# thangktran/HardwareAwareOptimalQuantumCircuitCuttingAndKnitting

Hardware: AMD Instinct MI355X
Metric: subcircuit-instances/s (full-knit wall time = ms_per_step), syc 32 p=2 (higher is better)
Workload: dtype f64

## Files before the change

hardwareawareoptimalquantumcircuitcuttingandknitting_amd/_lib.py:

```python
from __future__ import annotations

import ctypes
import os
import threading

_HERE = os.path.dirname(os.path.abspath(__file__))
LIB_PATH = os.environ.get("QKNIT_LIB") or os.path.join(_HERE, "libqknit.so")

c_i32, c_i64, c_u32, c_u64 = ctypes.c_int32, ctypes.c_int64, ctypes.c_uint32, ctypes.c_uint64
c_vp, c_dp, c_lp = ctypes.c_void_p, ctypes.POINTER(ctypes.c_double), ctypes.POINTER(ctypes.c_int64)


class QkPass(ctypes.Structure):
    _fields_ = [("tile_mask", c_u64), ("group_begin", c_i32), ("group_end", c_i32),
                ("flags", c_i32), ("traced_local", c_u32)]


class QkProgram(ctypes.Structure):
    _fields_ = [("n", c_i32), ("n_eff", c_i32), ("m", c_i32), ("n_slots", c_i32),
                ("packed", c_i32), ("n_passes", c_i32), ("passes", ctypes.POINTER(QkPass)),
                ("ops", c_vp), ("groups", c_vp), ("mats", c_vp)]


class QkLowrankPlan(ctypes.Structure):
    _fields_ = [("nbits", c_i32), ("terms", c_i32), ("rows_a", c_i64), ("rows_b", c_i64), ("mask_a", c_u64),
                ("mask_b", c_u64), ("wt_a", c_vp), ("wt_b", c_vp), ("probes", c_vp), ("lam_tol", ctypes.c_double),
                ("s_tol", ctypes.c_double), ("s_abs", ctypes.c_double), ("rank_tol", ctypes.c_double),
                ("rank_tol_rel", ctypes.c_double)]


class QkKnitPlan(ctypes.Structure):
    _fields_ = [("n_frag", c_i32), ("nbits", c_i32), ("terms", c_i64), ("rows", ctypes.POINTER(c_i64)),
                ("clbit_masks", ctypes.POINTER(c_u64)), ("transforms", ctypes.POINTER(c_vp))]


SIGNATURES = {
    "qk_version": (ctypes.c_char_p, []),
    "qk_ctx_create": (c_i32, [ctypes.c_int, ctypes.POINTER(c_vp)]),
    "qk_ctx_destroy": (c_i32, [c_vp]),
    "qk_ctx_set_stream": (c_i32, [c_vp, c_vp]),
    "qk_ctx_synchronize": (c_i32, [c_vp]),
    "qk_last_error": (ctypes.c_char_p, [c_vp]),
    "qk_stream_create_cu_masked": (c_i32, [ctypes.c_int, ctypes.POINTER(c_u32), ctypes.c_int, ctypes.POINTER(c_vp)]),
    "qk_stream_destroy": (c_i32, [c_vp]),
    "qk_stream_cu_count": (c_i32, [ctypes.c_int, c_vp, ctypes.POINTER(ctypes.c_int)]),
    "qk_out_alloc": (c_i32, [c_vp, c_i64, ctypes.POINTER(c_vp)]),
    "qk_out_free": (c_i32, [c_vp, c_vp]),
    "qk_out_mapped_bytes": (c_i32, [c_vp, ctypes.POINTER(c_i64)]),
    "qk_out_write_rate": (c_i32, [c_vp, c_vp, c_i64, ctypes.POINTER(ctypes.c_double)]),
    "qk_out_stats": (c_i32, [ctypes.POINTER(c_i64), c_i32]),
    "qk_sweep_workspace_bytes": (c_i32, [ctypes.POINTER(QkProgram), c_i64, ctypes.POINTER(c_i64)]),
    "qk_sweep": (c_i32, [c_vp, ctypes.POINTER(QkProgram), c_i64, c_vp, c_vp, c_vp, c_i64, c_vp]),
    "qk_module_compile": (c_i32, [c_vp, ctypes.c_char_p, ctypes.POINTER(ctypes.c_char_p), ctypes.c_int,
                                  ctypes.POINTER(c_vp)]),
    "qk_module_destroy": (c_i32, [c_vp]),
    "qk_module_load": (c_i32, [c_vp, c_vp, c_i64, ctypes.POINTER(ctypes.c_char_p), ctypes.c_int, ctypes.POINTER(c_vp)]),
    "qk_module_code": (c_i32, [c_vp, c_vp, ctypes.POINTER(c_i64)]),
    "qk_sweep_compiled": (c_i32, [c_vp, c_vp, ctypes.POINTER(QkProgram), c_i64, c_vp, c_vp, c_vp, c_i64,
                                  c_vp]),
    "qk_sweep_compiled_labels": (c_i32, [c_vp, c_vp, ctypes.POINTER(QkProgram), c_i64, c_vp, c_vp, c_i64, c_vp,
                                         c_vp, c_i64, c_vp]),
    "qk_sweep_compiled_multi": (c_i32, [c_vp, c_vp, ctypes.c_int, ctypes.POINTER(QkProgram), c_lp, c_vp, c_vp, c_lp,
                                        c_vp, c_vp, c_lp, c_vp, c_vp]),
    "qk_sweep_compiled_multi_shared": (c_i32, [c_vp, c_vp, ctypes.c_int, ctypes.POINTER(QkProgram), c_lp, c_vp, c_vp,
                                               c_lp, c_vp, c_vp, c_lp, c_vp, c_vp, c_lp, c_vp, c_vp]),
    "qk_reduce_labels": (c_i32, [c_vp, c_i64, c_vp, c_i64, c_vp, c_vp]),
    "qk_gemm_keyed": (c_i32, [c_vp, c_i64, c_i64, c_i64, c_vp, c_i64, c_vp, c_i64, c_vp, c_i64,
                              c_vp, c_i64, c_vp, ctypes.c_int]),
    "qk_gemm_keyed_pred": (c_i32, [c_vp, c_i64, c_i64, c_i64, c_vp, c_i64, c_vp, c_i64, c_vp, c_i64,
                                   c_vp, c_i64, c_vp, ctypes.c_int, c_vp]),
    "qk_gemm_outer_paired": (c_i32, [c_vp, c_i64, c_i64, c_i64, c_vp, c_i64, c_vp, c_i64, c_vp, c_i64,
                                     c_vp, c_vp]),
    "qk_knit_outer_stream": (c_i32, [c_vp, ctypes.c_int, c_i64, c_vp, c_i64, c_vp, c_i64, ctypes.c_uint64,
                                     ctypes.c_uint64, c_vp]),
    "qk_knit_outer_stream_kind": (c_i32, [ctypes.c_int, c_i64, c_u64, c_u64, c_i64, c_i64,
                                          ctypes.POINTER(ctypes.c_int), ctypes.POINTER(ctypes.c_int)]),
    "qk_knit_outer_stream_range": (c_i32, [c_vp, ctypes.c_int, c_i64, c_vp, c_i64, c_vp, c_i64, ctypes.c_uint64,
                                           ctypes.c_uint64, c_i64, c_i64, c_vp, c_vp]),
    "qk_rank_factors": (c_i32, [c_vp, c_i64, c_vp, c_vp, ctypes.c_double, ctypes.c_double, ctypes.c_double,
                                ctypes.c_int, c_vp, c_vp, c_vp]),
    "qk_prep_workspace_bytes": (c_i32, [c_vp, c_i64, c_i64, ctypes.POINTER(c_i64)]),
    "qk_prep_operands": (c_i32, [c_vp, ctypes.c_int, ctypes.c_int, c_vp, c_vp, c_i64, c_i64, c_vp, ctypes.c_int,
                                 c_vp, c_vp, c_i64, c_i64, c_vp, c_vp, c_vp, c_vp, c_vp, c_vp, c_i64]),
    "qk_qprep_workspace_bytes": (c_i32, [c_vp, c_i64, c_i64, ctypes.POINTER(c_i64)]),
    "qk_qprep_grams": (c_i32, [c_vp, ctypes.c_int, ctypes.c_int, c_vp, c_vp, c_i64, c_i64, ctypes.c_int, c_vp, c_vp,
                               c_i64, c_i64, c_vp, c_vp, c_vp, c_vp, c_vp, c_i64]),
    "qk_qprep_compress_check": (c_i32, [c_vp, ctypes.c_int, ctypes.c_int, ctypes.c_int, c_vp, c_vp, c_i64, c_i64,
                                        ctypes.c_int, c_vp, c_vp, c_i64, c_i64, c_vp, c_vp, c_vp, c_vp, c_vp, c_vp,
                                        c_vp, c_vp, ctypes.c_double, ctypes.c_double, c_vp, c_vp, c_vp, c_i64]),
    "qk_compress_operands": (c_i32, [c_vp, ctypes.c_int, ctypes.c_int, c_vp, c_vp, c_i64, c_vp, c_vp, c_vp, c_i64,
                                     c_vp]),
    "qk_compress_operands_ld": (c_i32, [c_vp, ctypes.c_int, ctypes.c_int, c_vp, c_vp, c_i64, c_i64, c_vp, c_i64, c_vp,
                                        c_vp, c_i64, c_i64, c_vp, c_i64]),
    "qk_compress_probe_v": (c_i32, [c_vp, ctypes.c_int, ctypes.c_int, c_vp, c_vp, c_i64, c_i64, c_vp, c_i64, c_vp, c_vp,
                                    c_i64, c_i64, c_vp, c_i64, c_vp, c_i64, c_vp, c_i64]),
    "qk_probe_errors_vpart": (c_i32, [c_vp, ctypes.c_int, ctypes.c_int, c_vp, c_i64, c_i64, c_vp, c_i64, c_vp, c_vp,
                                      c_i64, c_vp, c_vp, ctypes.c_double, ctypes.c_double, c_vp, c_vp, c_vp, c_i64,
                                      c_vp]),
    "qk_probe_workspace_bytes": (c_i32, [c_vp, c_i64, ctypes.POINTER(c_i64)]),
    "qk_probe_errors": (c_i32, [c_vp, ctypes.c_int, ctypes.c_int, c_vp, c_i64, c_i64, c_vp, c_i64, c_vp, c_vp, c_i64,
                                c_i64, c_vp, c_i64, c_vp, c_vp, ctypes.c_double, ctypes.c_double, c_vp, c_vp, c_vp,
                                c_i64]),
    "qk_probe_errors_tally": (c_i32, [c_vp, ctypes.c_int, ctypes.c_int, c_vp, c_i64, c_i64, c_vp, c_i64, c_vp, c_vp, c_i64,
                                c_i64, c_vp, c_i64, c_vp, c_vp, ctypes.c_double, ctypes.c_double, c_vp, c_vp, c_vp,
                                c_i64, c_vp]),
    "qk_probe_accept": (c_i32, [c_vp, c_vp, ctypes.c_int, c_vp, ctypes.c_double, ctypes.c_double, c_vp, c_vp]),
    "qk_rank_tally": (c_i32, [c_vp, c_vp, c_vp, c_vp]),
    "qk_knit_workspace_bytes": (c_i32, [ctypes.POINTER(QkKnitPlan), ctypes.POINTER(c_i64)]),
    "qk_knit": (c_i32, [c_vp, ctypes.POINTER(QkKnitPlan), c_vp, c_vp, c_i64, c_vp]),
    "qk_khatri_rao": (c_i32, [c_vp, c_i64, c_i64, c_i64, c_vp, c_i64, c_vp, c_i64, c_vp]),
    "qk_gather_rows": (c_i32, [c_vp, c_i64, c_i64, c_vp, c_vp, c_vp, c_vp]),
    "qk_npd_workspace_bytes": (c_i32, [c_i64, c_i64, ctypes.POINTER(c_i64)]),
    "qk_threshold_count": (c_i32, [c_vp, c_i64, c_vp, ctypes.c_double, c_vp, c_i64, c_vp]),
    "qk_npd": (c_i32, [c_vp, c_i64, c_vp, ctypes.c_double, c_i64, c_vp, c_i64, c_vp, c_vp, c_vp]),
    "qk_qd_from_rows": (c_i32, [c_vp, c_i64, c_i64, c_vp, c_vp, ctypes.c_double, c_vp]),
    "qk_qd_merge": (c_i32, [c_vp, c_i64, c_vp, c_vp, c_i64, c_vp, c_vp, ctypes.c_double, c_i64, c_vp]),
    "qk_qd_axpby": (c_i32, [c_vp, c_i64, ctypes.c_double, c_vp, ctypes.c_double, c_vp, ctypes.c_double, c_vp]),
    "qk_hellinger": (c_i32, [c_vp, c_i64, c_vp, c_vp, c_vp]),
    "qk_knit_lowrank_workspace_bytes": (c_i32, [c_vp, c_vp, ctypes.POINTER(c_i64)]),
    "qk_knit_lowrank": (c_i32, [c_vp, c_vp, c_vp, c_vp, c_vp, c_i64, c_vp, c_vp]),
    "qk_comm_unique_id": (c_i32, [c_vp]),
    "qk_comm_init": (c_i32, [c_vp, c_vp, ctypes.c_int, ctypes.c_int, ctypes.POINTER(c_vp)]),
    "qk_comm_destroy": (c_i32, [c_vp]),
    "qk_comm_size": (c_i32, [c_vp, ctypes.POINTER(ctypes.c_int), ctypes.POINTER(ctypes.c_int)]),
    "qk_allreduce": (c_i32, [c_vp, c_vp, c_vp, c_vp, c_i64]),
    "qk_reduce": (c_i32, [c_vp, c_vp, c_vp, c_vp, c_i64, ctypes.c_int]),
    "qk_allgather": (c_i32, [c_vp, c_vp, c_vp, c_vp, c_i64]),
    "qk_alltoall": (c_i32, [c_vp, c_vp, c_vp, c_vp, c_i64]),
    "qk_knit_select_workspace_bytes": (c_i32, [ctypes.c_int, c_u64, c_u64, ctypes.POINTER(c_i64)]),
    "qk_knit_select": (c_i32, [c_vp, ctypes.c_int, c_i64, c_vp, c_i64, c_vp, c_i64, c_u64, c_u64, ctypes.c_double,
                               c_vp, c_vp, c_i64, c_i64, c_vp, c_vp, c_vp]),
    "qk_select_above": (c_i32, [c_vp, c_i64, c_vp, ctypes.c_double, c_i64, c_i64, c_vp, c_vp, c_vp]),
    "qk_npd_pairs_workspace_bytes": (c_i32, [c_i64, ctypes.POINTER(c_i64)]),
    "qk_npd_pairs": (c_i32, [c_vp, c_i64, c_vp, c_vp, c_vp, c_i64, c_vp, c_vp, c_vp]),
    "qk_sample_cdf": (c_i32, [c_vp, c_i64, c_vp, c_i64, c_vp, c_vp]),
    "qk_sample_counts": (c_i32, [c_vp, c_i64, c_i64, c_vp, c_vp, c_vp, c_i64, c_vp, c_i64, c_u64, c_vp]),
    "qk_fold_counts": (c_i32, [c_vp, c_i64, c_vp, c_i64, c_vp, c_vp, c_i64, ctypes.c_double, c_vp]),
}

_lock = threading.Lock()
_lib = None


class QknitError(RuntimeError):
    pass


def lib() -> ctypes.CDLL:
    global _lib
    with _lock:
        if _lib is None:
            if not os.path.exists(LIB_PATH):
                raise QknitError(
                    f"{LIB_PATH} not built: run `python -c 'import __graft_entry__ as g; g.build()'`"
                )
            handle = ctypes.CDLL(LIB_PATH)
            for name, (res, args) in SIGNATURES.items():
                fn = getattr(handle, name)
                fn.restype = res
                fn.argtypes = args
            _lib = handle
# ... 8 lines not shown
```

hardwareawareoptimalquantumcircuitcuttingandknitting_amd/build.py:

```python
from __future__ import annotations

import os
import shutil
import subprocess

HERE = os.path.dirname(os.path.abspath(__file__))
SRCS = [os.path.join(HERE, "csrc", f) for f in ("qknit.hip", "qknit_post.hip", "qknit_jit.hip",
                                                              "qknit_sample.hip", "qknit_rank.hip",
                                                              "qknit_plan.hip", "qknit_prep.hip",
                                                              "qknit_select.hip", "qknit_comm.hip",
                                                              "qknit_mem.hip", "qknit_trunc.hip",
                                                              "qknit_prim.hip")]
DEPS = SRCS + [os.path.join(HERE, "csrc", h) for h in ("internal.h", "sweep_ops.h", "prim.h")]
HEADER = os.path.join(os.path.dirname(HERE), "include", "qknit.h")
OUT = os.path.join(HERE, "libqknit.so")
ARCH = os.environ.get("QKNIT_ARCH", "gfx950")


def hipcc() -> str:
    for cand in (os.environ.get("HIPCC"), shutil.which("hipcc"), "/opt/rocm/bin/hipcc"):
        if cand and os.path.exists(cand):
            return cand
    raise RuntimeError("hipcc not found")


def build_library(force: bool = False, verbose: bool = False, out: str = OUT,
                  defines: tuple = ()) -> str:
    stale = not os.path.exists(out) or any(
        os.path.getmtime(p) > os.path.getmtime(out) for p in DEPS + [HEADER]
    )
    if not (force or stale):
        return out
    tmp = out + ".tmp"
    flags = [f"--offload-arch={ARCH}", "-O3", "-std=c++17", "-fPIC", "-Wall", "-Wno-unused-result",
             *[f"-D{d}" for d in defines]]
    objdir = os.path.join(os.path.dirname(out), "build", os.path.basename(out) + ".objs")
    os.makedirs(objdir, exist_ok=True)
    jobs = []
    for src in SRCS:
        obj = os.path.join(objdir, os.path.basename(src) + ".o")
        cmd = [hipcc(), *flags, "-c", src, "-o", obj]
        jobs.append((cmd, obj, subprocess.Popen(cmd, stdout=subprocess.PIPE, stderr=subprocess.PIPE, text=True)))
    errs = []
    for cmd, obj, proc in jobs:
        _, err = proc.communicate()
        if proc.returncode != 0:
            errs.append(f"{' '.join(cmd)}\n{err}")
        elif verbose and err:
            print(err)
    if errs:
        raise RuntimeError("hipcc failed:\n" + "\n".join(errs))
    cmd = [hipcc(), *flags, "-shared", *[obj for _, obj, _ in jobs], "-lhiprtc", "-lrccl", "-o", tmp]
    res = subprocess.run(cmd, capture_output=True, text=True)
    if res.returncode != 0:
        raise RuntimeError(f"hipcc link failed:\n{' '.join(cmd)}\n{res.stderr}")
    os.replace(tmp, out)
    return out


AOT_CONFIGS = ("qft_16_1_p3", "syc_32_5_p2", "syc_32_1_p2", "syc_32_1_p2_forced", "hwe_16_1_p2", "hwe_16_1_p3")


def build_jit_cache(configs=AOT_CONFIGS, verbose: bool = False) -> list:
    import tempfile

    from . import VirtualCircuit, cutting, engine

    todo = {}
    for key in configs:
        name, n, d, p, var = cutting.BASELINE_CONFIGS[key]
        cut = cutting.config_cut_circuit(name, n, d, p, var)[1]
        virt = VirtualCircuit(cut)
        for basis in ({False, True} if virt.vgate_instructions else {False}):
            for src, _ in engine.jit_sources(virt, basis=basis):
                path = engine.jit_cache_path(src)
                if not os.path.exists(path):
                    todo[path] = src
    os.makedirs(engine.JIT_CACHE_DIR, exist_ok=True)
    procs = []
    with tempfile.TemporaryDirectory() as tmp:
        for i, (path, src) in enumerate(todo.items()):
            f = os.path.join(tmp, f"prog{i}.hip")
            with open(f, "w") as fh:
                fh.write(src)
            cmd = [hipcc(), "--genco", "--no-gpu-bundle-output", *engine.jit_options(src), f, "-o", path + ".tmp"]
            procs.append((path, cmd, subprocess.Popen(cmd, stdout=subprocess.PIPE, stderr=subprocess.PIPE, text=True)))
        errs = []
        for path, cmd, proc in procs:
            _, err = proc.communicate()
            if proc.returncode != 0:
                errs.append(f"{' '.join(cmd)}\n{err}")
            else:
                os.replace(path + ".tmp", path)
                if verbose:
                    print(f"jit cache: {path}")
        if errs:
# ... 3 lines not shown
```

hardwareawareoptimalquantumcircuitcuttingandknitting_amd/csrc/qknit.hip:

```cpp
#include <hip/hip_runtime.h>

#include <cstdlib>

#include <cstdint>
#include <cstdio>
#include <cstring>
#include <string>

#include "internal.h"
#include "sweep_ops.h"

namespace {

constexpr int TILE = 1 << QK_TILE_BITS;
constexpr int NT = 256;

int fail(qk_ctx* ctx, int code, const char* fmt, const char* detail = "") {
    if (ctx) {
        char buf[512];
        snprintf(buf, sizeof(buf), fmt, detail);
        ctx->err = buf;
    }
    return code;
}

#define QK_HIP(ctx, call)                                                     \
    do {                                                                      \
        hipError_t e_ = (call);                                               \
        if (e_ != hipSuccess) return fail(ctx, QK_EHIP, "%s", hipGetErrorString(e_)); \
    } while (0)

using namespace qk_sweep_ops;

__device__ __forceinline__ void pin(double2 (&v)[PER]) {
#pragma unroll
    for (int r = 0; r < PER; ++r) asm volatile("" : "+v"(v[r].x), "+v"(v[r].y));
}

__device__ __forceinline__ void dispatch_u1(int a, double2 (&v)[PER], const double* m) {
    switch (a) {
        case 0: ap_u1<0>(v, m); pin(v); break;
        case 1: ap_u1<1>(v, m); pin(v); break;
        case 2: ap_u1<2>(v, m); pin(v); break;
        default: ap_u1<3>(v, m); pin(v); break;
    }
}

__device__ __forceinline__ void dispatch_u1r(int a, double2 (&v)[PER], const double* m) {
    switch (a) {
        case 0: ap_u1r<0>(v, m); pin(v); break;
        case 1: ap_u1r<1>(v, m); pin(v); break;
        case 2: ap_u1r<2>(v, m); pin(v); break;
        default: ap_u1r<3>(v, m); pin(v); break;
    }
}

__device__ __forceinline__ void dispatch_u1x(int a, double2 (&v)[PER], const double* m) {
    switch (a) {
        case 0: ap_u1x<0>(v, m); pin(v); break;
        case 1: ap_u1x<1>(v, m); pin(v); break;
        case 2: ap_u1x<2>(v, m); pin(v); break;
        default: ap_u1x<3>(v, m); pin(v); break;
    }
}

__device__ __forceinline__ void dispatch_d1r(int a, double2 (&v)[PER], const double* d) {
    switch (a) {
        case 0: ap_d1r<0>(v, d); pin(v); break;
        case 1: ap_d1r<1>(v, d); pin(v); break;
        case 2: ap_d1r<2>(v, d); pin(v); break;
        default: ap_d1r<3>(v, d); pin(v); break;
    }
}

__device__ __forceinline__ void dispatch_d1(int a, double2 (&v)[PER], const double* d) {
    switch (a) {
        case 0: ap_d1<0>(v, d); pin(v); break;
        case 1: ap_d1<1>(v, d); pin(v); break;
        case 2: ap_d1<2>(v, d); pin(v); break;
        default: ap_d1<3>(v, d); pin(v); break;
    }
}

__device__ __forceinline__ int pair_id(int a, int b) {
    return a == 0 ? b - 1 : (a == 1 ? b + 1 : 5);
}

__device__ __forceinline__ void dispatch_u2(int a, int b, double2 (&v)[PER], const double* m) {
    switch (pair_id(a, b)) {
        case 0: ap_u2<0, 1>(v, m); pin(v); break;
        case 1: ap_u2<0, 2>(v, m); pin(v); break;
        case 2: ap_u2<0, 3>(v, m); pin(v); break;
// ... 322 lines not shown

#ifndef QK_GEMM_GROUP
#define QK_GEMM_GROUP 8
#endif
#ifndef QK_GEMM_NT
#define QK_GEMM_NT 1
#endif

typedef double d2_t __attribute__((ext_vector_type(2)));

__device__ __forceinline__ void gemm_load(d2_t (&r)[4], const double* __restrict__ X, int64_t ld,
                                          int64_t k0, int64_t K, int64_t c0, int64_t cols, bool full) {
    const double* p = X + k0 * ld + c0;
    const int rl = threadIdx.x >> 6, cl = 2 * (threadIdx.x & 63);
    const int64_t off = (int64_t)rl * ld + cl;
    if (full) {
#pragma unroll
        for (int j = 0; j < 4; ++j) r[j] = *reinterpret_cast<const d2_t*>(p + 4 * j * ld + off);
    } else {
        const int kl = (int)(K - k0 < GK ? K - k0 : GK);
        const int cc = (int)(cols - c0 < GT ? cols - c0 : GT);
#pragma unroll
        for (int j = 0; j < 4; ++j) {
            const double* q = p + 4 * j * ld + off;
            const bool rv = rl + 4 * j < kl;
            r[j].x = (rv && cl < cc) ? q[0] : 0.0;
            r[j].y = (rv && cl + 1 < cc) ? q[1] : 0.0;
        }
    }
}

#ifndef QK_GEMM_STORE
#define QK_GEMM_STORE 1
#endif

template <typename T>
__device__ __forceinline__ T dpp_swap_pair(T v) {
    static_assert(sizeof(T) == 8, "64-bit values only");
    int2 w = *reinterpret_cast<int2*>(&v);
    w.x = __builtin_amdgcn_mov_dpp(w.x, 0xB1, 0xF, 0xF, false);
    w.y = __builtin_amdgcn_mov_dpp(w.y, 0xB1, 0xF, 0xF, false);
    return *reinterpret_cast<T*>(&w);
}

__device__ __forceinline__ void gemm_store_pair(double* p, d2_t v) {
#if QK_GEMM_STORE == 2
    asm volatile("global_store_dwordx4 %0, %1, off sc1\n\ts_nop 1" : : "v"(p), "v"(v) : "memory");
#elif QK_GEMM_STORE == 3
    *reinterpret_cast<d2_t*>(p) = v;
#else
    __builtin_nontemporal_store(v, reinterpret_cast<d2_t*>(p));
#endif
}

__device__ __forceinline__ void gemm_store_out(double* p, double v) {
#if QK_GEMM_NT
    __builtin_nontemporal_store(v, p);
#else
    *p = v;
#endif
}

#ifndef QK_GEMM_PERSIST
#define QK_GEMM_PERSIST 1
#endif
#ifndef QK_GEMM_WG_PER_CU
#define QK_GEMM_WG_PER_CU 2
#endif

struct GemmArgs {
    int64_t M, N, K;
    const double* __restrict__ A;
    int64_t lda;
    const double* __restrict__ B;
    int64_t ldb;
    const int64_t* __restrict__ keyA;
    int64_t strideA;
    const int64_t* __restrict__ keyB;
    int64_t strideB;
    double* __restrict__ out;
    int beta;
    int64_t tiles_m, tiles_n;
    const int32_t* skip = nullptr;
};

__device__ __forceinline__ bool gemm_skipped(const GemmArgs& g) { return g.skip && *g.skip > 0; }

__device__ __forceinline__ void gemm_tile_coords(int64_t seq, int64_t tiles_m, int64_t tiles_n,
                                                 int64_t& bm, int64_t& bn) {
    const uint32_t q = (uint32_t)seq, tm = (uint32_t)tiles_m, tn = (uint32_t)tiles_n;
#if QK_GEMM_GROUP
    const uint32_t per_group = (uint32_t)QK_GEMM_GROUP * tn;
    const uint32_t g = q / per_group, r = q - g * per_group;
    const uint32_t first = g * QK_GEMM_GROUP;
    const uint32_t gsize = tm - first < (uint32_t)QK_GEMM_GROUP ? tm - first : (uint32_t)QK_GEMM_GROUP;
    bm = first + r % gsize;
    bn = r / gsize;
#else
    bm = q % tm;
    bn = q / tm;
#endif
}

template <bool FULL>
__device__ __forceinline__ void gemm_epilogue(const GemmArgs& g, int64_t m0, int64_t n0, d4_t (&acc)[4][4]) {
    const int lane = threadIdx.x & 63, wave = threadIdx.x >> 6;
    const int wm = wave & 1, wn = wave >> 1;
    const int64_t M = g.M, N = g.N;
    int64_t kcol[4];
#pragma unroll
    for (int j = 0; j < 4; ++j) {
        const int64_t col = n0 + wn * 64 + j * 16 + (lane & 15);
        kcol[j] = (FULL || col < N) ? (g.keyB ? g.keyB[col] : col * g.strideB) : -1;
    }
#if QK_GEMM_STORE
    bool pairable = FULL || (!g.beta && n0 + GT <= N);
    if (pairable) {
        bool ok = true;
#pragma unroll
        for (int j = 0; j < 4; ++j) {
            const int64_t nb = dpp_swap_pair(kcol[j]);
            ok = ok && ((lane & 1) ? nb + 1 == kcol[j] : kcol[j] + 1 == nb);
        }
        pairable = __all(ok);
    }
    if (pairable) {
        const bool odd = lane & 1;
#pragma unroll
        for (int i = 0; i < 4; ++i) {
#pragma unroll
            for (int rp = 0; rp < 4; rp += 2) {
                const int rr = rp + (odd ? 1 : 0);
                const int64_t row = m0 + wm * 64 + i * 16 + (lane >> 4) + 4 * rr;
                const int64_t krow = (FULL || row < M) ? (g.keyA ? g.keyA[row] : row * g.strideA) : -1;
#pragma unroll
                for (int j = 0; j < 4; ++j) {
                    const double x = odd ? acc[i][j][rp] : acc[i][j][rp + 1];
                    const double y = dpp_swap_pair(x);
                    d2_t v;
                    v.x = odd ? y : acc[i][j][rp];
                    v.y = odd ? acc[i][j][rp + 1] : y;
#ifdef QK_GEMM_NOSTORE
                    if (v.x != 1234.5678) continue;
#endif
                    if (FULL || krow >= 0) gemm_store_pair(g.out + krow + kcol[j] - (odd ? 1 : 0), v);
                }
            }
        }
        return;
    }
#endif
#pragma unroll
    for (int i = 0; i < 4; ++i) {
        int64_t krow[4];
#pragma unroll
        for (int r = 0; r < 4; ++r) {
            const int64_t row = m0 + wm * 64 + i * 16 + (lane >> 4) + 4 * r;
            krow[r] = row < M ? (g.keyA ? g.keyA[row] : row * g.strideA) : -1;
        }
#pragma unroll
        for (int j = 0; j < 4; ++j)
#pragma unroll
            for (int r = 0; r < 4; ++r) {
#ifdef QK_GEMM_NOSTORE
                if (acc[i][j][r] != 1234.5678) continue;
#endif
                if (krow[r] < 0 || kcol[j] < 0) continue;
                double* o = g.out + krow[r] + kcol[j];
                if (g.beta) *o += acc[i][j][r];
                else gemm_store_out(o, acc[i][j][r]);
            }
    }
}

__device__ __forceinline__ bool gemm_vec(const double* X, int64_t ld, int64_t c0, int64_t cols) {
    return ((ld & 1) == 0) && ((reinterpret_cast<uintptr_t>(X) & 15) == 0) && c0 + GT <= cols;
}

__device__ __forceinline__ void gemm_load_first(const GemmArgs& g, int64_t bm, int64_t bn, d2_t (&ra)[4],
                                                d2_t (&rb)[4]) {
    gemm_load(ra, g.A, g.lda, 0, g.K, bm * GT, g.M, gemm_vec(g.A, g.lda, bm * GT, g.M) && GK <= g.K);
    gemm_load(rb, g.B, g.ldb, 0, g.K, bn * GT, g.N, gemm_vec(g.B, g.ldb, bn * GT, g.N) && GK <= g.K);
}

__device__ __forceinline__ void gemm_tile(const GemmArgs& g, int64_t bm, int64_t bn, bool have_next,
                                          int64_t nbm, int64_t nbn, d2_t (&ra)[4], d2_t (&rb)[4],
                                          double (*As)[GK][GT + GPAD], double (*Bs)[GK][GT + GPAD],
                                          int& buf) {
    const int tid = threadIdx.x, lane = tid & 63, wave = tid >> 6;
    const int wm = wave & 1, wn = wave >> 1;
    const int64_t M = g.M, N = g.N, K = g.K;
    const int64_t m0 = bm * GT, n0 = bn * GT;

    d4_t acc[4][4];
#pragma unroll
    for (int i = 0; i < 4; ++i)
#pragma unroll
        for (int j = 0; j < 4; ++j) acc[i][j] = (d4_t){0.0, 0.0, 0.0, 0.0};

    const int lr = tid >> 6;
    const int lc = 2 * (tid & 63);
    for (int64_t k0 = 0; k0 < K; k0 += GK) {
#ifdef QK_GEMM_NOLDSW
        if (k0 == 0)
#endif
        {
#pragma unroll
        for (int j = 0; j < 4; ++j) {
            *reinterpret_cast<d2_t*>(&As[buf][lr + 4 * j][lc]) = ra[j];
            *reinterpret_cast<d2_t*>(&Bs[buf][lr + 4 * j][lc]) = rb[j];
        }
        __syncthreads();
        }
        const bool more = k0 + GK < K;
#ifdef QK_GEMM_NOLOAD
        if (!more && have_next) {
#else
        if (more || have_next) {
#endif
            const int64_t pk = more ? k0 + GK : 0;
            const int64_t pm = more ? m0 : nbm * GT, pn = more ? n0 : nbn * GT;
            const bool kfull = pk + GK <= K;
            gemm_load(ra, g.A, g.lda, pk, K, pm, M, gemm_vec(g.A, g.lda, pm, M) && kfull);
            gemm_load(rb, g.B, g.ldb, pk, K, pn, N, gemm_vec(g.B, g.ldb, pn, N) && kfull);
        }
#pragma unroll
        for (int kk = 0; kk < GK / 4; ++kk) {
            const int kr2 = kk * 4 + (lane >> 4);
            double fa[4], fb[4];
#pragma unroll
            for (int t = 0; t < 4; ++t) {
                fa[t] = As[buf][kr2][wm * 64 + t * 16 + (lane & 15)];
                fb[t] = Bs[buf][kr2][wn * 64 + t * 16 + (lane & 15)];
            }
#pragma unroll
            for (int i = 0; i < 4; ++i)
#pragma unroll
                for (int j = 0; j < 4; ++j)
                    acc[i][j] = __builtin_amdgcn_mfma_f64_16x16x4f64(fa[i], fb[j], acc[i][j], 0, 0, 0);
        }
        buf ^= 1;
    }
    gemm_epilogue<false>(g, m0, n0, acc);
}

__global__ __launch_bounds__(256, 2) void qk_gemm_keyed_kernel(GemmArgs g) {
    __shared__ __attribute__((aligned(16))) double As[2][GK][GT + GPAD];
    __shared__ __attribute__((aligned(16))) double Bs[2][GK][GT + GPAD];
    if (gemm_skipped(g)) return;
    const int64_t nblk = g.tiles_m * g.tiles_n;
    int buf = 0;
    int64_t bm, bn;
#if QK_GEMM_PERSIST
    const int64_t G = gridDim.x;
    const bool xcd = nblk % 8 == 0 && G % 8 == 0;
    const int64_t per_xcd = xcd ? nblk / 8 : nblk, stride = xcd ? G / 8 : G;
    const int64_t base = xcd ? (blockIdx.x % 8) * per_xcd : 0;
    int64_t li = xcd ? blockIdx.x / 8 : blockIdx.x;
    if (li >= per_xcd) return;
    d2_t ra[4], rb[4];
    gemm_tile_coords(base + li, g.tiles_m, g.tiles_n, bm, bn);
    gemm_load_first(g, bm, bn, ra, rb);
    for (; li < per_xcd; li += stride) {
        const bool have_next = li + stride < per_xcd;
        int64_t nbm = 0, nbn = 0;
        if (have_next) gemm_tile_coords(base + li + stride, g.tiles_m, g.tiles_n, nbm, nbn);
        gemm_tile(g, bm, bn, have_next, nbm, nbn, ra, rb, As, Bs, buf);
        bm = nbm;
        bn = nbn;
    }
#else
    int64_t bid = (int64_t)blockIdx.y * gridDim.x + blockIdx.x;
    if (bid >= nblk) return;
    if (nblk % 8 == 0) bid = (bid % 8) * (nblk / 8) + bid / 8;
    gemm_tile_coords(bid, g.tiles_m, g.tiles_n, bm, bn);
    d2_t ra[4], rb[4];
    gemm_load_first(g, bm, bn, ra, rb);
    gemm_tile(g, bm, bn, false, 0, 0, ra, rb, As, Bs, buf);
#endif
}

#ifndef QK_GEMM_GLDS
#define QK_GEMM_GLDS 1
#endif
#ifndef QK_G2K
#define QK_G2K 16
#endif
#ifndef QK_G2S
#define QK_G2S 2
#endif
#ifndef QK_GLDS_WG_PER_CU
#define QK_GLDS_WG_PER_CU 2
#endif
#ifndef QK_GEMM_PRIO
#define QK_GEMM_PRIO 0
#endif
constexpr int G2K = QK_G2K;
constexpr int G2S = QK_G2S;
constexpr int G2L = G2K / 2;

struct GemmRing {
    double a[G2K][GT + GPAD];
    double b[G2K][GT + GPAD];
};

__device__ __forceinline__ void glds16(const double* src, double* lds_row) {
    __builtin_amdgcn_global_load_lds(reinterpret_cast<const void*>(src),
                                     reinterpret_cast<__attribute__((address_space(3))) void*>(
                                         reinterpret_cast<uintptr_t>(lds_row)),
                                     16, 0, 0);
}

__device__ __forceinline__ void gemm_ring_wait(int n) {
#define QK_VMW(k) case k: asm volatile("s_waitcnt vmcnt(" #k ")" ::: "memory"); break;
#define QK_VMW8(k) QK_VMW(k) QK_VMW(k + 1) QK_VMW(k + 2) QK_VMW(k + 3) QK_VMW(k + 4) QK_VMW(k + 5) QK_VMW(k + 6) QK_VMW(k + 7)
    switch (n < 63 ? n : 63) {
        QK_VMW8(0) QK_VMW8(8) QK_VMW8(16) QK_VMW8(24) QK_VMW8(32) QK_VMW8(40) QK_VMW8(48)
        QK_VMW(56) QK_VMW(57) QK_VMW(58) QK_VMW(59) QK_VMW(60) QK_VMW(61) QK_VMW(62) QK_VMW(63)
        default: asm volatile("s_waitcnt vmcnt(0)" ::: "memory");
    }
#undef QK_VMW8
#undef QK_VMW
}

__global__ __launch_bounds__(256, 2) void qk_gemm_glds_kernel(GemmArgs g) {
    __shared__ __attribute__((aligned(16))) GemmRing ring[G2S];
    if (gemm_skipped(g)) return;
    const int lane = threadIdx.x & 63, wave = threadIdx.x >> 6;
    const int wm = wave & 1, wn = wave >> 1;
    const int64_t nblk = g.tiles_m * g.tiles_n;
    const int64_t G = gridDim.x;
    const bool xcd = nblk % 8 == 0 && G % 8 == 0;
    const int64_t per_xcd = xcd ? nblk / 8 : nblk, stride = xcd ? G / 8 : G;
    const int64_t base = xcd ? (blockIdx.x % 8) * per_xcd : 0;
    const int64_t li0 = xcd ? blockIdx.x / 8 : blockIdx.x;
    if (li0 >= per_xcd) return;
    const int nct = (int)(g.K / G2K);
    const int ntile = (int)((per_xcd - li0 + stride - 1) / stride);
    const int total = ntile * nct;

    int it = 0, ic = 0, issued = 0;
    int64_t ibm, ibn;
    gemm_tile_coords(base + li0, g.tiles_m, g.tiles_n, ibm, ibn);
    const int wave_s = __builtin_amdgcn_readfirstlane(wave);
    const int src_off = 2 * lane;
    auto issue = [&]() {
        if (issued >= total) return;
        GemmRing& r = ring[issued % G2S];
        const int64_t k0 = (int64_t)ic * G2K;
#pragma unroll
        for (int q = 0; q < G2K / 4; ++q) {
            const int row = wave_s * (G2K / 4) + q;
            const double* pa = g.A + (k0 + row) * g.lda + ibm * GT;
            const double* pb = g.B + (k0 + row) * g.ldb + ibn * GT;
            glds16(pa + src_off, &r.a[row][0]);
            glds16(pb + src_off, &r.b[row][0]);
        }
        ++issued;
        if (++ic == nct) {
            ic = 0;
            ++it;
            if (it < ntile) gemm_tile_coords(base + li0 + (int64_t)it * stride, g.tiles_m, g.tiles_n, ibm, ibn);
        }
    };
    for (int s = 0; s < G2S - 1; ++s) issue();

    d4_t acc[4][4];
#pragma unroll
    for (int i = 0; i < 4; ++i)
#pragma unroll
        for (int j = 0; j < 4; ++j) acc[i][j] = (d4_t){0.0, 0.0, 0.0, 0.0};
    int64_t bm, bn;
    gemm_tile_coords(base + li0, g.tiles_m, g.tiles_n, bm, bn);
    int t = 0, c = 0;
    for (int gc = 0; gc < total; ++gc) {
        int after = G2L * ((total - 1 - gc) < (G2S - 2) ? (total - 1 - gc) : (G2S - 2));
#pragma unroll
        for (int d = 1; d < G2S; ++d)
            if (gc - d >= 0 && (gc - d + 1) % nct == 0) after += 32;
        gemm_ring_wait(after);
        asm volatile("s_waitcnt lgkmcnt(0)" ::: "memory");
        __builtin_amdgcn_s_barrier();
        const GemmRing& r = ring[gc % G2S];
        double fa[2][4], fb[2][4];
        auto frags = [&](int kk) {
            const int kr = kk * 4 + (lane >> 4);
#pragma unroll
            for (int q = 0; q < 4; ++q) {
                fa[kk & 1][q] = r.a[kr][wm * 64 + q * 16 + (lane & 15)];
                fb[kk & 1][q] = r.b[kr][wn * 64 + q * 16 + (lane & 15)];
            }
        };
        frags(0);
        issue();
#pragma unroll
        for (int kk = 0; kk < G2K / 4; ++kk) {
            if (kk + 1 < G2K / 4) frags(kk + 1);
#if QK_GEMM_PRIO
            __builtin_amdgcn_s_setprio(1);
#endif
#pragma unroll
            for (int i = 0; i < 4; ++i)
#pragma unroll
                for (int j = 0; j < 4; ++j)
                    acc[i][j] = __builtin_amdgcn_mfma_f64_16x16x4f64(fa[kk & 1][i], fb[kk & 1][j], acc[i][j], 0,
                                                                     0, 0);
#if QK_GEMM_PRIO
            __builtin_amdgcn_s_setprio(0);
#endif
        }
        if (++c == nct) {
            gemm_epilogue<true>(g, bm * GT, bn * GT, acc);
#pragma unroll
            for (int i = 0; i < 4; ++i)
#pragma unroll
                for (int j = 0; j < 4; ++j) acc[i][j] = (d4_t){0.0, 0.0, 0.0, 0.0};
            c = 0;
            if (++t < ntile) gemm_tile_coords(base + li0 + (int64_t)t * stride, g.tiles_m, g.tiles_n, bm, bn);
        }
    }
}

#ifndef QK_GEMM_WAVE
#define QK_GEMM_WAVE 1
#endif
#ifndef QK_WAVE_WG_PER_CU
#define QK_WAVE_WG_PER_CU 2
#endif
constexpr int DW = 4;

struct WaveRing {
    double a[DW][4][64];
    double b[DW][4][64];
    int64_t key[2][64];
};

__device__ __forceinline__ void glds16_at(const void* src, void* lds_base) {
    __builtin_amdgcn_global_load_lds(src,
                                     reinterpret_cast<__attribute__((address_space(3))) void*>(
                                         reinterpret_cast<uintptr_t>(lds_base)),
                                     16, 0, 0);
}

template <int NKS>
__global__ __launch_bounds__(256, 2) void qk_gemm_wave_kernel(GemmArgs g) {
    __shared__ __attribute__((aligned(16))) WaveRing rings[4];
    if (gemm_skipped(g)) return;
    const int lane = threadIdx.x & 63, wave = threadIdx.x >> 6;
    const int wm = wave & 1, wn = wave >> 1;
    WaveRing& ring = rings[__builtin_amdgcn_readfirstlane(wave)];
    const int64_t nblk = g.tiles_m * g.tiles_n;
    const int64_t G = gridDim.x;
    const bool xcd = nblk % 8 == 0 && G % 8 == 0;
    const int64_t per_xcd = xcd ? nblk / 8 : nblk, stride = xcd ? G / 8 : G;
    const int64_t base = xcd ? (blockIdx.x % 8) * per_xcd : 0;
    int64_t li = xcd ? blockIdx.x / 8 : blockIdx.x;
    if (li >= per_xcd) return;
    const int64_t lda = g.lda, ldb = g.ldb;
    const int p = lane & 31;
    const int chunkA = p < 16 ? 2 * p : 2 * (p - 16) + 1;
    const int64_t offA = (int64_t)(lane >> 5) * lda + wm * 64 + 2 * chunkA;
    const int64_t offB = (int64_t)(lane >> 5) * ldb + wn * 64 + 2 * p;
    const int64_t* tabA = g.keyA ? g.keyA : reinterpret_cast<const int64_t*>(g.A);
    const int64_t* tabB = g.keyB ? g.keyB : reinterpret_cast<const int64_t*>(g.B);
    const int64_t keyOff = 2 * (lane & 31);

    int64_t bm, bn;
    gemm_tile_coords(base + li, g.tiles_m, g.tiles_n, bm, bn);
    const double* pa = g.A + bm * GT + offA;
    const double* pb = g.B + bn * GT + offB;
    const double* na = pa;
    const double* nb = pb;
    if (li + stride < per_xcd) {
        int64_t tbm, tbn;
        gemm_tile_coords(base + li + stride, g.tiles_m, g.tiles_n, tbm, tbn);
        na = g.A + tbm * GT + offA;
        nb = g.B + tbn * GT + offB;
    }
    auto issue = [&](int slot, int ks) {
        const double* a = ks < NKS ? pa + (int64_t)(4 * ks) * lda : na + (int64_t)(4 * (ks - NKS)) * lda;
        const double* b = ks < NKS ? pb + (int64_t)(4 * ks) * ldb : nb + (int64_t)(4 * (ks - NKS)) * ldb;
        glds16_at(a, &ring.a[slot][0][0]);
        glds16_at(a + 2 * lda, &ring.a[slot][2][0]);
        glds16_at(b, &ring.b[slot][0][0]);
        glds16_at(b + 2 * ldb, &ring.b[slot][2][0]);
    };
#pragma unroll
    for (int s = 0; s < DW - 1; ++s) issue(s, s);

    int prev_stores = 0;
    const int rho = lane & 15, kk = lane >> 4;
    auto tile = [&]() -> bool {
        d4_t acc[4][4];
#pragma unroll
        for (int i = 0; i < 4; ++i)
#pragma unroll
            for (int j = 0; j < 4; ++j) acc[i][j] = (d4_t){0.0, 0.0, 0.0, 0.0};
        static_assert(NKS % DW == 0, "k-steps per tile must be a multiple of the ring depth");
#pragma unroll
        for (int ks = 0; ks < NKS; ++ks) {
            issue((ks + DW - 1) % DW, ks + DW - 1);
            if (ks == 0) {
                const int64_t* t = lane < 32 ? tabA + (g.keyA ? bm * GT + wm * 64 : 0) + keyOff
                                             : tabB + (g.keyB ? bn * GT + wn * 64 : 0) + keyOff;
                glds16_at(t, &ring.key[0][0]);
            }
            static_assert(DW == 4, "wait counts below are for a 4-deep ring");
            if (ks <= DW - 2) {
                if (prev_stores == 0) asm volatile("s_waitcnt vmcnt(13)" ::: "memory");
                else if (prev_stores == 32) asm volatile("s_waitcnt vmcnt(45)" ::: "memory");
                else asm volatile("s_waitcnt vmcnt(63)" ::: "memory");
            } else if (ks == DW - 1) {
                asm volatile("s_waitcnt vmcnt(13)" ::: "memory");
            } else {
                asm volatile("s_waitcnt vmcnt(12)" ::: "memory");
            }
            const int s = ks % DW;
            const d2_t a0 = *reinterpret_cast<const d2_t*>(&ring.a[s][kk][2 * rho]);
            const d2_t a1 = *reinterpret_cast<const d2_t*>(&ring.a[s][kk][32 + 2 * rho]);
            const d2_t b0 = *reinterpret_cast<const d2_t*>(&ring.b[s][kk][2 * rho]);
            const d2_t b1 = *reinterpret_cast<const d2_t*>(&ring.b[s][kk][32 + 2 * rho]);
            const double fa[4] = {a0.x, a0.y, a1.x, a1.y};
            const double fb[4] = {b0.x, b0.y, b1.x, b1.y};
#pragma unroll
            for (int i = 0; i < 4; ++i)
#pragma unroll
                for (int j = 0; j < 4; ++j)
                    acc[i][j] = __builtin_amdgcn_mfma_f64_16x16x4f64(fa[i], fb[j], acc[i][j], 0, 0, 0);
            __builtin_amdgcn_sched_barrier(0);
        }
        static_assert(4 * (NKS - 1) <= 63, "vmcnt field");
        asm volatile("s_waitcnt vmcnt(%0)" ::"n"(4 * (NKS - 1)) : "memory");
        const int64_t* keyR = &ring.key[0][0];
        const int64_t* keyC = &ring.key[0][0] + 64;
        int64_t kr[4][4], kc[4];
        if (g.keyA) {
#pragma unroll
            for (int r = 0; r < 4; ++r)
#pragma unroll
                for (int i = 0; i < 4; ++i) kr[r][i] = keyR[4 * kk + 16 * r + i];
        } else {
#pragma unroll
            for (int r = 0; r < 4; ++r)
#pragma unroll
                for (int i = 0; i < 4; ++i) kr[r][i] = (bm * GT + wm * 64 + 4 * kk + 16 * r + i) * g.strideA;
        }
        if (g.keyB) {
#pragma unroll
            for (int j = 0; j < 4; ++j) kc[j] = keyC[2 * rho + (j & 1) + 32 * (j >> 1)];
        } else {
#pragma unroll
            for (int j = 0; j < 4; ++j) kc[j] = (bn * GT + wn * 64 + 2 * rho + (j & 1) + 32 * (j >> 1)) * g.strideB;
        }
        int64_t odd = (kc[0] | kc[2]) & 1;
#pragma unroll
        for (int r = 0; r < 4; ++r)
#pragma unroll
            for (int i = 0; i < 4; ++i) odd |= kr[r][i] & 1;
        const bool pair = __all(kc[1] == kc[0] + 1 && kc[3] == kc[2] + 1 && odd == 0);
        if (pair) {
#pragma unroll
            for (int r = 0; r < 4; ++r)
#pragma unroll
                for (int i = 0; i < 4; ++i)
#pragma unroll
                    for (int jp = 0; jp < 2; ++jp) {
                        d2_t v;
                        v.x = acc[i][2 * jp][r];
                        v.y = acc[i][2 * jp + 1][r];
                        gemm_store_pair(g.out + kr[r][i] + kc[2 * jp], v);
                    }
            prev_stores = 32;
        } else {
#pragma unroll
            for (int r = 0; r < 4; ++r)
#pragma unroll
                for (int i = 0; i < 4; ++i)
#pragma unroll
                    for (int j = 0; j < 4; ++j) gemm_store_out(g.out + kr[r][i] + kc[j], acc[i][j][r]);
            prev_stores = 64;
        }
        li += stride;
        if (li >= per_xcd) return false;
        gemm_tile_coords(base + li, g.tiles_m, g.tiles_n, bm, bn);
        pa = na;
        pb = nb;
        if (li + stride < per_xcd) {
            int64_t tbm, tbn;
            gemm_tile_coords(base + li + stride, g.tiles_m, g.tiles_n, tbm, tbn);
            na = g.A + tbm * GT + offA;
            nb = g.B + tbn * GT + offB;
        }
        return true;
    };
    while (tile()) {
    }
    asm volatile("s_waitcnt vmcnt(0)" ::: "memory");
}

constexpr int SK_MAX = 8;
#ifndef QK_SK_U
#define QK_SK_U 4
#endif
constexpr int SK_U = QK_SK_U;

template <bool KEYED>
__global__ __launch_bounds__(256) void qk_gemm_smallk_kernel(GemmArgs g) {
    if (gemm_skipped(g)) return;
    const int K = (int)g.K;
    for (int64_t row = blockIdx.x; row < g.M; row += gridDim.x) {
        double a[SK_MAX];
#pragma unroll
        for (int k = 0; k < SK_MAX; ++k) a[k] = k < K ? g.A[k * g.lda + row] : 0.0;
        const int64_t base = g.keyA ? g.keyA[row] : row * g.strideA;
        double* o = g.out + base;
        if ((base & 1) == 0) {
            int64_t j0 = 2 * (int64_t)threadIdx.x;
            for (; j0 + 512 * (SK_U - 1) < g.N; j0 += 512 * SK_U) {
                d2_t acc[SK_U];
#pragma unroll
                for (int u = 0; u < SK_U; ++u) acc[u] = (d2_t){0.0, 0.0};
#pragma unroll
                for (int k = 0; k < SK_MAX; ++k) {
                    if (k < K) {
#pragma unroll
                        for (int u = 0; u < SK_U; ++u) {
                            const d2_t b = *reinterpret_cast<const d2_t*>(g.B + k * g.ldb + j0 + 512 * u);
                            acc[u].x = fma(a[k], b.x, acc[u].x);
                            acc[u].y = fma(a[k], b.y, acc[u].y);
                        }
                    }
                }
#pragma unroll
                for (int u = 0; u < SK_U; ++u) {
                    const int64_t col = KEYED ? g.keyB[j0 + 512 * u] : j0 + 512 * u;
                    __builtin_nontemporal_store(acc[u], reinterpret_cast<d2_t*>(o + col));
                }
            }
            for (int64_t j = j0; j < g.N; j += 512) {
                d2_t acc = {0.0, 0.0};
                for (int k = 0; k < K; ++k) {
                    const d2_t b = *reinterpret_cast<const d2_t*>(g.B + k * g.ldb + j);
                    acc.x = fma(a[k], b.x, acc.x);
                    acc.y = fma(a[k], b.y, acc.y);
                }
                __builtin_nontemporal_store(acc, reinterpret_cast<d2_t*>(o + (KEYED ? g.keyB[j] : j)));
            }
        } else {
            for (int64_t j = threadIdx.x; j < g.N; j += 256) {
                double acc = 0.0;
                for (int k = 0; k < K; ++k) acc = fma(a[k], g.B[k * g.ldb + j], acc);
                __builtin_nontemporal_store(acc, o + (KEYED ? g.keyB[j] : j));
            }
        }
    }
}

#ifndef QK_OS_U
#define QK_OS_U 1
#endif
#ifndef QK_OS_NT
#define QK_OS_NT 1
#endif
#ifndef QK_OS_WG_PER_CU
#define QK_OS_WG_PER_CU 8
#endif
#ifndef QK_OS_P
#define QK_OS_P 1
#endif
constexpr int OS_U = QK_OS_U;
constexpr int OS_P = QK_OS_P;
constexpr int64_t OS_CHUNK = 2 * OS_P * 256 * OS_U;

struct OuterStreamArgs {
    int nbits, K;
    const double* __restrict__ A;
    int64_t lda;
    const double* __restrict__ B;
    int64_t ldb;
    uint32_t maskA, maskB;
    double* __restrict__ out;
};

__device__ __forceinline__ uint32_t pext32(uint32_t x, uint32_t mask) {
    uint32_t r = 0, bit = 1;
    for (; mask; mask &= mask - 1, bit <<= 1)
        if (x & mask & (~mask + 1)) r |= bit;
    return r;
}

__global__ __launch_bounds__(256) void qk_knit_outer_stream_kernel(OuterStreamArgs a) {
    __shared__ uint32_t tab[2][4][256];
    for (int i = threadIdx.x; i < 4 * 256; i += 256) {
        const int byte = i >> 8, v = i & 255;
        tab[0][byte][v] = pext32((uint32_t)v << (8 * byte), a.maskA);
        tab[1][byte][v] = pext32((uint32_t)v << (8 * byte), a.maskB);
    }
    __syncthreads();
    const int K = a.K;
    const int64_t total = int64_t(1) << a.nbits;
    for (int64_t c0 = (int64_t)blockIdx.x * OS_CHUNK; c0 < total; c0 += (int64_t)gridDim.x * OS_CHUNK) {
        d2_t v[OS_U * OS_P];
#pragma unroll
        for (int up = 0; up < OS_U * OS_P; ++up) {
            const int u = up / OS_P, pp = up % OS_P;
            const int64_t o = c0 + 512 * OS_P * u + 2 * (OS_P * threadIdx.x + pp);
            const uint32_t x = (uint32_t)o;
            uint32_t row = 0, col = 0;
#pragma unroll
            for (int byte = 0; byte < 4; ++byte) {
                const uint32_t b = (x >> (8 * byte)) & 255;
                row += tab[0][byte][b];
                col += tab[1][byte][b];
            }
            d2_t acc = {0.0, 0.0};
            if (o < total) {
#pragma unroll
                for (int k = 0; k < SK_MAX; ++k) {
                    if (k < K) {
                        const double av = a.A[k * a.lda + row];
                        const d2_t bv = *reinterpret_cast<const d2_t*>(a.B + k * a.ldb + col);
                        acc.x = fma(av, bv.x, acc.x);
                        acc.y = fma(av, bv.y, acc.y);
                    }
                }
            }
            v[up] = acc;
        }
#pragma unroll
        for (int up = 0; up < OS_U * OS_P; ++up) {
            const int u = up / OS_P, pp = up % OS_P;
            const int64_t o = c0 + 512 * OS_P * u + 2 * (OS_P * threadIdx.x + pp);
            if (o < total) {
#if QK_OS_NT
                __builtin_nontemporal_store(v[up], reinterpret_cast<d2_t*>(a.out + o));
#else
                *reinterpret_cast<d2_t*>(a.out + o) = v[up];
#endif
            }
        }
    }
}

#ifndef QK_OB_NT
#define QK_OB_NT 0
#endif
struct OuterBlockedArgs {
    int K, TB;
    const double* __restrict__ A;
    int64_t lda;
    const double* __restrict__ B;
    int64_t ldb;
    uint32_t maskA, maskB;
    int64_t task_begin, task_end;
    int64_t o_begin;
    const int32_t* kdev;
    double* __restrict__ out;
    int64_t spread;
};

template <bool BG>
__global__ __launch_bounds__(256) void qk_knit_outer_blocked_kernel(OuterBlockedArgs a) {
    int K = a.K;
    if (a.kdev) {
        const int kd = *a.kdev;
        if (kd <= 0) return;
        K = kd < K ? kd : K;
    }
    __shared__ uint32_t tab[2][2][256];
    extern __shared__ double stage[];
    const uint32_t low = (1u << a.TB) - 1u;
    const uint32_t mAl = a.maskA & low, mBl = a.maskB & low;
    const int na = 1 << __builtin_popcount(mAl), nb = 1 << __builtin_popcount(mBl);
    double* sA = stage;
    double* sB = stage + (int64_t)a.K * na;
    for (int i = threadIdx.x; i < 512; i += 256) {
        const int byte = i >> 8, v = i & 255;
        tab[0][byte][v] = pext32((uint32_t)v << (8 * byte), mAl);
        tab[1][byte][v] = pext32((uint32_t)v << (8 * byte), mBl);
    }
    __syncthreads();
    const uint32_t r0 = tab[0][0][(2 * threadIdx.x) & 255], c0 = tab[1][0][(2 * threadIdx.x) & 255];
    const int iters = (1 << a.TB) / 512;
    const int64_t n_tasks = a.task_end - a.task_begin, per_part = n_tasks / a.spread;
    for (int64_t i = blockIdx.x; i < n_tasks; i += gridDim.x) {
        const int64_t t = a.task_begin + (i % a.spread) * per_part + i / a.spread;
        const uint32_t base = (uint32_t)(t << a.TB);
        const uint32_t ah = pext32(base, a.maskA), bh = pext32(base, a.maskB);
        __syncthreads();
        for (int i = threadIdx.x; i < K * na; i += 256) {
            const int k = i / na;
            sA[i] = a.A[k * a.lda + ah + (i - k * na)];
        }
        if (!BG)
            for (int i = threadIdx.x; i < K * nb; i += 256) {
                const int k = i / nb;
                sB[i] = a.B[k * a.ldb + bh + (i - k * nb)];
            }
        __syncthreads();
        const double* Bg = a.B + bh;
        double* o = a.out + ((int64_t)base - a.o_begin);
#pragma unroll 4
        for (int it = 0; it < iters; ++it) {
            const uint32_t hi = (uint32_t)(2 * it + (threadIdx.x >> 7));
            const uint32_t row = r0 + tab[0][1][hi], col = c0 + tab[1][1][hi];
            d2_t acc = {0.0, 0.0};
#pragma unroll
            for (int k = 0; k < SK_MAX; ++k)
                if (k < K) {
                    const double av = sA[k * na + row];
                    const d2_t bv = BG ? *reinterpret_cast<const d2_t*>(Bg + k * a.ldb + col)
                                       : *reinterpret_cast<const d2_t*>(sB + k * nb + col);
                    acc.x = fma(av, bv.x, acc.x);
                    acc.y = fma(av, bv.y, acc.y);
                }
#if QK_OB_NT
            __builtin_nontemporal_store(acc, reinterpret_cast<d2_t*>(o + 512 * it + 2 * threadIdx.x));
#else
            *reinterpret_cast<d2_t*>(o + 512 * it + 2 * threadIdx.x) = acc;
#endif
        }
    }
}

struct OuterRowsArgs {
    int K;
    const double* __restrict__ A;
    int64_t lda;
    const double* __restrict__ B;
    int64_t ldb;
    uint32_t maskA_hi, maskB_hi;
    int64_t piece_begin, piece_end;
    int64_t o_begin;
    const int32_t* kdev;
    double* __restrict__ out;
    int64_t spread;
};

template <int KR, int C>
__global__ __launch_bounds__(256) void qk_knit_outer_rows_kernel(OuterRowsArgs a) {
    constexpr int NP = 1 << (C - 9);
    int K = a.K;
    if (a.kdev) {
        const int kd = *a.kdev;
        if (kd <= 0) return;
        K = kd < K ? kd : K;
    }
    d2_t b[KR][NP];
    int64_t pb_loaded = -1;
    const int64_t n_pieces = a.piece_end - a.piece_begin, per_part = n_pieces / a.spread;
    for (int64_t i = blockIdx.x; i < n_pieces; i += gridDim.x) {
        const int64_t p = a.piece_begin + (i % a.spread) * per_part + i / a.spread;
        const uint32_t pl = (uint32_t)p;
        const int64_t pb = pext32(pl, a.maskB_hi);
        const uint32_t pa = pext32(pl, a.maskA_hi);
        if (pb != pb_loaded) {
            const double* Bp = a.B + (pb << C) + 2 * threadIdx.x;
#pragma unroll
            for (int k = 0; k < KR; ++k)
#pragma unroll
                for (int i = 0; i < NP; ++i)
                    b[k][i] = k < K ? *reinterpret_cast<const d2_t*>(Bp + k * a.ldb + 512 * i) : (d2_t){0.0, 0.0};
            pb_loaded = pb;
        }
        double av[KR];
#pragma unroll
        for (int k = 0; k < KR; ++k) av[k] = k < K ? a.A[k * a.lda + pa] : 0.0;
        double* o = a.out + ((p << C) - a.o_begin) + 2 * threadIdx.x;
#pragma unroll
        for (int i = 0; i < NP; ++i) {
            d2_t acc = {0.0, 0.0};
#pragma unroll
            for (int k = 0; k < KR; ++k)
                if (k < K) {
                    acc.x = fma(av[k], b[k][i].x, acc.x);
                    acc.y = fma(av[k], b[k][i].y, acc.y);
                }
            *reinterpret_cast<d2_t*>(o + 512 * i) = acc;
        }
    }
}

static int outer_rows_bits(int64_t K, uint64_t maskB, int align_bits) {
    static const int off = getenv("QKNIT_OB_ROWS") ? atoi(getenv("QKNIT_OB_ROWS")) : 1;
    if (!off || K < 1 || K > 8) return 0;
    const int low = __builtin_ctzll(~maskB);
    const int want = K <= 1 ? 13 : (K <= 2 ? 12 : 11);
    return (want <= low && want <= align_bits) ? want : 0;
}

template <int KR, int C>
static int outer_rows_per_cu() {
    static int n = [] {
        int b = 0;
        if (hipOccupancyMaxActiveBlocksPerMultiprocessor(&b, qk_knit_outer_rows_kernel<KR, C>, 256, 0) != hipSuccess)
            b = 2;
        return b < 1 ? 1 : b;
    }();
    return n;
}

constexpr int64_t OB_STAGE_BYTES = 24 * 1024;
constexpr int OB_WG_PER_CU = 64;

int outer_blocked_tile(int nbits, int64_t K, uint64_t maskA, uint64_t maskB, int align_bits, bool* b_global) {
// ... 130 lines not shown

int qk_sweep_workspace_bytes(const qk_program* p, int64_t n_jobs, int64_t* bytes) {
    if (!p || !bytes || n_jobs < 0) return QK_EARG;
    *bytes = p->packed ? 0 : n_jobs * ((int64_t)1 << p->n) * (int64_t)sizeof(double2);
    return QK_OK;
}

int qk_sweep(qk_ctx* ctx, const qk_program* p, int64_t n_jobs, const double* job_slots,
             const double* job_sign, void* workspace, int64_t workspace_bytes, double* pjob) {
    if (!ctx) return QK_EARG;
    if (!p || !p->passes || p->n_passes < 1) return fail(ctx, QK_EARG, "qk_sweep: empty program%s");
    if (n_jobs <= 0) return QK_OK;
    if (!job_sign || !pjob || (p->n_slots > 0 && !job_slots))
        return fail(ctx, QK_EARG, "qk_sweep: null buffer%s");
    if (p->m < 0 || p->m > p->n_eff || p->n_eff > 40)
        return fail(ctx, QK_EARG, "qk_sweep: bad widths%s");
    if (p->packed) {
        if (p->n_eff < QK_FIBER_BITS || p->n_eff > QK_TILE_BITS || p->n_passes != 1)
            return fail(ctx, QK_EARG, "qk_sweep: bad PACKED program%s");
    } else {
        if (p->n <= QK_TILE_BITS || p->n_eff != p->n) return fail(ctx, QK_EARG, "qk_sweep: bad SPLIT program%s");
        int64_t need = 0;
        qk_sweep_workspace_bytes(p, n_jobs, &need);
        if (!workspace || workspace_bytes < need) return fail(ctx, QK_EARG, "qk_sweep: workspace too small%s");
    }
    if (!(p->passes[p->n_passes - 1].flags & 2) || !(p->passes[0].flags & 1))
        return fail(ctx, QK_EARG, "qk_sweep: first pass must INIT and last must be FINAL%s");
    QK_HIP(ctx, hipSetDevice(ctx->device));
    SweepArgs a{};
    a.ops = p->ops;
    a.groups = p->groups;
    a.mats = p->mats;
    a.job_slots = job_slots;
    a.job_sign = job_sign;
    a.state = (double2*)workspace;
    a.pjob = pjob;
    a.n_jobs = n_jobs;
    a.n = p->n;
    a.n_eff = p->n_eff;
    a.m = p->m;
    a.n_slots = p->n_slots;
    for (int ip = 0; ip < p->n_passes; ++ip) {
        const qk_pass& ps = p->passes[ip];
        if (!p->packed && __builtin_popcountll(ps.tile_mask) != QK_TILE_BITS)
            return fail(ctx, QK_EARG, "qk_sweep: SPLIT tile must hold 12 state bits%s");
        a.tile_mask = ps.tile_mask;
        a.group_begin = ps.group_begin;
        a.group_end = ps.group_end;
        a.flags = ps.flags;
        a.traced_local = ps.traced_local;
        const uint64_t nmask = (p->n >= 64) ? ~0ull : ((1ull << p->n) - 1);
        a.init_sparse = (!p->packed && ip == 0 && p->n_passes > 1) ? 1 : 0;
        a.zero_mask = (!p->packed && ip == 1) ? (nmask & ~p->passes[0].tile_mask) : 0;
        if (p->packed) {
            const int64_t per = (int64_t)1 << (QK_TILE_BITS - p->n_eff);
            const int64_t blocks = (n_jobs + per - 1) / per;
            if (blocks > 0x7fffffff) return fail(ctx, QK_EARG, "qk_sweep: too many jobs%s");
            hipLaunchKernelGGL(qk_sweep_pass_kernel<true>, dim3((unsigned)blocks), dim3(NT), 0, ctx->stream, a,
                               a.ops, a.groups, a.mats);
        } else {
            const int64_t blocks = a.init_sparse ? n_jobs : (n_jobs << (p->n - QK_TILE_BITS));
            if (blocks > 0x7fffffff) return fail(ctx, QK_EARG, "qk_sweep: too many tiles%s");
            hipLaunchKernelGGL(qk_sweep_pass_kernel<false>, dim3((unsigned)blocks), dim3(NT), 0, ctx->stream, a,
                               a.ops, a.groups, a.mats);
        }
        QK_HIP(ctx, hipGetLastError());
    }
    return QK_OK;
}

int qk_reduce_labels(qk_ctx* ctx, int64_t n_labels, const int64_t* offsets, int64_t width,
                     const double* pjob, double* q) {
    if (!ctx) return QK_EARG;
    if (n_labels < 0 || width < 0) return fail(ctx, QK_EARG, "qk_reduce_labels: negative size%s");
    if (n_labels == 0 || width == 0) return QK_OK;
    if (!offsets || !pjob || !q) return fail(ctx, QK_EARG, "qk_reduce_labels: null buffer%s");
    QK_HIP(ctx, hipSetDevice(ctx->device));
    hipLaunchKernelGGL(qk_reduce_labels_kernel, dim3(grid_for(n_labels * width, 256)), dim3(256), 0,
                       ctx->stream, n_labels, offsets, width, pjob, q);
    QK_HIP(ctx, hipGetLastError());
    return QK_OK;
}

int qk_gemm_keyed(qk_ctx* ctx, int64_t M, int64_t N, int64_t K, const double* A, int64_t lda,
                  const double* B, int64_t ldb, const int64_t* keyA, int64_t strideA,
                  const int64_t* keyB, int64_t strideB, double* out, int beta) {
    return qk_gemm_keyed_pred(ctx, M, N, K, A, lda, B, ldb, keyA, strideA, keyB, strideB, out, beta, nullptr);
}

int qk_gemm_keyed_pred(qk_ctx* ctx, int64_t M, int64_t N, int64_t K, const double* A, int64_t lda,
                       const double* B, int64_t ldb, const int64_t* keyA, int64_t strideA,
                       const int64_t* keyB, int64_t strideB, double* out, int beta, const int32_t* skip) {
    if (!ctx) return QK_EARG;
    if (M < 0 || N < 0 || K < 0) return fail(ctx, QK_EARG, "qk_gemm_keyed: negative size%s");
    if (M == 0 || N == 0) return QK_OK;
    if (!out || (K > 0 && (!A || !B))) return fail(ctx, QK_EARG, "qk_gemm_keyed: null buffer%s");
    if (lda < M || ldb < N) return fail(ctx, QK_EARG, "qk_gemm_keyed: leading dimension too small%s");
    const int64_t tm = (M + GT - 1) / GT, tn = (N + GT - 1) / GT;
    const int64_t nblk = tm * tn;
    QK_HIP(ctx, hipSetDevice(ctx->device));
    if (nblk >= (int64_t(1) << 31)) return fail(ctx, QK_EARG, "qk_gemm_keyed: too many tiles%s");
    GemmArgs g{M, N, K, A, lda, B, ldb, keyA, strideA, keyB, strideB, out, beta, tm, tn, skip};
    const bool aligned16 = ((reinterpret_cast<uintptr_t>(A) | reinterpret_cast<uintptr_t>(B)) & 15) == 0 &&
                           (lda % 2) == 0 && (ldb % 2) == 0;
    if (K >= 1 && K <= SK_MAX && !beta && !keyB && strideB == 1 && N % 2 == 0 && aligned16 &&
        (reinterpret_cast<uintptr_t>(out) & 15) == 0 && M * N >= (int64_t(1) << 16)) {
        const int cus = ctx->cus;
        const int64_t G = M < (int64_t)cus * 8 ? M : (int64_t)cus * 8;
        hipLaunchKernelGGL(qk_gemm_smallk_kernel<false>, dim3((unsigned)G), dim3(256), 0, ctx->stream, g);
        QK_HIP(ctx, hipGetLastError());
        return QK_OK;
    }
    if (QK_GEMM_WAVE && !beta && M % GT == 0 && N % GT == 0 && (K == 16 || K == 32 || K == 64) && aligned16 &&
        ((reinterpret_cast<uintptr_t>(out) | reinterpret_cast<uintptr_t>(keyA) | reinterpret_cast<uintptr_t>(keyB)) &
         15) == 0) {
        const int cus = ctx->cus;
        int64_t G = (int64_t)cus * QK_WAVE_WG_PER_CU;
        G = G < 8 ? 8 : G - G % 8;
        if (G > nblk) G = nblk;
        if (K == 16) hipLaunchKernelGGL(qk_gemm_wave_kernel<4>, dim3((unsigned)G), dim3(256), 0, ctx->stream, g);
        else if (K == 32) hipLaunchKernelGGL(qk_gemm_wave_kernel<8>, dim3((unsigned)G), dim3(256), 0, ctx->stream, g);
        else hipLaunchKernelGGL(qk_gemm_wave_kernel<16>, dim3((unsigned)G), dim3(256), 0, ctx->stream, g);
        QK_HIP(ctx, hipGetLastError());
        return QK_OK;
    }
    if (QK_GEMM_GLDS && !beta && M % GT == 0 && N % GT == 0 && K % G2K == 0 && K > 0 && aligned16) {
        const int cus = ctx->cus;
        int64_t G = (int64_t)cus * QK_GLDS_WG_PER_CU;
        G = G < 8 ? 8 : G - G % 8;
        if (G > nblk) G = nblk;
        hipLaunchKernelGGL(qk_gemm_glds_kernel, dim3((unsigned)G), dim3(256), 0, ctx->stream, g);
        QK_HIP(ctx, hipGetLastError());
        return QK_OK;
    }
#if QK_GEMM_PERSIST
    const int cus = ctx->cus;
    int64_t G = (int64_t)cus * QK_GEMM_WG_PER_CU;
    G = G < 8 ? 8 : G - G % 8;
    if (G > nblk) G = nblk;
    hipLaunchKernelGGL(qk_gemm_keyed_kernel, dim3((unsigned)G), dim3(256), 0, ctx->stream, g);
#else
    const int64_t gx = nblk < (1 << 20) ? nblk : (1 << 20);
    const int64_t gy = (nblk + gx - 1) / gx;
    if (gy > 65535) return fail(ctx, QK_EARG, "qk_gemm_keyed: too many tiles%s");
    hipLaunchKernelGGL(qk_gemm_keyed_kernel, dim3((unsigned)gx, (unsigned)gy), dim3(256), 0, ctx->stream, g);
#endif
    QK_HIP(ctx, hipGetLastError());
    return QK_OK;
}

int qk_gemm_outer_paired(qk_ctx* ctx, int64_t M, int64_t N, int64_t K, const double* A, int64_t lda,
                         const double* B, int64_t ldb, const int64_t* keyA, int64_t strideA,
                         const int64_t* keyB, double* out) {
    if (!ctx) return QK_EARG;
    if (M < 0 || N < 0 || K < 1 || K > SK_MAX) return fail(ctx, QK_EARG, "qk_gemm_outer_paired: bad size%s");
    if (M == 0 || N == 0) return QK_OK;
    if (!out || !A || !B || !keyB) return fail(ctx, QK_EARG, "qk_gemm_outer_paired: null buffer%s");
    if (lda < M || ldb < N) return fail(ctx, QK_EARG, "qk_gemm_outer_paired: leading dimension too small%s");
    if ((N & 1) || (ldb & 1) || ((reinterpret_cast<uintptr_t>(B) | reinterpret_cast<uintptr_t>(out)) & 15))
        return fail(ctx, QK_EARG, "qk_gemm_outer_paired: N, ldb even and 16-B aligned B/out required%s");
    GemmArgs g{M, N, K, A, lda, B, ldb, keyA, strideA, keyB, 0, out, 0, 0, 0};
    QK_HIP(ctx, hipSetDevice(ctx->device));
    const int cus = ctx->cus;
    const int64_t G = M < (int64_t)cus * 8 ? M : (int64_t)cus * 8;
    hipLaunchKernelGGL(qk_gemm_smallk_kernel<true>, dim3((unsigned)G), dim3(256), 0, ctx->stream, g);
    QK_HIP(ctx, hipGetLastError());
    return QK_OK;
}

int qk_knit_outer_stream(qk_ctx* ctx, int nbits, int64_t K, const double* A, int64_t lda, const double* B,
                         int64_t ldb, uint64_t maskA, uint64_t maskB, double* out) {
    if (!ctx) return QK_EARG;
    if (nbits < 2 || nbits > 32) return fail(ctx, QK_EARG, "qk_knit_outer_stream: need 2 <= nbits <= 32%s");
    return qk_knit_outer_stream_range(ctx, nbits, K, A, lda, B, ldb, maskA, maskB, 0, int64_t(1) << nbits,
                                      nullptr, out);
}

int qk_knit_outer_stream_range(qk_ctx* ctx, int nbits, int64_t K, const double* A, int64_t lda, const double* B,
                               int64_t ldb, uint64_t maskA, uint64_t maskB, int64_t o_begin, int64_t o_count,
                               const int32_t* k_dev, double* out) {
    if (!ctx) return QK_EARG;
    if (nbits < 2 || nbits > 32 || K < 1 || K > SK_MAX)
        return fail(ctx, QK_EARG, "qk_knit_outer_stream: need 2 <= nbits <= 32, 1 <= K <= 8%s");
    const uint64_t full = (uint64_t(1) << nbits) - 1;
    if ((maskA & maskB) || (maskA | maskB) != full || !(maskB & 1))
        return fail(ctx, QK_EARG, "qk_knit_outer_stream: masks must be disjoint, cover all bits, bit 0 in B%s");
    if (!out || !A || !B) return fail(ctx, QK_EARG, "qk_knit_outer_stream: null buffer%s");
    const int64_t M = int64_t(1) << __builtin_popcountll(maskA), N = int64_t(1) << __builtin_popcountll(maskB);
    if (lda < M || ldb < N || (ldb & 1) || ((reinterpret_cast<uintptr_t>(B) | reinterpret_cast<uintptr_t>(out)) & 15))
        return fail(ctx, QK_EARG, "qk_knit_outer_stream: leading dimension / alignment%s");
    if (o_begin < 0 || o_count < 0 || o_begin + o_count > (int64_t(1) << nbits))
        return fail(ctx, QK_EARG, "qk_knit_outer_stream: output range outside 0..2^nbits%s");
    if (o_count == 0) return QK_OK;
    QK_HIP(ctx, hipSetDevice(ctx->device));
    const int cus = ctx->cus;
    const int align = __builtin_ctzll((uint64_t)(o_begin | o_count));
    if (const int rc = outer_rows_bits(K, maskB, align)) {
        const int64_t pieces = o_count >> rc;
        const int64_t nb = int64_t(1) << (__builtin_popcountll(maskB) - rc);
        const int per_cu = K <= 1 ? outer_rows_per_cu<1, 13>() : K <= 2 ? outer_rows_per_cu<2, 12>()
                           : K <= 4 ? outer_rows_per_cu<4, 11>() : outer_rows_per_cu<8, 11>();
        int64_t G = (int64_t)cus * per_cu;
        if (G >= nb) G -= G % nb;
        if (G > pieces) G = pieces;
        const char* rs_env = getenv("QKNIT_OR_SPREAD");
        int64_t spread = rs_env ? atoll(rs_env) : 8;
        if (spread < 1 || pieces % spread || G % (spread * nb) || pieces < 4 * G) spread = 1;
        OuterRowsArgs r{(int)K, A, lda, B, ldb, (uint32_t)(maskA >> rc), (uint32_t)(maskB >> rc), o_begin >> rc,
                        (o_begin >> rc) + pieces, o_begin, k_dev, out, spread};
        const dim3 grid((unsigned)(G < 1 ? 1 : G));
        if (K <= 1) {
            hipLaunchKernelGGL((qk_knit_outer_rows_kernel<1, 13>), grid, dim3(256), 0, ctx->stream, r);
        } else if (K <= 2) {
            hipLaunchKernelGGL((qk_knit_outer_rows_kernel<2, 12>), grid, dim3(256), 0, ctx->stream, r);
        } else if (K <= 4) {
            hipLaunchKernelGGL((qk_knit_outer_rows_kernel<4, 11>), grid, dim3(256), 0, ctx->stream, r);
        } else {
            hipLaunchKernelGGL((qk_knit_outer_rows_kernel<8, 11>), grid, dim3(256), 0, ctx->stream, r);
        }
        QK_HIP(ctx, hipGetLastError());
        return QK_OK;
    }
    bool bg = false;
    const int tb = outer_blocked_tile(nbits, K, maskA, maskB, align, &bg);
    if (tb) {
        const uint64_t low = (uint64_t(1) << tb) - 1;
        const size_t stage = 8 * (size_t)K * ((size_t(1) << __builtin_popcountll(maskA & low)) +
                                              (bg ? 0 : (size_t(1) << __builtin_popcountll(maskB & low))));
        const int64_t tasks = o_count >> tb;
        const char* wgpc_env = getenv("QKNIT_OB_WG_PER_CU");
        const int wgpc = wgpc_env ? atoi(wgpc_env) : OB_WG_PER_CU;
        const int64_t G0 = wgpc > 0 ? (int64_t)cus * wgpc : tasks;
        const char* spread_env = getenv("QKNIT_OB_SPREAD");
        int64_t spread = spread_env ? atoll(spread_env) : (tasks >= 4 * G0 ? 8 : 1);
        if (spread < 1 || tasks % spread) spread = 1;
        OuterBlockedArgs b{(int)K, tb, A, lda, B, ldb, (uint32_t)maskA, (uint32_t)maskB, o_begin >> tb,
                           (o_begin >> tb) + tasks, o_begin, k_dev, out, spread};
        const dim3 grid((unsigned)(tasks < G0 ? tasks : G0));
        if (bg)
            hipLaunchKernelGGL(qk_knit_outer_blocked_kernel<true>, grid, dim3(256), stage, ctx->stream, b);
        else
            hipLaunchKernelGGL(qk_knit_outer_blocked_kernel<false>, grid, dim3(256), stage, ctx->stream, b);
        QK_HIP(ctx, hipGetLastError());
        return QK_OK;
    }
    if (o_begin != 0 || o_count != (int64_t(1) << nbits) || k_dev)
        return fail(ctx, QK_EARG, "qk_knit_outer_stream: output ranges / device K need task-aligned ranges of >= 2^9%s");
    const int64_t chunks = (int64_t(1) << nbits) / OS_CHUNK;
    const int64_t G0 = (int64_t)cus * QK_OS_WG_PER_CU;
    const int64_t G = chunks < 1 ? 1 : (chunks < G0 ? chunks : G0);
    OuterStreamArgs a{nbits, (int)K, A, lda, B, ldb, (uint32_t)maskA, (uint32_t)maskB, out};
    hipLaunchKernelGGL(qk_knit_outer_stream_kernel, dim3((unsigned)G), dim3(256), 0, ctx->stream, a);
    QK_HIP(ctx, hipGetLastError());
    return QK_OK;
}

int qk_knit_outer_stream_kind(int nbits, int64_t K, uint64_t maskA, uint64_t maskB, int64_t o_begin,
                              int64_t o_count, int* kind, int* task_bits) {
    if (!kind || !task_bits || nbits < 2 || nbits > 32 || K < 1 || K > SK_MAX || o_count <= 0) return QK_EARG;
    const int align = __builtin_ctzll((uint64_t)(o_begin | o_count));
    if (const int rc = outer_rows_bits(K, maskB, align)) {
        *kind = 3;
        *task_bits = rc;
        return QK_OK;
    }
    bool bg = false;
    const int tb = outer_blocked_tile(nbits, K, maskA, maskB, align, &bg);
    *kind = tb ? (bg ? 2 : 1) : 0;
    *task_bits = tb;
    return QK_OK;
}

int qk_khatri_rao(qk_ctx* ctx, int64_t K, int64_t M, int64_t N, const double* A, int64_t lda,
                  const double* B, int64_t ldb, double* out) {
    if (!ctx) return QK_EARG;
    if (K < 0 || M < 0 || N < 0) return fail(ctx, QK_EARG, "qk_khatri_rao: negative size%s");
    if (K == 0 || M == 0 || N == 0) return QK_OK;
    if (!A || !B || !out) return fail(ctx, QK_EARG, "qk_khatri_rao: null buffer%s");
    QK_HIP(ctx, hipSetDevice(ctx->device));
    hipLaunchKernelGGL(qk_khatri_rao_kernel, dim3(grid_for(K * M * N, 256)), dim3(256), 0, ctx->stream, K,
                       M, N, A, lda, B, ldb, out);
    QK_HIP(ctx, hipGetLastError());
    return QK_OK;
}

int qk_gather_rows(qk_ctx* ctx, int64_t R, int64_t width, const int64_t* idx, const double* coef,
                   const double* src, double* dst) {
    if (!ctx) return QK_EARG;
    if (R < 0 || width < 0) return fail(ctx, QK_EARG, "qk_gather_rows: negative size%s");
    if (R == 0 || width == 0) return QK_OK;
    if (!idx || !coef || !src || !dst) return fail(ctx, QK_EARG, "qk_gather_rows: null buffer%s");
    QK_HIP(ctx, hipSetDevice(ctx->device));
    hipLaunchKernelGGL(qk_gather_rows_kernel, dim3(grid_for(R * width, 256)), dim3(256), 0, ctx->stream, R,
                       width, idx, coef, src, dst);
    QK_HIP(ctx, hipGetLastError());
    return QK_OK;
}

}
```

hardwareawareoptimalquantumcircuitcuttingandknitting_amd/csrc/qknit_plan.hip:

```cpp
#include <hip/hip_runtime.h>

#include <algorithm>
#include <cstdlib>
#include <string>
#include <vector>

#include "internal.h"

namespace {

int pfail(qk_ctx* ctx, int code, const std::string& msg) {
    if (ctx) ctx->err = msg;
    return code;
}

__global__ void qk_pdep_keys_kernel(int64_t n, uint64_t mask, int64_t* keys) {
    for (int64_t x = blockIdx.x * (int64_t)blockDim.x + threadIdx.x; x < n; x += (int64_t)gridDim.x * blockDim.x) {
        uint64_t m = mask, k = 0, bit = 1;
        for (; m; m &= m - 1, bit <<= 1)
            if ((uint64_t)x & bit) k |= m & (~m + 1);
        keys[x] = (int64_t)k;
    }
}

// ... 88 lines not shown

extern "C" {

int qk_knit_workspace_bytes(const qk_knit_plan* plan, int64_t* bytes) {
    if (!bytes) return QK_EARG;
    Layout L;
    std::string why;
    const int rc = layout(plan, L, why);
    if (rc) return rc;
    *bytes = L.total;
    return QK_OK;
}

int qk_knit(qk_ctx* ctx, const qk_knit_plan* plan, const double* const* q, void* workspace, int64_t workspace_bytes,
            double* out) {
    if (!ctx) return QK_EARG;
    Layout L;
    std::string why;
    int rc = layout(plan, L, why);
    if (rc) return pfail(ctx, rc, why);
    if (!q || !out || !workspace || workspace_bytes < L.total)
        return pfail(ctx, QK_EARG, "qk_knit: null rows / output, or workspace below qk_knit_workspace_bytes");
    for (int f = 0; f < plan->n_frag; ++f)
        if (!q[f]) return pfail(ctx, QK_EARG, "qk_knit: null swept rows");
    if (hipSetDevice(ctx->device) != hipSuccess) return pfail(ctx, QK_EHIP, "qk_knit: hipSetDevice");
    char* ws = static_cast<char*>(workspace);
    const int64_t K = plan->terms;
    auto width = [&](int f) { return int64_t(1) << __builtin_popcountll(plan->clbit_masks[f]); };
    auto X = [&](int f) { return reinterpret_cast<double*>(ws + L.x_off[f]); };
    auto keys = [&](int f) { return L.key_off[f] < 0 ? nullptr : reinterpret_cast<int64_t*>(ws + L.key_off[f]); };
    for (int f = 0; f < plan->n_frag; ++f) {
        const int64_t w = width(f);
        rc = qk_gemm_keyed(ctx, K, w, plan->rows[f], plan->transforms[f], K, q[f], w, nullptr, w, nullptr, 1, X(f), 0);
        if (rc) return rc;
        if (keys(f)) {
            hipLaunchKernelGGL(qk_pdep_keys_kernel, dim3(grid_of(w)), dim3(256), 0, ctx->stream, w,
                               (uint64_t)plan->clbit_masks[f], keys(f));
        }
    }
    auto stride_of = [&](int f) -> int64_t {
        const uint64_t m = plan->clbit_masks[f];
        return m ? int64_t(1) << __builtin_ctzll(m) : 0;
    };
    if (plan->n_frag == 1) {
        const int f = 0;
        double* ones = reinterpret_cast<double*>(ws + L.ones_off);
        hipLaunchKernelGGL(qk_fill_kernel, dim3(grid_of(K)), dim3(256), 0, ctx->stream, K, 1.0, ones);
        rc = qk_gemm_keyed(ctx, width(f), 1, K, X(f), width(f), ones, 1, keys(f), keys(f) ? 0 : stride_of(f), nullptr,
                           0, out, 0);
        if (!rc && hipGetLastError() != hipSuccess) rc = pfail(ctx, QK_EHIP, "qk_knit: launch failed");
        return rc;
    }
    const int fb = L.order.back();
    const double* A = X(L.order[0]);
    const int64_t* kA = keys(L.order[0]);
    int64_t M = width(L.order[0]), sA = kA ? 0 : stride_of(L.order[0]);
    for (int i = 1; i + 1 < plan->n_frag; ++i) {
        const int f = L.order[i];
        double* kr = reinterpret_cast<double*>(ws + L.kr_off + (i & 1) * L.kr_size);
        int64_t* kk = reinterpret_cast<int64_t*>(ws + L.krk_off + (i & 1) * L.krk_size);
        rc = qk_khatri_rao(ctx, K, M, width(f), A, M, X(f), width(f), kr);
        if (rc) return rc;
        hipLaunchKernelGGL(qk_add_keys_kernel, dim3(grid_of(M * width(f))), dim3(256), 0, ctx->stream, M, width(f), kA,
                           keys(f), kk);
        A = kr;
        kA = kk;
        sA = 0;
        M *= width(f);
    }
    rc = qk_gemm_keyed(ctx, M, width(fb), K, A, M, X(fb), width(fb), kA, sA, keys(fb), keys(fb) ? 0 : stride_of(fb),
                       out, 0);
    if (!rc && hipGetLastError() != hipSuccess) rc = pfail(ctx, QK_EHIP, "qk_knit: launch failed");
    return rc;
}

}

namespace {

constexpr int LR_RMAX = 8;
constexpr int LR_PROBES = 16;

struct LowrankLayout {
    int64_t xa, xb, g, u, prep, ta, tb, r, a2, b2, e2, k, err, probe, ka, kb, total;
    int64_t prep_bytes, probe_bytes;
    bool qspace;
};

bool lowrank_qspace(const qk_lowrank_plan* p) {
    const int64_t NA = int64_t(1) << __builtin_popcountll(p->mask_a), NB = int64_t(1) << __builtin_popcountll(p->mask_b);
    const char* env = getenv("QKNIT_QPREP");
    return env && env[0] == '1' && p->rows_a <= 80 && p->rows_b <= 80 && NA % 512 == 0 && NB % 512 == 0;
}

int lowrank_layout(qk_ctx* ctx, const qk_lowrank_plan* p, LowrankLayout& L, std::string& why) {
    if (!p || p->terms < 2 || p->terms > 64 || (p->terms & 1) || p->rows_a < 1 || p->rows_b < 1 || !p->wt_a ||
        !p->wt_b || !p->probes || p->nbits < 2 || p->nbits > 32) {
        why = "qk_knit_lowrank: need even 2 <= terms <= 64, swept rows, transforms, probes, 2 <= nbits <= 32";
        return QK_EARG;
    }
    if (p->rows_a > INT32_MAX || p->rows_b > INT32_MAX) {
        why = "qk_knit_lowrank: rows_a and rows_b must be at most INT32_MAX";
        return QK_EARG;
    }
    const uint64_t full = (uint64_t(1) << p->nbits) - 1;
    if ((p->mask_a & p->mask_b) || (p->mask_a | p->mask_b) != full || !(p->mask_b & 1)) {
        why = "qk_knit_lowrank: masks must be disjoint, cover all nbits output bits, bit 0 in mask_b";
        return QK_EARG;
    }
    const int64_t NA = int64_t(1) << __builtin_popcountll(p->mask_a), NB = int64_t(1) << __builtin_popcountll(p->mask_b);
    if (NA % 128 || NB % 128) {
        why = "qk_knit_lowrank: each fragment needs >= 7 measured clbits (operand widths multiples of 128)";
        return QK_EARG;
    }
    const int64_t K = p->terms;
    int64_t prep = 0, probe = 0;
    int rc = qk_prep_workspace_bytes(ctx, NA, NB, &prep);
    if (!rc) rc = qk_probe_workspace_bytes(ctx, NA, &probe);
    int64_t qprep = 0;
    if (!rc) rc = qk_qprep_workspace_bytes(ctx, NA, NB, &qprep);
    L.qspace = lowrank_qspace(p);
    if (L.qspace && qprep > prep) prep = qprep;
    if (rc) {
        why = "qk_knit_lowrank: workspace queries failed";
        return rc;
    }
    int64_t off = 0;
    auto take = [&](int64_t bytes) { const int64_t o = off; off += align16(bytes); return o; };
    L.xa = take(K * NA * 8);
    L.xb = take(K * NB * 8);
    L.g = take(2 * K * K * 8);
    L.u = take(K * LR_PROBES * 8);
    L.prep = take(prep);
    L.ta = take(LR_RMAX * K * 8);
    L.tb = take(LR_RMAX * K * 8);
    L.r = take(8);
    L.a2 = take(LR_RMAX * NA * 8);
    L.b2 = take(LR_RMAX * NB * 8);
    L.e2 = take(2 * LR_PROBES * 8);
    L.k = take(8);
    L.err = take(8);
    L.probe = take(probe);
    L.ka = contiguous_bits(p->mask_a) ? -1 : take(NA * 8);
    L.kb = contiguous_bits(p->mask_b) ? -1 : take(NB * 8);
    L.total = off;
    L.prep_bytes = prep;
    L.probe_bytes = probe;
    return QK_OK;
}

__global__ void qk_copy_i32_kernel(const int32_t* src, int32_t* dst) { *dst = *src; }

}

extern "C" {

int qk_knit_lowrank_workspace_bytes(qk_ctx* ctx, const qk_lowrank_plan* plan, int64_t* bytes) {
    if (!ctx || !bytes) return QK_EARG;
    LowrankLayout L;
    std::string why;
    const int rc = lowrank_layout(ctx, plan, L, why);
    if (rc) return pfail(ctx, rc, why);
    *bytes = L.total;
    return QK_OK;
}

int qk_knit_lowrank(qk_ctx* ctx, const qk_lowrank_plan* p, const double* q_a, const double* q_b, void* workspace,
                    int64_t workspace_bytes, double* out, int32_t* rank_out) {
    if (!ctx) return QK_EARG;
    LowrankLayout L;
    std::string why;
    int rc = lowrank_layout(ctx, p, L, why);
    if (rc) return pfail(ctx, rc, why);
    if (!q_a || !q_b || !out || !workspace || workspace_bytes < L.total)
        return pfail(ctx, QK_EARG, "qk_knit_lowrank: null rows / output, or workspace below qk_knit_lowrank_workspace_bytes");
    if (hipSetDevice(ctx->device) != hipSuccess) return pfail(ctx, QK_EHIP, "qk_knit_lowrank: hipSetDevice");
    char* ws = static_cast<char*>(workspace);
    auto D = [&](int64_t off) { return reinterpret_cast<double*>(ws + off); };
    const int K = p->terms;
    const int64_t NA = int64_t(1) << __builtin_popcountll(p->mask_a), NB = int64_t(1) << __builtin_popcountll(p->mask_b);
    double *XA = D(L.xa), *XB = D(L.xb), *G = D(L.g), *U = D(L.u);
    int32_t* r = reinterpret_cast<int32_t*>(ws + L.r);
    int32_t* k = reinterpret_cast<int32_t*>(ws + L.k);
    if (L.qspace) {
        const int RA = (int)p->rows_a, RB = (int)p->rows_b;
        rc = qk_qprep_grams(ctx, K, RA, p->wt_a, q_a, NA, NA, RB, p->wt_b, q_b, NB, NB, p->probes, G, G + K * K, U,
                            D(L.prep), L.prep_bytes);
        if (!rc) rc = qk_rank_factors(ctx, K, G, G + K * K, p->lam_tol, p->s_tol, p->s_abs, LR_RMAX, D(L.ta), D(L.tb), r);
        if (!rc)
            rc = qk_qprep_compress_check(ctx, K, LR_RMAX, RA, p->wt_a, q_a, NA, NA, RB, p->wt_b, q_b, NB, NB, D(L.ta),
                                         D(L.tb), U, p->probes, D(L.a2), D(L.b2), D(L.e2), r, p->rank_tol,
                                         p->rank_tol_rel, k, D(L.err), D(L.prep), L.prep_bytes);
        if (!rc) rc = qk_gemm_keyed_pred(ctx, K, NA, RA, p->wt_a, K, q_a, NA, nullptr, NA, nullptr, 1, XA, 0, k);
        if (!rc) rc = qk_gemm_keyed_pred(ctx, K, NB, RB, p->wt_b, K, q_b, NB, nullptr, NB, nullptr, 1, XB, 0, k);
    } else {
        rc = qk_prep_operands(ctx, K, (int)p->rows_a, p->wt_a, q_a, NA, NA, XA, (int)p->rows_b, p->wt_b, q_b, NB, NB,
                              XB, p->probes, G, G + K * K, U, D(L.prep), L.prep_bytes);
        if (!rc) rc = qk_rank_factors(ctx, K, G, G + K * K, p->lam_tol, p->s_tol, p->s_abs, LR_RMAX, D(L.ta), D(L.tb), r);
        if (!rc) rc = qk_compress_operands(ctx, K, LR_RMAX, D(L.ta), XA, NA, D(L.a2), D(L.tb), XB, NB, D(L.b2));
        if (!rc)
            rc = qk_probe_errors(ctx, K, LR_RMAX, XA, NA, NA, D(L.a2), NA, U, D(L.b2), NB, NB, p->probes, NB, D(L.e2),
                                 r, p->rank_tol, p->rank_tol_rel, k, D(L.err), D(L.probe), L.probe_bytes);
    }
    if (!rc)
        rc = qk_knit_outer_stream_range(ctx, p->nbits, LR_RMAX, D(L.a2), NA, D(L.b2), NB, p->mask_a, p->mask_b, 0,
                                        int64_t(1) << p->nbits, k, out);
    if (rc) return rc;
    int64_t* ka = L.ka >= 0 ? reinterpret_cast<int64_t*>(ws + L.ka) : nullptr;
    int64_t* kb = L.kb >= 0 ? reinterpret_cast<int64_t*>(ws + L.kb) : nullptr;
    if (ka) hipLaunchKernelGGL(qk_pdep_keys_kernel, dim3(grid_of(NA)), dim3(256), 0, ctx->stream, NA, p->mask_a, ka);
    if (kb) hipLaunchKernelGGL(qk_pdep_keys_kernel, dim3(grid_of(NB)), dim3(256), 0, ctx->stream, NB, p->mask_b, kb);
    const int64_t sa = ka ? 0 : int64_t(1) << __builtin_ctzll(p->mask_a);
    const int64_t sb = kb ? 0 : int64_t(1) << __builtin_ctzll(p->mask_b);
    rc = qk_gemm_keyed_pred(ctx, NA, NB, K, XA, NA, XB, NB, ka, sa, kb, sb, out, 0, k);
    if (rc) return rc;
    if (rank_out) hipLaunchKernelGGL(qk_copy_i32_kernel, dim3(1), dim3(1), 0, ctx->stream, k, rank_out);
    if (hipGetLastError() != hipSuccess) return pfail(ctx, QK_EHIP, "qk_knit_lowrank: launch failed");
    return QK_OK;
}

}
```

hardwareawareoptimalquantumcircuitcuttingandknitting_amd/csrc/qknit_prep.hip:

```cpp
#include <hip/hip_runtime.h>

#include <cstdint>
#include <string>

#include "internal.h"

namespace {

typedef double d4_t __attribute__((ext_vector_type(4)));
typedef double d2_t __attribute__((ext_vector_type(2)));

constexpr int PK = 64;
constexpr int PCT = 128;
constexpr int PNP = 16;
constexpr int PTH = 512;
constexpr int XLD = PCT + 2;
constexpr int PG_BLK = 10;
constexpr int PPG = PG_BLK * 256;
constexpr int PPA = PPG;
constexpr int PPB = PPG + PK * PNP;
__host__ __device__ constexpr int prep_tri(int bi, int bj) { return bi * 4 - bi * (bi - 1) / 2 + (bj - bi); }

struct PrepSide {
    const double* Wt;
    const double* q;
    int64_t ldq;
    int64_t N;
    int R;
    double* X;
    const double* P;
};

struct PrepArgs {
    PrepSide s[2];
    int K;
    int split;
    double* part;
};

#ifndef QK_PREP_RS
#define QK_PREP_RS 16
#endif
constexpr int PRS = QK_PREP_RS;
constexpr int PRPW = PRS / 8;
static_assert(PRS % 8 == 0 && PRS >= 8, "stage rows: a multiple of 8 (8 waves)");
#ifndef QK_PREP_NS
#define QK_PREP_NS 2
#endif
#ifndef QK_PREP_WG_PER_CU
#define QK_PREP_WG_PER_CU 2
#endif
#ifndef QK_COMPRESS_COLS
#define QK_COMPRESS_COLS 1
#endif
#ifndef QK_PREP_EXP
#define QK_PREP_EXP 0
#endif
constexpr int PNS = QK_PREP_NS;
#ifndef QK_PREP_QPAD
#define QK_PREP_QPAD 16
#endif
#ifndef QK_PREP_WPAD
#define QK_PREP_WPAD 16
#endif
constexpr int QLD = PCT + QK_PREP_QPAD;
constexpr int WLD = PK + QK_PREP_WPAD;
struct PrepStage {
    double q[PRS][QLD];
    double w[PRS][WLD];
};
union PrepLds {
    PrepStage st[PNS];
    double x[PK][XLD];
};

__device__ __forceinline__ void prep_glds(const double* src, double* lds_row) {
    __builtin_amdgcn_global_load_lds(reinterpret_cast<const void*>(src),
                                     reinterpret_cast<__attribute__((address_space(3))) void*>(
                                         reinterpret_cast<uintptr_t>(lds_row)),
                                     16, 0, 0);
}

__device__ __forceinline__ void prep_vmwait(int n) {
    switch (n < 15 ? n : 15) {
#define QK_PW(k) case k: asm volatile("s_waitcnt vmcnt(" #k ")" ::: "memory"); break;
        QK_PW(0) QK_PW(1) QK_PW(2) QK_PW(3) QK_PW(4) QK_PW(5) QK_PW(6) QK_PW(7)
        QK_PW(8) QK_PW(9) QK_PW(10) QK_PW(11) QK_PW(12) QK_PW(13) QK_PW(14) QK_PW(15)
#undef QK_PW
// ... 424 lines not shown
            }
#pragma unroll
            for (int s = 0; s < VB; ++s) {
                const double a = i16 < 8 ? Bt[wave][i16][4 * (s0 + s) + k4] : 0.0;
                va = __builtin_amdgcn_mfma_f64_16x16x4f64(a, pb[s], va, 0, 0, 0);
            }
        }
    }
#pragma unroll
    for (int r = 0; r < 2; ++r) Vw[wave][(k4 + 4 * r) * 16 + i16] = va[r];
    __syncthreads();
    if (tid < PV_PART)
        vpart[wg * PV_PART + tid] = (Vw[0][tid] + Vw[1][tid]) + (Vw[2][tid] + Vw[3][tid]);
}

__global__ __launch_bounds__(256) void qk_probe_v_kernel(int rmax, const double* __restrict__ B2, int64_t ldb2,
                                                         int64_t NB, const double* __restrict__ P, int64_t ldp,
                                                         double* __restrict__ vpart) {
    const int tid = threadIdx.x, lane = tid & 63, wave = tid >> 6;
    double acc[8][4];
#pragma unroll
    for (int jj = 0; jj < 8; ++jj)
#pragma unroll
        for (int q = 0; q < 4; ++q) acc[jj][q] = 0.0;
    struct Col {
        double b[8], pv[4];
    };
    const int64_t step = (int64_t)gridDim.x * 64;
    auto fetch = [&](int64_t c, Col& x) {
        const int64_t cc = c < NB ? c : NB - 1;
#pragma unroll
        for (int jj = 0; jj < 8; ++jj) x.b[jj] = B2[(int64_t)min(jj, rmax - 1) * ldb2 + cc];
#pragma unroll
        for (int q = 0; q < 4; ++q) x.pv[q] = P[(int64_t)(4 * wave + q) * ldp + cc];
    };
    auto mac = [&](const Col& x) {
#pragma unroll
        for (int jj = 0; jj < 8; ++jj)
#pragma unroll
            for (int q = 0; q < 4; ++q) acc[jj][q] = fma(x.b[jj], x.pv[q], acc[jj][q]);
    };
    int64_t c = (int64_t)blockIdx.x * 64 + lane;
    if (c < NB) {
        Col x0, x1;
        fetch(c, x0);
        for (;; c += 2 * step) {
            fetch(c + step, x1);
            __builtin_amdgcn_sched_barrier(0);
            mac(x0);
            if (c + step >= NB) break;
            fetch(c + 2 * step, x0);
            __builtin_amdgcn_sched_barrier(0);
            mac(x1);
            if (c + 2 * step >= NB) break;
        }
    }
#pragma unroll
    for (int jj = 0; jj < 8; ++jj)
#pragma unroll
        for (int q = 0; q < 4; ++q) {
            double v = acc[jj][q];
#pragma unroll
            for (int s = 1; s < 64; s <<= 1) v += __shfl_xor(v, s, 64);
            acc[jj][q] = jj < rmax ? v : 0.0;
        }
    double* out = vpart + (int64_t)blockIdx.x * PV_PART;
    if (lane < 32) {
        const int j8 = lane >> 2, q = lane & 3;
        double v = 0.0;
#pragma unroll
        for (int jj = 0; jj < 8; ++jj)
#pragma unroll
            for (int qq = 0; qq < 4; ++qq)
                if (jj == j8 && qq == q) v = acc[jj][qq];
        out[j8 * 16 + 4 * wave + q] = v;
    }
}

__global__ __launch_bounds__(256) void qk_probe_d_kernel(int K, int rmax, const double* __restrict__ XA, int64_t ldx,
                                                         int64_t NA, const double* __restrict__ A2, int64_t lda2,
                                                         const double* __restrict__ U,
                                                         const double* __restrict__ vpart, int gv,
                                                         double* __restrict__ epart) {
    __shared__ double Us[PK][PNP];
    __shared__ double Vs[16][PNP];
    __shared__ double ep[4][2 * PNP];
    const int tid = threadIdx.x, lane = tid & 63, wave = tid >> 6, l16 = lane & 15, l4 = lane >> 4;
    {
        __shared__ double vh[PV_PART];
        const int e = tid & (PV_PART - 1), h = tid >> 7;
        double t[16];
#pragma unroll
        for (int u = 0; u < 16; ++u) t[u] = 0.0;
        int b = h;
        for (; b + 30 < gv; b += 32) {
            double v[16];
#pragma unroll
            for (int u = 0; u < 16; ++u) v[u] = vpart[(int64_t)(b + 2 * u) * PV_PART + e];
#pragma unroll
            for (int u = 0; u < 16; ++u) t[u] += v[u];
        }
        for (; b < gv; b += 2) t[0] += vpart[(int64_t)b * PV_PART + e];
#pragma unroll
        for (int w = 8; w >= 1; w >>= 1)
#pragma unroll
            for (int u = 0; u < w; ++u) t[u] += t[u + w];
        if (h == 1) vh[e] = t[0];
        __syncthreads();
        if (h == 0) Vs[e / 16][e % 16] = -(t[0] + vh[e]);
        else Vs[8 + e / 16][e % 16] = 0.0;
    }
    for (int e = tid; e < PK * PNP; e += 256) Us[e / PNP][e % PNP] = (e / PNP) < K ? U[e] : 0.0;
    __syncthreads();
    double e2 = 0.0, f2 = 0.0;
    for (int64_t cb = (int64_t)blockIdx.x * 4 + wave; cb * 16 < NA; cb += (int64_t)gridDim.x * 4) {
        const int64_t c = cb * 16 + l16;
        double av[PK / 4], a2[2];
#pragma unroll
        for (int kk = 0; kk < PK / 4; ++kk) av[kk] = XA[(int64_t)min(4 * kk + l4, K - 1) * ldx + c];
#pragma unroll
        for (int jj = 0; jj < 2; ++jj) a2[jj] = A2[(int64_t)min(4 * jj + l4, rmax - 1) * lda2 + c];
        d4_t acc = {0, 0, 0, 0};
#pragma unroll
        for (int kk = 0; kk < PK / 4; ++kk)
            acc = __builtin_amdgcn_mfma_f64_16x16x4f64(av[kk], Us[4 * kk + l4][l16], acc, 0, 0, 0);
#pragma unroll
        for (int rr = 0; rr < 4; ++rr) f2 = fma(acc[rr], acc[rr], f2);
#pragma unroll
        for (int jj = 0; jj < 2; ++jj)
            acc = __builtin_amdgcn_mfma_f64_16x16x4f64(a2[jj], Vs[4 * jj + l4][l16], acc, 0, 0, 0);
#pragma unroll
        for (int rr = 0; rr < 4; ++rr) e2 = fma(acc[rr], acc[rr], e2);
    }
    e2 += __shfl_xor(e2, 16, 64);
    e2 += __shfl_xor(e2, 32, 64);
    f2 += __shfl_xor(f2, 16, 64);
    f2 += __shfl_xor(f2, 32, 64);
    if (l4 == 0) {
        ep[wave][l16] = e2;
        ep[wave][PNP + l16] = f2;
    }
    __syncthreads();
    if (tid < 2 * PNP)
        epart[(int64_t)blockIdx.x * 2 * PNP + tid] = ep[0][tid] + ep[1][tid] + ep[2][tid] + ep[3][tid];
}

constexpr int PE = 2 * PNP;

__global__ __launch_bounds__(256) void qk_probe_accept_kernel(const double* __restrict__ epart, int n,
                                                              const int32_t* __restrict__ r_dev, double tol,
                                                              double rel_tol, double* __restrict__ e2_out,
                                                              int32_t* __restrict__ k_out, double* __restrict__ err_out,
                                                              int64_t* __restrict__ tally = nullptr) {
    __shared__ double acc[256];
    const int tid = threadIdx.x, p = tid % PE;
    constexpr int STEP = 256 / PE;
    double s8[8] = {0, 0, 0, 0, 0, 0, 0, 0};
    int b = tid / PE;
    for (; b + 31 * STEP < n; b += 32 * STEP) {
        double v[32];
#pragma unroll
        for (int u = 0; u < 32; ++u) v[u] = epart[(int64_t)(b + u * STEP) * PE + p];
#pragma unroll
        for (int u = 0; u < 32; ++u) s8[u & 7] += v[u];
    }
    for (; b < n; b += STEP) s8[0] += epart[(int64_t)b * PE + p];
    const double s = ((s8[0] + s8[1]) + (s8[2] + s8[3])) + ((s8[4] + s8[5]) + (s8[6] + s8[7]));
    acc[tid] = s;
    __syncthreads();
    for (int w = 128; w >= PE; w >>= 1) {
        if (tid < w) acc[tid] += acc[tid + w];
        __syncthreads();
    }
    if (tid < PE && e2_out) e2_out[tid] = acc[tid];
    if (tid == 0 && k_out) {
        double m = 0.0, f = 0.0;
        for (int q = 0; q < PNP; ++q) {
            m = fmax(m, acc[q]);
            f = fmax(f, acc[PNP + q]);
        }
        const double err = sqrt(m);
        const double bound = fmax(tol, rel_tol * sqrt(f));
        const int r = *r_dev;
        if (err_out) *err_out = err;
        const int k = (r > 0 && err <= bound) ? r : 0;
        *k_out = k;
        if (tally) {
            tally[0] += r == 0 ? 1 : 0;
            tally[1] += (r > 0 && k == 0) ? 1 : 0;
            tally[2] = k;
            tally[3] += 1;
        }
    }
}

constexpr int QG_T = 512;
constexpr int QG_LD = PCT + 18;
constexpr int QG_NB = 5;
constexpr int QG_RMAX = 16 * QG_NB;
constexpr int QG_UP = QG_NB * (QG_NB + 1) / 2;
constexpr int QG_PART = (QG_UP + QG_NB) * 256;

template <typename F>
__device__ __forceinline__ void stage16(const double* __restrict__ src, int n, int nthreads, F store) {
    for (int e0 = threadIdx.x; e0 < n; e0 += 16 * nthreads) {
        double v[16];
#pragma unroll
        for (int u = 0; u < 16; ++u) {
            const int e = e0 + u * nthreads;
            v[u] = e < n ? src[e] : 0.0;
        }
#pragma unroll
        for (int u = 0; u < 16; ++u) {
            const int e = e0 + u * nthreads;
            if (e < n) store(e, v[u]);
        }
    }
}

struct QGramSide {
    const double* q;
    int64_t ldq, N;
    int R;
    const double* P;
};

struct QGramArgs {
    QGramSide s[2];
    int split;
    int slots;
    double* part;
};

__device__ __forceinline__ void qg_block(int b, int& bi, int& bj) {
    bi = 0;
    int n = QG_NB;
    while (b >= n) {
        b -= n;
        ++bi;
        --n;
    }
    bj = bi + b;
}

__global__ __launch_bounds__(QG_T, 2) void qk_qgram_kernel(QGramArgs a) {
    extern __shared__ __attribute__((aligned(16))) double qs[];
    const int tid = threadIdx.x, lane = tid & 63, wave = tid >> 6;
    const int l16 = lane & 15, l4 = lane >> 4;
    const int wave_s = __builtin_amdgcn_readfirstlane(wave);
    for (int sd = 0; sd < 2; ++sd) {
        const QGramSide& S = a.s[sd];
        const int R = S.R, nb = (R + 15) / 16;
        int bi[3], bj[3];
        bool live[3], probe[3];
#pragma unroll
        for (int t = 0; t < 3; ++t) {
            const int b = wave + 8 * t;
            probe[t] = b >= QG_UP;
            if (!probe[t]) qg_block(b, bi[t], bj[t]);
            else bi[t] = b - QG_UP, bj[t] = 0;
            live[t] = b < QG_UP + QG_NB && bi[t] < nb && (probe[t] ? S.P != nullptr : bj[t] < nb);
        }
        d4_t acc[3];
#pragma unroll
        for (int t = 0; t < 3; ++t) acc[t] = (d4_t){0, 0, 0, 0};
        const bool mine = !a.split || (int)(blockIdx.x & 1) == sd;
        const int64_t t_first = a.split ? (int64_t)(blockIdx.x >> 1) : (int64_t)blockIdx.x;
        const int64_t t_step = a.split ? (int64_t)(gridDim.x >> 1) : (int64_t)gridDim.x;
        const int64_t tiles = S.N / PCT;
        const bool want_p = (live[0] && probe[0]) || (live[1] && probe[1]) || (live[2] && probe[2]);
        for (int64_t t = mine ? t_first : tiles; t < tiles; t += t_step) {
            const int64_t c0 = t * PCT;
            asm volatile("s_waitcnt lgkmcnt(0)" ::: "memory");
            __builtin_amdgcn_s_barrier();
            for (int r = wave_s; r < R; r += QG_T / 64) prep_glds(S.q + (int64_t)r * S.ldq + c0 + 2 * lane, &qs[r * QG_LD]);
            d2_t pv[PCT / 8];
// ... 670 lines not shown
```

hardwareawareoptimalquantumcircuitcuttingandknitting_amd/engine.py:

```python
from __future__ import annotations

import atexit
import contextlib
import ctypes
import dataclasses
import hashlib
import logging
import os
import threading
from dataclasses import dataclass, field
from time import perf_counter

import numpy as np

from . import _lib
from .fragment_program import (FragmentProgram, JobTable, basis_reduce, build_jobs, compile_fragment,
                               dedup_labels)
from .knit_plan import LabelSpace, deposit_keys, factor_vgate
from .sweep_plan import K_SLOT, EncodedProgram, encode

_torch = None


def torch():
# ... 468 lines not shown
    T = torch()
    if dprog.module is None:
        raise ValueError("sweep_labels needs a compiled (SPLIT) program")
    dev = T.device("cuda", ctx.device)
    width = 1 << dprog.enc.m
    if q is None:
        q = T.empty((n_labels, width), dtype=T.float64, device=dev)
    if chunks is None:
        chunks = [(0, n_labels, 0, n_jobs, off_t)]
    need = ctypes.c_int64()
    ctx.check(ctx.lib.qk_sweep_workspace_bytes(ctypes.byref(dprog.struct), max(c[3] - c[2] for c in chunks),
                                               ctypes.byref(need)), "qk_sweep_workspace_bytes")
    if workspace is None or workspace.numel() < need.value:
        workspace = T.empty(max(need.value, 1), dtype=T.uint8, device=dev)
    slot_row = slot_t[0].numel() * 8 if (dprog.enc.n_slots and slot_t.dim() == 2) else 0
    for l0, l1, j0, j1, oc in chunks:
        ctx.check(ctx.lib.qk_sweep_compiled_labels(ctx.handle, dprog.module, ctypes.byref(dprog.struct), j1 - j0,
                                                   slot_t.data_ptr() + j0 * slot_row, sign_t.data_ptr() + 8 * j0,
                                                   l1 - l0, oc.data_ptr(), workspace.data_ptr(), need.value,
                                                   q.data_ptr() + 8 * width * l0), "qk_sweep_compiled_labels")
    return q, workspace


def reduce_labels(ctx: Context, pjob, off_t, n_labels: int, q=None):
    T = torch()
    width = pjob.shape[1]
    if q is None:
        q = T.empty((n_labels, width), dtype=T.float64, device=pjob.device)
    ctx.check(ctx.lib.qk_reduce_labels(ctx.handle, n_labels, off_t.data_ptr(), width,
                                       pjob.data_ptr(), q.data_ptr()), "qk_reduce_labels")
    return q


_SEED_STRIDE = 0x632BE59BD9B4E019
_U64 = (1 << 64) - 1


def fragment_seed(seed: int, index: int) -> int:
    return (int(seed) + index * _SEED_STRIDE) & _U64


def sample_fragment(ctx: Context, fs: "FragmentState", shots: int, seed: int, accuracy: float):
    T = torch()
    dev = T.device("cuda", ctx.device)
    L = len(fs.labels)
    if shots <= 0:
        raise ValueError("shots must be positive")
    if fs.dropped:
        return T.ones((L, 1), dtype=T.float64, device=dev)
    if fs.expand is not None:
        raise ValueError("basis-reduced fragments cannot be sampled (prepare with basis=False)")
    jobs = fs.jobs
    width = 1 << fs.prog.m
    slot_t, sign_t, off_t = jobs_to_device(jobs, ctx.device)
    pjob, _ = sweep_jobs(ctx, fs.dprog, slot_t, sign_t, jobs.n_jobs)
    pjob = fold_traced(ctx, pjob, fs.fold)
    cdf = T.empty_like(pjob)
    n_seg = len(jobs.label_offsets) - 1
    ctx.check(ctx.lib.qk_sample_cdf(ctx.handle, n_seg, off_t.data_ptr(), width, pjob.data_ptr(),
                                    cdf.data_ptr()), "qk_sample_cdf")
    seg = np.ascontiguousarray(fs.row_of_label(), dtype=np.int64)
    offs = jobs.label_offsets
    row_off = np.zeros(L + 1, dtype=np.int64)
    np.cumsum((offs[1:] - offs[:-1])[seg], out=row_off[1:])
    rows = np.concatenate([np.arange(offs[s], offs[s + 1]) for s in seg])
    seg_t = T.from_numpy(seg).to(dev)
    row_off_t = T.from_numpy(row_off).to(dev)
    row_sign_t = T.from_numpy(np.ascontiguousarray(jobs.sign[rows])).to(dev)
    counts = T.zeros((int(row_off[-1]), width), dtype=T.int32, device=dev)
    ctx.check(ctx.lib.qk_sample_counts(ctx.handle, L, 0, seg_t.data_ptr(), off_t.data_ptr(), row_off_t.data_ptr(),
                                       width, cdf.data_ptr(), int(shots), int(seed) & _U64, counts.data_ptr()),
              "qk_sample_counts")
    q = T.empty((L, width), dtype=T.float64, device=dev)
    ctx.check(ctx.lib.qk_fold_counts(ctx.handle, L, row_off_t.data_ptr(), width, row_sign_t.data_ptr(),
                                     counts.data_ptr(), int(shots), float(accuracy), q.data_ptr()), "qk_fold_counts")
    return q


def label_rows(fs: "FragmentState") -> "FragmentState":
    return dataclasses.replace(fs, uidx=None, unique_labels=None)


def gemm_keyed(ctx: Context, A, B, keyA=None, keyB=None, out=None, strideA: int = 0,
               strideB: int = 1, beta: int = 0, skip=None):
    K, M = A.shape
    K2, N = B.shape
    assert K == K2 and A.dtype == B.dtype and (A.stride(1) == 1 or M == 1) and (B.stride(1) == 1 or N == 1)
    lda, ldb = (A.stride(0) if K > 1 else M), (B.stride(0) if K > 1 else N)
    if keyA is not None:
        assert keyA.shape[0] == M and keyA.dtype == torch().int64
    if keyB is not None:
        assert keyB.shape[0] == N and keyB.dtype == torch().int64
    ctx.check(ctx.lib.qk_gemm_keyed_pred(ctx.handle, M, N, K, A.data_ptr(), lda, B.data_ptr(), ldb,
                                         _ptr(keyA), strideA, _ptr(keyB), strideB, out.data_ptr(), beta, _ptr(skip)),
              "qk_gemm_keyed_pred")
    return out


def gemm_outer_paired(ctx: Context, A, B, keyB, keyA=None, out=None, strideA: int = 0):
    K, M = A.shape
    K2, N = B.shape
    assert K == K2 and 1 <= K <= 8 and A.is_contiguous() and B.is_contiguous()
    assert keyB.shape[0] == N and keyB.dtype == torch().int64
    if keyA is not None:
        assert keyA.shape[0] == M and keyA.dtype == torch().int64
    ctx.check(ctx.lib.qk_gemm_outer_paired(ctx.handle, M, N, K, A.data_ptr(), M, B.data_ptr(), N,
                                           _ptr(keyA), strideA, keyB.data_ptr(), out.data_ptr()),
              "qk_gemm_outer_paired")
    return out


def knit_outer_stream(ctx: Context, A, B, clbits_a: list, clbits_b: list, nbits: int, out,
                      o_begin: int = 0, o_count: int | None = None, k_dev=None):
    K, M = A.shape
    K2, N = B.shape
    assert K == K2 and 1 <= K <= 8 and A.is_contiguous() and B.is_contiguous()
    mA, mB = sum(1 << c for c in clbits_a), sum(1 << c for c in clbits_b)
    if o_count is None:
        o_count = (1 << nbits) - o_begin
    assert M == 1 << len(clbits_a) and N == 1 << len(clbits_b) and out.numel() >= o_count
    if k_dev is not None:
        assert k_dev.dtype == torch().int32 and k_dev.device == out.device
    ctx.check(ctx.lib.qk_knit_outer_stream_range(ctx.handle, nbits, K, A.data_ptr(), M, B.data_ptr(), N, mA, mB,
                                                 o_begin, o_count, _ptr(k_dev), out.data_ptr()),
              "qk_knit_outer_stream_range")
    return out


OUTER_STREAM_KERNELS = ("qk_knit_outer_stream_kernel", "qk_knit_outer_blocked_kernel",
                        "qk_knit_outer_blocked_kernel<b_global>", "qk_knit_outer_rows_kernel")


def knit_outer_stream_kernel(K: int, clbits_a: list, clbits_b: list, nbits: int, o_begin: int = 0,
                             o_count: int | None = None) -> str:
    mA, mB = sum(1 << c for c in clbits_a), sum(1 << c for c in clbits_b)
    if o_count is None:
        o_count = (1 << nbits) - o_begin
    kind, tb = ctypes.c_int(), ctypes.c_int()
    _lib.check(None, _lib.lib().qk_knit_outer_stream_kind(nbits, K, mA, mB, o_begin, o_count, ctypes.byref(kind),
                                                          ctypes.byref(tb)), "qk_knit_outer_stream_kind")
    return OUTER_STREAM_KERNELS[kind.value]


def stream_knit_ok(clbits_a: list, clbits_b: list, nbits: int) -> bool:
    a, b = set(clbits_a), set(clbits_b)
    return (2 <= nbits <= 32 and not (a & b) and (a | b) == set(range(nbits)) and 0 in b
            and list(clbits_a) == sorted(a) and list(clbits_b) == sorted(b))


def paired_keys(clbits: list) -> bool:
    return len(clbits) >= 1 and sorted(clbits)[0] == 0


def khatri_rao(ctx: Context, A, B):
    T = torch()
    K, M = A.shape
    _, N = B.shape
    out = T.empty((K, M * N), dtype=T.float64, device=A.device)
    ctx.check(ctx.lib.qk_khatri_rao(ctx.handle, K, M, N, A.data_ptr(), M, B.data_ptr(), N,
                                    out.data_ptr()), "qk_khatri_rao")
    return out


def gather_rows(ctx: Context, src, idx_t, coef_t):
    T = torch()
    R = idx_t.shape[0]
    width = src.shape[1]
    out = T.empty((R, width), dtype=T.float64, device=src.device)
    ctx.check(ctx.lib.qk_gather_rows(ctx.handle, R, width, idx_t.data_ptr(), coef_t.data_ptr(),
                                     src.data_ptr(), out.data_ptr()), "qk_gather_rows")
    return out


def clbit_indexer(circuit):
    index = {}
    i = 0
    for creg in circuit.cregs:
        for b in creg:
            index[b] = i
            i += 1
    return lambda c: index[c]


@dataclass
class FragmentState:
    fragment: object
    labels: list
    prog: FragmentProgram
    dprog: DeviceProgram | None
    jobs: JobTable | None
    touches: list
    dropped: bool = False
    uidx: np.ndarray | None = None
    unique_labels: list | None = None
    basis_labels: list | None = None
    expand: np.ndarray | None = None
    fold: int = 1
    jit: tuple = (False, None, None)

    @property
    def swept_labels(self) -> list:
        if self.basis_labels is not None:
            return self.basis_labels
        return self.unique_labels if self.unique_labels is not None else self.labels

    @property
    def n_rows(self) -> int:
        return len(self.swept_labels)

# ... 852 lines not shown
```

hardwareawareoptimalquantumcircuitcuttingandknitting_amd/pipeline.py:

```python
from __future__ import annotations

import ctypes
import os
import threading
from time import perf_counter

import numpy as np

from . import _lib, engine
from .fragment_program import JobTable


_PROBES: dict = {}
_PROBES_LOCK = threading.Lock()


def _mm_nt(X, Y):
    L = X.shape[1]
    nb = L // 256 if L % 256 == 0 else 1
    if nb <= 1:
        return X @ Y.T
    Xb = X.view(X.shape[0], nb, 256).transpose(0, 1)
    Yb = Y.reshape(Y.shape[0], nb, 256).transpose(0, 1)
    return (Xb @ Yb.transpose(1, 2)).sum(0)
# ... 155 lines not shown
    def to_device(self, arr):
        return self.T.from_numpy(np.ascontiguousarray(arr)).to(self.dev)

    def sweep(self, fs, slot, sign, n_jobs, pjob, ws):
        engine.sweep_jobs(self.ctx, fs.dprog, slot, sign, n_jobs, pjob=pjob, workspace=ws)

    def sweep_rows(self, fs):
        return engine.sweep_fragment(self.ctx, fs)

    def fold_traced(self, q, fold):
        return engine.fold_traced(self.ctx, q, fold)

    def device_width(self, fs) -> int:
        return 1 << (fs.dprog.enc.m if fs.dprog is not None else fs.prog.m)

    def bind(self):
        self.ctx.bind_stream()

    def plan_multi(self, frags: list, sweeps: list):
        n = len(frags)
        vp = lambda xs: (ctypes.c_void_p * n)(*xs)
        i64 = lambda xs: (ctypes.c_int64 * n)(*xs)
        module = engine.compiled_multi_module(self.device, [fs.dprog.enc for fs in frags])
        outs = [(sw["q"] if sw["fused"] else sw["pjob"]) for sw in sweeps]
        maps = multi_block_maps([fs.dprog.enc for fs in frags], sweeps)
        self._maps = [None if m is None else self.to_device(m.view(np.int64)) for m in maps]
        rounds = len(maps)
        args = [module, (_lib.QkProgram * n)(*[fs.dprog.struct for fs in frags]), i64([sw["n_jobs"] for sw in sweeps]),
                vp([sw["slot"].data_ptr() for sw in sweeps]), vp([sw["sign"].data_ptr() for sw in sweeps]),
                i64([sw["n_local"] for sw in sweeps]),
                vp([sw["off"].data_ptr() if sw["fused"] else None for sw in sweeps]),
                vp([sw["ws"].data_ptr() for sw in sweeps]), i64([sw["ws"].numel() for sw in sweeps]),
                vp([o.data_ptr() for o in outs]),
                (ctypes.c_void_p * rounds)(*[None if m is None else m.data_ptr() for m in self._maps])]
        shared = [engine.init_prefixes(fs.dprog.enc, sw["jobs"]) if sw.get("jobs") is not None else None
                  for fs, sw in zip(frags, sweeps)]
        self.shared_init = [None if s is None else int(s[0].size) for s in shared]
        if any(s is not None for s in shared):
            self._shared = [None if s is None else (sw["slot"][self.to_device(s[0])].contiguous(),
                                                    self.to_device(s[1]))
                            for s, sw in zip(shared, sweeps)]
            args += [i64([0 if s is None else int(s[0].size) for s in shared]),
                     vp([None if s is None else s[0].data_ptr() for s in self._shared]),
                     vp([None if s is None else s[1].data_ptr() for s in self._shared])]
        return tuple(args)

    def sweep_multi(self, plan):
        module, progs, *rest = plan
        if len(rest) == 12:
            self.ctx.check(self.ctx.lib.qk_sweep_compiled_multi_shared(self.ctx.handle, module, len(progs), progs,
                                                                       *rest), "qk_sweep_compiled_multi_shared")
            return
        self.ctx.check(self.ctx.lib.qk_sweep_compiled_multi(self.ctx.handle, module, len(progs), progs, *rest),
                       "qk_sweep_compiled_multi")

    def fuses_labels(self, fs) -> bool:
        return fs.dprog is not None and fs.dprog.module is not None

    def sweep_labels(self, fs, slot, sign, n_jobs, off, n_labels, q, ws, chunks=None):
        engine.sweep_labels(self.ctx, fs.dprog, slot, sign, n_jobs, off, n_labels, q=q, workspace=ws, chunks=chunks)

    def reduce_labels(self, pjob, off, n_labels, q):
        return engine.reduce_labels(self.ctx, pjob, off, n_labels, q=q)

    def gather_rows(self, q, idx, coef):
        return engine.gather_rows(self.ctx, q, idx, coef)

    def gemm_keyed(self, A, B, **kw):
        return engine.gemm_keyed(self.ctx, A, B, **kw)

    def khatri_rao(self, A, B):
        return engine.khatri_rao(self.ctx, A, B)

    def gemm_outer_paired(self, A, B, keyB, **kw):
        return engine.gemm_outer_paired(self.ctx, A, B, keyB, **kw)

    def knit_outer_stream(self, A, B, clbits_a, clbits_b, nbits, out, o_begin=0, o_count=None, k_dev=None):
        return engine.knit_outer_stream(self.ctx, A, B, clbits_a, clbits_b, nbits, out, o_begin=o_begin,
                                        o_count=o_count, k_dev=k_dev)

    def outer_stream_kernel(self, K, clbits_a, clbits_b, nbits, o_begin=0, o_count=None):
        return engine.knit_outer_stream_kernel(K, clbits_a, clbits_b, nbits, o_begin, o_count)

    def rank_factors(self, GA, GB):
        return engine.rank_factors_device(self.ctx, GA, GB)

    def prep_operands(self, WtA, qA, WtB, qB, probes):
        return engine.prep_operands(self.ctx, WtA, qA, WtB, qB, probes)

    fuses_tally = True

    def probe_errors(self, XA, A2, U, B2, probes, r=None, tol=0.0, a2_cols=None, rel_tol=0.0, tally=None, vpart=None):
        return engine.probe_errors(self.ctx, XA, A2, U, B2, probes, r=r, tol=tol, a2_cols=a2_cols, rel_tol=rel_tol,
                                   tally=tally, vpart=vpart)

    def compress_v(self, TA, XA, TB, XB, probes, a_cols=None, a_width=None):
        if os.environ.get("QKNIT_COMPRESS_V", "1") == "0" or not engine.compress_probe_v_ok(XA, XB, a_cols):
            return None
        return engine.compress_probe_v(self.ctx, TA, XA, TB, XB, probes, a_cols=a_cols, a_width=a_width)

    def probe_accept(self, e2, r, tol, rel_tol=0.0):
        return engine.probe_accept(self.ctx, e2, r, tol, rel_tol)

    def rank_tally(self, r, k, acc):
        self.ctx.check(self.ctx.lib.qk_rank_tally(self.ctx.handle, r.data_ptr(), k.data_ptr(), acc.data_ptr()),
                       "qk_rank_tally")

    def compress(self, TA, XA, TB, XB, a_cols=None, a_width=None):
        return engine.compress_operands(self.ctx, TA, XA, TB, XB, a_cols=a_cols, a_width=a_width)

    def knit_select(self, A, B, clbits_a, clbits_b, nbits, accuracy, k_dev=None):
        return engine.knit_select(self.ctx, A, B, clbits_a, clbits_b, nbits, accuracy, k_dev=k_dev)

    def npd_pairs(self, keys, vals):
        return engine.npd_pairs(self.ctx, keys, vals)

    def qprep_grams(self, WtA, qA, WtB, qB, probes):
        return engine.qprep_grams(self.ctx, WtA, qA, WtB, qB, probes)

    def qprep_compress_check(self, WtA, qA, WtB, qB, TA, TB, U, probes, r, tol, rel_tol):
        return engine.qprep_compress_check(self.ctx, WtA, qA, WtB, qB, TA, TB, U, probes, r, tol, rel_tol)

    def select_above(self, dense, accuracy, key_base=0):
        return engine.select_above(self.ctx, dense, accuracy, key_base=key_base)

    def npd_dense(self, dense, accuracy):
        return engine.nearest_probability_distribution(self.ctx, dense, accuracy)

    def out_buffer(self, n: int, select: bool = True):
        return engine.out_buffer(self.ctx, n, select=select)

    def event(self):
        return self.T.cuda.Event(enable_timing=True)


class KnitPipeline:
    def __init__(self, virt, device: int = 0, factored: bool = False, rank: int = 0, world: int = 1,
                 mode: str | None = None, group=None, backend=None, chunk_jobs: int | None = None,
                 jit: bool | None = None, light_cone: bool = True, data_rank: bool | None = None):
        self.be = backend if backend is not None else HipBackend(device)
        self.chunk_jobs = int(os.environ.get("QKNIT_SWEEP_CHUNK_JOBS", "0")) if chunk_jobs is None else chunk_jobs
        self.fork = False
        self._multi = None
        self._streams = []
        self._sweep_graph = None
        self.T = engine.torch()
        self.virt = virt
        self.rank, self.world, self.group = rank, world, group
        factored = factored and engine.factored_ok(virt)
        self.factored = factored
        kw = {} if light_cone else {"relevance": False}
        if jit is not None:
            kw["jit"] = jit
        self.plan_ms = {}
        tick = perf_counter()
        with engine.host_planning():
            self.frags = self.be.prepare_fragments(virt, basis=factored, **kw)
            tick = self._phase("prepare_fragments", tick)
            self.ops = engine.knit_operands(virt, self.frags, factored, compress=light_cone)
            tick = self._phase("knit_operands", tick)
        self.N = virt.circuit.num_clbits
        q_bytes = sum(len(fs.labels) << fs.prog.m for fs in self.frags) * 8
        out_bytes = (1 << self.N) * 8
        self.order = engine.contract_order(self.ops.clbits)
        if mode is None:
            if world == 1:
                mode = "single"
            elif out_bytes <= q_bytes and not factored:
                mode = "reduce"
            else:
                mode = "slice" if self.slice_ok(world) else "gather"
        if mode == "reduce" and factored:
            raise ValueError("reduce mode needs the direct (label-sliced) knit")
        if mode not in ("single", "reduce", "gather", "slice"):
            raise ValueError(f"unknown mode {mode}")
        if mode == "slice" and not self.slice_ok(world):
            raise ValueError("slice mode needs a factored two-fragment knit whose fragments partition the output "
                             "bits, a power-of-two world and >= 2^9 outputs per rank")
        self.mode = mode
        two = len(self.frags) == 2 and not any(fs.dropped for fs in self.frags)
        ok = mode in ("single", "gather", "slice") and factored and two
        self.data_rank = (ok and virt.circuit.num_clbits >= 24) if data_rank is None else (data_rank and ok)
        self.rank_tol = 1e-14
        self.rank_tol_rel = 1e-12
        self.rank_fallbacks = 0
        self.rank_incompressible = 0
        self.last_rank = None
        cA, cB = self._stream_bits()
        self.dev_rank = bool(self.data_rank and cA is not None and self.ops.num_terms <= 64
                             and hasattr(self.be, "rank_factors"))
        self._pending = 0
        self._tally = None
        self._tally_read = np.zeros(4, dtype=np.int64)
        self.slice_sync = os.environ.get("QKNIT_SLICE_SYNC", "0") == "1"
        self.slice_exact = os.environ.get("QKNIT_SLICE_EXACT", "predicated")
        self.last_kernel = None
        self.last_prep = None
        self._probe = None
        self._pinned = None
        self._prep_stream = None
        self._write_stream = None
        self.overlap_cus = None
        self.overlap = os.environ.get("QKNIT_OVERLAP", "0") == "1"
        self.spec_write = os.environ.get("QKNIT_SPEC_WRITE", "0") == "1"
        self._spec_stream = None
        ob = os.environ.get("QKNIT_OUT_BUFFERS", "")
        self.out_buffers = int(ob) if ob else (3 if world >= 8 else 2 if world >= 2 else 1)
        self._outs = None
        self._wstreams = None
        self._flip = 0
        self._write_cus = None
        self.events = []
        self.sweep_events = []
        self.prep_events = []
        self.record_events = False
        self.row_jobs = ROW_JOBS
        self.row_prune = ROW_PRUNE
        self.out_alloc = None
        self.slice_prep = None
        self.slice_costs = None
        self._plan()

    def _phase(self, name: str, since: float) -> float:
        now = perf_counter()
        self.plan_ms[name] = self.plan_ms.get(name, 0.0) + (now - since) * 1e3
        return now

    def _stream_bits(self):
        live = [i for i, fs in enumerate(self.frags) if not fs.dropped]
        if len(live) != 2 or len(self.order) != 2:
            return None, None
        cA, cB = self.ops.clbits[self.order[0]], self.ops.clbits[self.order[-1]]
        return (cA, cB) if engine.stream_knit_ok(cA, cB, self.N) else (None, None)

    def slice_ok(self, world: int) -> bool:
        cA, cB = self._stream_bits()
        if cA is None or world < 1 or world & (world - 1) or not self.factored:
            return False
        return (1 << self.N) // world >= 512 and min(len(cA), len(cB)) >= world.bit_length() - 1

    def _plan(self):
        T, be = self.T, self.be
        self.sweeps = []
        self.row_src, self.n_rows, self.plan_jobs = [], [], []
        L = self.ops.num_terms
        self.term_range = _shard(L, self.rank, self.world) if self.mode == "reduce" else (0, L)
        self.place = {}
        tick = perf_counter()
        pruned = self._prune_rows()
        tick = self._phase("row_pruning", tick)
        swept = [self._swept_rows(i, fs, pruned.get(i)) for i, fs in enumerate(self.frags)]
        if self.mode == "slice":
            self.slice_prep, self.slice_costs = self._choose_slice_prep(swept)
        self.sharded = self.mode == "gather" or (self.mode == "slice" and self.slice_prep == "sharded")
        for i, fs in enumerate(self.frags):
            if fs.dropped:
                self.sweeps.append(None)
                self.row_src.append(None)
                self.n_rows.append(fs.n_rows)
                self.plan_jobs.append(0)
                continue
            src, jobs, nl = swept[i]
            self.row_src.append(src)
            self.n_rows.append(nl)
            self.plan_jobs.append(jobs.n_jobs)
            lo = 0
            if self.sharded:
                per = -(-nl // self.world)
                dealt = _deal_rows(jobs.label_jobs(), self.world)
                place = np.zeros(nl, dtype=np.int64)
                for r, rows_r in enumerate(dealt):
                    place[rows_r] = r * per + np.arange(len(rows_r))
                self.place[i] = place
                sub = jobs.take(dealt[self.rank])
            else:
                if self.mode == "reduce":
                    t0, t1 = self.term_range
                    rows = np.unique(self.ops.rows[i][t0:t1])
                    lo, hi = (int(rows.min()), int(rows.max()) + 1) if rows.size else (0, 0)
                else:
                    lo, hi = 0, nl
                sub = jobs.take(np.arange(lo, hi))
            n_local = len(sub.label_offsets) - 1
            slot_t, sign_t, off_t = be.upload_jobs(sub)
            n_jobs = sub.n_jobs
            width = self.be.device_width(fs) if hasattr(self.be, "device_width") else 1 << fs.prog.m
            need = be.workspace_bytes(fs, n_jobs) if n_jobs else 0
            sharded = self.sharded
# ... 228 lines not shown
            for s in self._streams:
                main.wait_stream(s)
            be.bind()
        for work in pending:
            work.wait()
        return qs

    def _fold(self, fs, q):
        return self.be.fold_traced(q, fs.fold) if getattr(fs, "fold", 1) > 1 else q

    def _sweep_fragment(self, fs, sw):
        be = self.be
        if sw["fused"]:
            be.sweep_labels(fs, sw["slot"], sw["sign"], sw["n_jobs"], sw["off"], sw["n_local"], sw["q"], sw["ws"],
                            chunks=sw["chunks"])
            return sw["q"]
        if sw["n_jobs"]:
            be.sweep(fs, sw["slot"], sw["sign"], sw["n_jobs"], sw["pjob"], sw["ws"])
        if sw["q"] is not None:
            return be.reduce_labels(sw["pjob"], sw["off"], sw["n_local"], sw["q"])
        return sw["pjob"]

    def capture_sweep(self):
        T = self.T
        if self.mode != "single":
            raise ValueError("sweep graphs are for single-GPU pipelines")
        self.fork = True
        self.sweep()
        T.cuda.synchronize()
        g = T.cuda.CUDAGraph()
        with T.cuda.graph(g):
            self.be.bind()
            qs = self.sweep()
        self.be.bind()
        self._sweep_graph, self._graph_qs = g, qs
        return qs

    def replay_sweep(self) -> list:
        self._sweep_graph.replay()
        return self._graph_qs

    def _exchange(self, i, qpad):
        import torch.distributed as dist

        kind, send, recv = self.xbuf[i]
        if kind == "a2a":
            P, per, bw = send.shape
            send.copy_(qpad[:per].view(per, P, bw).transpose(0, 1))
            work = dist.all_to_all_single(recv, send, group=self.group, async_op=True)
        else:
            per = recv.shape[0] // self.world
            work = dist.all_gather_into_tensor(recv, qpad[:per], group=self.group, async_op=True)
        return work, recv

    def operands(self, qs: list) -> list:
        T, be = self.T, self.be
        mats = []
        for i, q in enumerate(qs):
            q = q.contiguous()
            if self.transforms[i] is not None:
                W = self.transforms[i]
                a = be.empty((W.shape[1], q.shape[1]), T.float64)
                be.gemm_keyed(W, q, out=a, strideA=q.shape[1])
            else:
                a = be.gather_rows(q, self.gather_idx[i], self.gather_coef[i])
            mats.append(a)
        return mats

    N_PROBES = 16
    RANK_GIVE_UP = 3

    def _probes(self, n: int, device):
        if self._probe is None or self._probe.shape[1] != n:
            key = (n, str(device))
            with _PROBES_LOCK:
                hit = _PROBES.get(key)
                if hit is None:
                    T = self.T
                    g = T.Generator().manual_seed(1234)
                    hit = _PROBES[key] = T.randn((self.N_PROBES, n), generator=g, dtype=T.float64).to(device)
            self._probe = hit
        return self._probe

    def _prep_step(self, qs) -> dict:
        return self._prep_slice(qs) if self.mode == "slice" and self.sharded else self._prep_dev_rank(qs)

    def _launch_step(self, p: dict):
        return self._launch_slice(p) if self.mode == "slice" else self._launch_dev_rank(p)

    def knit(self, qs: list):
        if self.dev_rank and self.mode in ("single", "slice"):
            p = self._prep_step(qs)
            if self.out is None:
                self.out = self._alloc_out(None)
            return self._launch_step(p)
        mats = self.operands(qs)
        if self.out is None:
            self.out = self._alloc_out(mats)
        if self.mode == "slice":
            ia, ib = self.order[0], self.order[-1]
            return self._slice_exact(mats[ia], mats[ib], self.ops.clbits[ia], self.ops.clbits[ib])
        low = self._rank_compress(mats) if self.data_rank else None
        if self.record_events:
            start, end = self.be.event(), self.be.event()
            start.record()
        if low is not None:
            res = self._contract_lowrank(low[0])
        elif self.mode == "single" and len(self.order) == 2 and mats[self.order[0]].shape[0] <= 8:
            res = self._contract_lowrank(mats)
        else:
            res = self._contract(mats)
        if self.record_events:
            end.record()
            self.events.append((start, end))
        if low is not None and not float(low[1]) <= max(self.rank_tol, self.rank_tol_rel * low[2]):
            self._rank_rejects = getattr(self, "_rank_rejects", 0) + 1
            if self._rank_rejects >= self.RANK_GIVE_UP:
                self.data_rank = False
            self.rank_fallbacks += 1
            self.last_rank = None
            res = self._contract(mats)
        elif low is not None:
            self._rank_rejects = 0
        if self.mode == "reduce":
            import torch.distributed as dist

            dist.reduce(res, dst=0, group=self.group)
        return res

    def _fused_prep(self, qs) -> bool:
        ia, ib = self.order[0], self.order[-1]
        if not hasattr(self.be, "prep_operands") or self.transforms[ia] is None or self.transforms[ib] is None:
            return False
        K = self.transforms[ia].shape[1]
        return (self.transforms[ib].shape[1] == K and self.transforms[ia].shape[0] == qs[ia].shape[0]
                and self.transforms[ib].shape[0] == qs[ib].shape[0]
                and engine.prep_ok(K, qs[ia].shape[1], qs[ib].shape[1]))

    def _qspace_prep(self, qs) -> bool:
        ia, ib = self.order[0], self.order[-1]
        if self.spec_write or not hasattr(self.be, "qprep_grams") or self.transforms[ia] is None \
                or self.transforms[ib] is None:
            return False
        WA, WB = self.transforms[ia], self.transforms[ib]
        return (WA.shape[1] == WB.shape[1] and WA.shape[0] == qs[ia].shape[0] and WB.shape[0] == qs[ib].shape[0]
                and engine.qprep_ok(WA.shape[1], WA.shape[0], WB.shape[0], qs[ia].shape[1], qs[ib].shape[1]))

    def _prep_fused(self, qs, probes):
        ia, ib = self.order[0], self.order[-1]
        qa = qs[ia] if qs[ia].stride(1) == 1 else qs[ia].contiguous()
        qb = qs[ib] if qs[ib].stride(1) == 1 else qs[ib].contiguous()
        XA, XB, G, U = self.be.prep_operands(self.transforms[ia], qa, self.transforms[ib], qb, probes)
        mats = [None] * len(qs)
        mats[ia], mats[ib] = XA, XB
        self.last_prep = "fused"
        return mats, G, U

    def _accept(self, A, B, A2, B2, x, r, ref_rows=None, cmp_rows=None, reduce_err=None, note=True):
        T = self.T
        if ref_rows is None:
            ref_rows = A.T @ _mm_nt(B, x)
            cmp_rows = A2.T @ _mm_nt(B2, x)
        e2 = T.cat([((ref_rows - cmp_rows) ** 2).sum(dim=0), (ref_rows ** 2).sum(dim=0)])
        if reduce_err is not None:
            e2 = reduce_err(e2)
        n = e2.numel() // 2
        err = e2[:n].max().sqrt()
        bound = T.clamp(self.rank_tol_rel * e2[n:].max().sqrt(), min=self.rank_tol)
        k_eff = T.where((err <= bound) & (r > 0), r, T.zeros_like(r))
        if note:
            self._note_rank(r, k_eff)
        return k_eff, err

    def _prep_dev_rank(self, qs) -> dict:
        ia, ib = self.order[0], self.order[-1]
        if self._qspace_prep(qs):
            T = self.T
            x = self._probes(qs[ib].shape[1], qs[ib].device)
            WA, WB = self.transforms[ia], self.transforms[ib]
            qA, qB = qs[ia].contiguous(), qs[ib].contiguous()
            G, U = self.be.qprep_grams(WA, qA, WB, qB, x)
            TA, TB, r = self.be.rank_factors(G[0], G[1])
            A2, B2, k_eff, _ = self.be.qprep_compress_check(WA, qA, WB, qB, TA, TB, U, x, r, self.rank_tol,
                                                            self.rank_tol_rel)
            self._note_rank(r, k_eff)
            mats = [None] * len(qs)
            for i, W, q in ((ia, WA, qA), (ib, WB, qB)):
                mats[i] = T.empty((W.shape[1], q.shape[1]), dtype=T.float64, device=q.device)
                self.be.gemm_keyed(W, q, out=mats[i], strideA=q.shape[1], skip=k_eff)
            self.last_prep = "qspace"
            return {"A2": A2, "B2": B2, "k_eff": k_eff, "mats": mats}
        if self._fused_prep(qs):
            x = self._probes(qs[ib].shape[1], qs[ib].device)
            mats, G, U = self._prep_fused(qs, x)
            TA, TB, r = self.be.rank_factors(G[0], G[1])
            if not self.spec_write:
                return self._compress_and_check(TA, TB, r, mats, U, x)
            A2, B2 = self.be.compress(TA, mats[ia], TB, mats[ib])
            if self.spec_write and getattr(self.be, "dev", None) is not None and self.be.dev.type == "cuda":
                T = self.T
                main = T.cuda.current_stream()
                if self._spec_stream is None:
                    self._spec_stream = T.cuda.Stream(device=self.be.dev)
                S2 = self._spec_stream
                S2.wait_stream(main)
                with T.cuda.stream(S2):
                    self.be.bind()
                    _, k_eff, _ = self.be.probe_errors(mats[ia], A2, U, B2, x, r=r, tol=self.rank_tol,
                                                       rel_tol=self.rank_tol_rel)
                    self._note_rank(r, k_eff)
                self.be.bind()
                for t in (mats[ia], A2, U, B2, x, r, k_eff):
                    t.record_stream(S2)
                return {"A2": A2, "B2": B2, "k_eff": k_eff, "k_write": r, "check": S2, "mats": mats}
            if getattr(self.be, "fuses_tally", False):
                _, k_eff, _ = self.be.probe_errors(mats[ia], A2, U, B2, x, r=r, tol=self.rank_tol,
                                                   rel_tol=self.rank_tol_rel, tally=self._tally_for(r.device))
                self._pending += 1
            else:
                _, k_eff, _ = self.be.probe_errors(mats[ia], A2, U, B2, x, r=r, tol=self.rank_tol,
                                                   rel_tol=self.rank_tol_rel)
                self._note_rank(r, k_eff)
            return {"A2": A2, "B2": B2, "k_eff": k_eff, "mats": mats}
        mats = self.operands(qs)
        self.last_prep = "torch"
        A, B = mats[ia], mats[ib]
        G = self.T.stack([_mm_nt(A, A), _mm_nt(B, B)])
        TA, TB, r = self.be.rank_factors(G[0].contiguous(), G[1].contiguous())
        A2, B2 = (TA @ A).contiguous(), (TB @ B).contiguous()
        k_eff, _ = self._accept(A, B, A2, B2, self._probes(B.shape[1], B.device), r)
        return {"A2": A2, "B2": B2, "k_eff": k_eff, "mats": mats}

    def _compress_and_check(self, TA, TB, r, mats, U, x) -> dict:
        ia, ib = self.order[0], self.order[-1]
        a_cols = self._replicated_a_cols()
        kw = {"a_cols": a_cols} if a_cols is not None else {}
        cv = self.be.compress_v(TA, mats[ia], TB, mats[ib], x, **kw) if hasattr(self.be, "compress_v") else None
        check = {}
        if cv is not None:
            A2, B2, check["vpart"] = cv
        else:
            A2, B2 = self.be.compress(TA, mats[ia], TB, mats[ib], **kw)
        XA = mats[ia]
        if a_cols is not None:
            XA = XA[:, a_cols[0]:a_cols[0] + a_cols[1]]
            check["a2_cols"] = a_cols
        tally = getattr(self.be, "fuses_tally", False)
        if tally:
            check["tally"] = self._tally_for(r.device)
        _, k_eff, _ = self.be.probe_errors(XA, A2, U, B2, x, r=r, tol=self.rank_tol, rel_tol=self.rank_tol_rel,
                                           **check)
        if tally:
            self._pending += 1
        else:
            self._note_rank(r, k_eff)
        return {"A2": A2, "B2": B2, "k_eff": k_eff, "mats": mats}

    def _kernel_name(self, K, cA, cB, o_begin=0, o_count=None):
        name = getattr(self.be, "outer_stream_kernel", None)
        return name(K, cA, cB, self.N, o_begin, o_count) if name else type(self.be).__name__

    def _launch_dev_rank(self, p: dict):
        ia, ib = self.order[0], self.order[-1]
        cA, cB = self.ops.clbits[ia], self.ops.clbits[ib]
        if self.record_events:
            start, end = self.be.event(), self.be.event()
            start.record()
        self.last_kernel = self._kernel_name(p["A2"].shape[0], cA, cB)
        self.be.knit_outer_stream(p["A2"], p["B2"], cA, cB, self.N, self.out, k_dev=p.get("k_write", p["k_eff"]))
        if self.record_events:
            end.record()
            self.events.append((start, end))
        if "check" in p:
            self.T.cuda.current_stream().wait_stream(p["check"])
        return self._contract(p["mats"], skip=p["k_eff"])

    def _prep_slice(self, qs) -> dict:
        import torch.distributed as dist

        T, be, P = self.T, self.be, self.world
        ia, ib = self.order[0], self.order[-1]
        bwA, bwB = qs[ia].shape[1], qs[ib].shape[1]
        x_full = self._probes(bwB * P, qs[ib].device)
        if getattr(self, "_x_local", None) is None or self._x_local.shape[1] != bwB:
            self._x_local = x_full[:, self.rank * bwB:(self.rank + 1) * bwB].contiguous()
        x = self._x_local
        npr = self.N_PROBES
        if self._fused_prep(qs):
            mats, G, U = self._prep_fused(qs, x)
            XA, XB = mats[ia], mats[ib]
            K = XA.shape[0]
            red = _joined(T, G, U)
            dist.all_reduce(red, group=self.group)
            G = red[:2 * K * K].view(2, K, K)
            U = red[2 * K * K:].view(K, npr).contiguous()
            TA, TB, r = be.rank_factors(G[0].contiguous(), G[1].contiguous())
            R8 = TA.shape[0]
            if self.slice_sync:
                fac = T.cat([TA.reshape(-1), TB.reshape(-1), r.to(T.float64)])
                dist.broadcast(fac, src=self._group_rank0(), group=self.group)
                TA = fac[:R8 * K].view(R8, K)
                TB = fac[R8 * K:2 * R8 * K].view(R8, K)
                r = fac[-1:].to(T.int32)
            A2l, B2l = be.compress(TA.contiguous(), XA, TB.contiguous(), XB)
            loc = _joined(T, A2l, B2l)
        else:
            mats = self.operands(qs)
            self.last_prep = "torch"
            XA, XB = mats[ia], mats[ib]
            K = XA.shape[0]
            red = T.cat([_mm_nt(XA, XA).reshape(-1), _mm_nt(XB, XB).reshape(-1), _mm_nt(XB, x).reshape(-1)])
            dist.all_reduce(red, group=self.group)
            GA = red[:K * K].view(K, K).contiguous()
            GB = red[K * K:2 * K * K].view(K, K).contiguous()
            Bx = red[2 * K * K:].view(K, npr)
            TA, TB, r = be.rank_factors(GA, GB)
            R8 = TA.shape[0]
            fac = T.cat([TA.reshape(-1), TB.reshape(-1), r.to(T.float64)])
            dist.broadcast(fac, src=self._group_rank0(), group=self.group)
            TA = fac[:R8 * K].view(R8, K)
            TB = fac[R8 * K:2 * R8 * K].view(R8, K)
            r = fac[-1:].to(T.int32)
            loc = T.cat([(TA @ XA).reshape(-1), (TB @ XB).reshape(-1)])
        gat = T.empty(P * loc.numel(), dtype=loc.dtype, device=loc.device)
        dist.all_gather_into_tensor(gat, loc, group=self.group)
        gat = gat.view(P, loc.numel())
        A2 = gat[:, :R8 * bwA].view(P, R8, bwA).permute(1, 0, 2).reshape(R8, P * bwA).contiguous()
        B2 = gat[:, R8 * bwA:].view(P, R8, bwB).permute(1, 0, 2).reshape(R8, P * bwB).contiguous()
        if self._fused_prep(qs):
            _, k_eff, _ = be.probe_errors(XA, A2, U, B2, x_full.contiguous(), r=r, tol=self.rank_tol,
                                          a2_cols=(self.rank * bwA, bwA), rel_tol=self.rank_tol_rel)
        else:
            ref_rows = XA.T @ Bx
            cmp_rows = A2[:, self.rank * bwA:(self.rank + 1) * bwA].T @ _mm_nt(B2, x_full)
            k_eff, _ = self._accept(None, None, None, None, None, r, ref_rows, cmp_rows, note=False)
        dist.all_reduce(k_eff, op=dist.ReduceOp.MIN, group=self.group)
        self._note_rank(r, k_eff)
        if self.slice_exact == "host":
            on_gpu = k_eff.device.type == "cuda"
            pinned = T.empty(1, dtype=T.int32, pin_memory=on_gpu)
            pinned.copy_(k_eff, non_blocking=on_gpu)
            ready = T.cuda.Event() if on_gpu else None
            if on_gpu:
                ready.record()
            return {"A2": A2, "B2": B2, "k_eff": k_eff, "XA": XA, "XB": XB, "pinned": pinned, "ready": ready,
                    "mats": mats}
        ex = self._slice_exact_operands(XA, XB, async_op=True)
        return {"A2": A2, "B2": B2, "k_eff": k_eff, "exact": ex, "mats": mats}

    def _launch_slice(self, p: dict):
        be = self.be
        ia, ib = self.order[0], self.order[-1]
        cA, cB = self.ops.clbits[ia], self.ops.clbits[ib]
        o_begin, o_count = self.slice
        if self.record_events:
# ... 318 lines not shown
            st = engine._affine_stride(cA)
            kA = None if st is not None else engine._device_keys(tuple(cA), None, None, A.device)
            kB = engine._device_keys(tuple(cB), None, None, B.device)
            self.last_kernel = "qk_gemm_smallk_kernel<true>"
            return self.be.gemm_outer_paired(A, B, kB, keyA=kA, strideA=st or 0, out=self.out)
        self.last_kernel = None
        pad = (-r) % 16
        if pad:
            A = T.cat([A, A.new_zeros((pad, A.shape[1]))])
            B = T.cat([B, B.new_zeros((pad, B.shape[1]))])
        out = list(mats)
        out[ia], out[ib] = A, B
        return self._contract(out)


    def _alloc_out(self, mats):
        if self.mode == "slice":
            n = self.slice[1]
        elif self.mode != "gather":
            n = 1 << self.N
        else:
            lo, hi = self.row_block
            n = max(hi - lo, 1) * mats[self.order[-1]].shape[1]
        return self.new_out(n, zero=self.mode == "gather" or not self.covers_outputs())

    def new_out(self, n: int, zero: bool = False, select: bool = True):
        alloc = getattr(self.be, "out_buffer", None)
        if alloc is None:
            self.out_alloc = "backend"
            self._last_owner = None
            return self.be.zeros((n,), self.T.float64) if zero else self.be.empty((n,), self.T.float64)
        n_sel = len(engine.out_selections)
        out, owner = alloc(n) if select else alloc(n, select=False)
        self.out_alloc = "qk_out_alloc (1-GiB mapped chunks)" if owner is not None else "torch"
        if len(engine.out_selections) > n_sel:
            last = engine.out_selections[-1]
            self.out_alloc += f" ({last[0]})" if owner is None else f", write-rate selected: {last} GB/s"
        if owner is not None:
            st = engine.out_stats()
            self.out_alloc += (f"; process: {st['reserved']} reservations ({st['reserve_failed']} failed), "
                               f"{st['live']} live, {st['retired']} retired "
                               f"({st['retired_bytes'] / 2**30:.0f} GiB of address space)")
        self._last_owner = owner
        if zero:
            out.zero_()
        return out

    def take_out(self, defer_select: bool = False):
        n = self.slice[1] if self.mode == "slice" else 1 << self.N
        zero = not self.covers_outputs()
        own = getattr(self, "_call_owner", None)
        if own is not None and own.n == n and not own.in_use():
            if getattr(own, "write_gbs", None) is None or own.write_gbs >= engine.OUT_FAST_GBS:
                out = own.tensor()
                if zero:
                    out.zero_()
                return out
            self._call_owner = own = None
            select = True
        else:
            select = own is not None or not defer_select
        out = self.new_out(n, zero=zero, select=select)
        self._call_owner = self._last_owner
        if self._call_owner is not None and not select:
            self._call_owner.write_gbs = None
            self._time_call_write = True
        return out

    def note_call_write(self, events_before: int):
        if not getattr(self, "_time_call_write", False):
            return
        self._time_call_write = False
        own = getattr(self, "_call_owner", None)
        ev = self.events[events_before:]
        if own is None or not ev:
            return
        ms = ev[-1][0].elapsed_time(ev[-1][1])
        M, N, _ = self.gemm_shape()
        own.write_gbs = 8.0 * M * N / (ms * 1e-3) / 1e9 if ms > 0 else float("inf")
        if own.write_gbs < engine.OUT_FAST_GBS:
            engine.out_selections.append([f"drop-in first call: un-timed mapping wrote at {own.write_gbs:.1f} GB/s, "
                                          "replaced on the next call"])

    def _contract(self, mats, skip=None):
        if self.mode != "gather":
            gemm = self.be.gemm_keyed if skip is None else (lambda A, B, **kw: self.be.gemm_keyed(A, B, skip=skip, **kw))
            return engine.contract(None, mats, self.ops.clbits, self.out, gemm=gemm, kr=self.be.khatri_rao)
        order = self.order
        A = mats[order[0]]
        for i in order[1:-1]:
            A = self.be.khatri_rao(A.contiguous(), mats[i].contiguous())
        B = mats[order[-1]]
        lo, hi = self.row_block
        if not self.split_a:
            A = A[:, lo:hi]
        A = A.contiguous()
        return self.be.gemm_keyed(A, B.contiguous(), keyA=None, strideA=B.shape[1], keyB=None, strideB=1,
                                  out=self.out)

    def plan_bytes(self) -> int:
        seen, total = set(), 0
        for sw in self.sweeps:
            if sw is None:
                continue
            for k in ("slot", "sign", "off", "pjob", "q", "ws"):
                t = sw.get(k)
                if t is not None and hasattr(t, "data_ptr") and t.data_ptr() not in seen:
                    seen.add(t.data_ptr())
                    total += t.numel() * t.element_size()
        for W in self.transforms:
            if W is not None:
                total += W.numel() * W.element_size()
        return total

    def covers_outputs(self) -> bool:
        bits = set()
        for i, fs in enumerate(self.frags):
            if not fs.dropped:
                bits |= set(self.ops.clbits[i])
        return self.mode in ("single", "slice") and bits == set(range(self.N))

    def run_into(self, out):
        self.out = out
        try:
            self.step()
        finally:
            self.out = None
        return out

    def _select_pair(self):
        live = [i for i, fs in enumerate(self.frags) if not fs.dropped]
        if self.mode != "single" or len(live) != 2 or len(self.order) != 2 or not hasattr(self.be, "knit_select"):
            return None
        ia, ib = self.order[0], self.order[-1]
        cA, cB = list(self.ops.clbits[ia]), list(self.ops.clbits[ib])
        if cA != sorted(cA) or cB != sorted(cB) or set(cA) & set(cB):
            return None
        return ia, ib

    def knit_dict(self, accuracy: float, qs=None):
        if qs is None:
            qs = self.sweep()
        if self.mode == "slice":
            return self._knit_dict_slice(accuracy, qs)
        pair = self._select_pair()
        if pair is not None and self.dev_rank:
            p = self._prep_dev_rank(qs)
            ia, ib = pair
            keys, vals = self.be.knit_select(p["A2"], p["B2"], self.ops.clbits[ia], self.ops.clbits[ib], self.N,
                                             accuracy, k_dev=p["k_eff"])
            self.last_kernel = "qk_knit_select_kernel"
            if int(p["k_eff"].reshape(-1)[0]) > 0:
                return self.be.npd_pairs(keys, vals)
            mats = p["mats"]
        else:
            mats = self.operands(qs)
            if pair is not None and mats[pair[0]].shape[0] <= 8:
                ia, ib = pair
                keys, vals = self.be.knit_select(mats[ia].contiguous(), mats[ib].contiguous(), self.ops.clbits[ia],
                                                 self.ops.clbits[ib], self.N, accuracy)
                self.last_kernel = "qk_knit_select_kernel"
                return self.be.npd_pairs(keys, vals)
        keep = self.out
        self.out = self.be.zeros((1 << self.N,), self.T.float64)
        try:
            dense = self._contract(mats)
            self.last_kernel = None
            return self.be.npd_dense(dense, accuracy)
        finally:
# ... 133 lines not shown
```

include/qknit.h:

```cpp
#ifndef QKNIT_H
#define QKNIT_H

#include <stdint.h>

#ifdef __cplusplus
extern "C" {
#endif

#define QK_OK 0
#define QK_EARG 1
#define QK_EHIP 2
#define QK_ESTATE 3

#define QK_TILE_BITS 12
#define QK_FIBER_BITS 4

enum { QK_U1 = 0, QK_D1 = 1, QK_SLOT = 2, QK_U2 = 3, QK_D2 = 4, QK_CX = 5, QK_SWAP = 6, QK_SCALE = 7,
       QK_U1R = 8, QK_U1X = 9, QK_D1R = 10, QK_D2R = 11, QK_SCALER = 12 };

typedef struct qk_op {
    int32_t kind;
    int32_t a, b;
    int32_t e1, e2;
    int32_t slot;
// ... 22 lines not shown
    int32_t packed;
    int32_t n_passes;
    const qk_pass* passes;
    const qk_op* ops;
    const qk_group* groups;
    const double* mats;
} qk_program;

typedef struct qk_ctx qk_ctx;

int qk_ctx_create(int device, qk_ctx** out);
int qk_ctx_destroy(qk_ctx* ctx);
int qk_ctx_set_stream(qk_ctx* ctx, void* hip_stream);
int qk_ctx_synchronize(qk_ctx* ctx);
const char* qk_last_error(qk_ctx* ctx);

int qk_stream_create_cu_masked(int device, const uint32_t* cu_mask, int mask_words, void** stream);
int qk_stream_destroy(void* stream);
int qk_stream_cu_count(int device, void* stream, int* cus);
const char* qk_version(void);

int qk_out_alloc(qk_ctx* ctx, int64_t bytes, void** ptr);
int qk_out_free(qk_ctx* ctx, void* ptr);
int qk_out_mapped_bytes(const void* ptr, int64_t* bytes);
int qk_out_write_rate(qk_ctx* ctx, void* ptr, int64_t bytes, double* gbs);
int qk_out_stats(int64_t* out, int n);

int qk_sweep_workspace_bytes(const qk_program* prog, int64_t n_jobs, int64_t* bytes);

int qk_sweep(qk_ctx* ctx, const qk_program* prog, int64_t n_jobs, const double* job_slots,
             const double* job_sign, void* workspace, int64_t workspace_bytes, double* pjob);

typedef struct qk_module qk_module;

int qk_module_compile(qk_ctx* ctx, const char* source, const char* const* names, int n_names,
                      qk_module** out);
int qk_module_destroy(qk_module* module);
int qk_module_load(qk_ctx* ctx, const void* image, int64_t image_bytes, const char* const* names, int n_names,
                   qk_module** out);
int qk_module_code(const qk_module* module, void* buf, int64_t* bytes);

int qk_sweep_compiled(qk_ctx* ctx, const qk_module* module, const qk_program* prog, int64_t n_jobs,
                      const double* job_slots, const double* job_sign, void* workspace,
                      int64_t workspace_bytes, double* pjob);

int qk_sweep_compiled_labels(qk_ctx* ctx, const qk_module* module, const qk_program* prog, int64_t n_jobs,
                             const double* job_slots, const double* job_sign, int64_t n_labels,
                             const int64_t* label_offsets, void* workspace, int64_t workspace_bytes, double* q);

int qk_sweep_compiled_multi(qk_ctx* ctx, const qk_module* module, int n_prog, const qk_program* progs,
                            const int64_t* n_jobs, const double* const* job_slots, const double* const* job_sign,
                            const int64_t* n_labels, const int64_t* const* label_offsets, void* const* workspaces,
                            const int64_t* workspace_bytes, double* const* outs, const uint64_t* const* block_maps);

int qk_sweep_compiled_multi_shared(qk_ctx* ctx, const qk_module* module, int n_prog, const qk_program* progs,
                                   const int64_t* n_jobs, const double* const* job_slots,
                                   const double* const* job_sign, const int64_t* n_labels,
                                   const int64_t* const* label_offsets, void* const* workspaces,
                                   const int64_t* workspace_bytes, double* const* outs,
                                   const uint64_t* const* block_maps, const int64_t* n_init,
                                   const double* const* init_slots, const int32_t* const* prefix_of);

int qk_reduce_labels(qk_ctx* ctx, int64_t n_labels, const int64_t* offsets, int64_t width,
                     const double* pjob, double* q);

int qk_gemm_keyed(qk_ctx* ctx, int64_t M, int64_t N, int64_t K, const double* A, int64_t lda,
                  const double* B, int64_t ldb, const int64_t* keyA, int64_t strideA,
                  const int64_t* keyB, int64_t strideB, double* out, int beta);

int qk_gemm_keyed_pred(qk_ctx* ctx, int64_t M, int64_t N, int64_t K, const double* A, int64_t lda,
                       const double* B, int64_t ldb, const int64_t* keyA, int64_t strideA,
                       const int64_t* keyB, int64_t strideB, double* out, int beta, const int32_t* skip);

int qk_gemm_outer_paired(qk_ctx* ctx, int64_t M, int64_t N, int64_t K, const double* A, int64_t lda,
                         const double* B, int64_t ldb, const int64_t* keyA, int64_t strideA,
                         const int64_t* keyB, double* out);

int qk_knit_outer_stream(qk_ctx* ctx, int nbits, int64_t K, const double* A, int64_t lda, const double* B,
                         int64_t ldb, uint64_t maskA, uint64_t maskB, double* out);

int qk_knit_outer_stream_range(qk_ctx* ctx, int nbits, int64_t K, const double* A, int64_t lda, const double* B,
                               int64_t ldb, uint64_t maskA, uint64_t maskB, int64_t o_begin, int64_t o_count,
                               const int32_t* k_dev, double* out);

int qk_knit_outer_stream_kind(int nbits, int64_t K, uint64_t maskA, uint64_t maskB, int64_t o_begin,
                              int64_t o_count, int* kind, int* task_bits);
int qk_khatri_rao(qk_ctx* ctx, int64_t K, int64_t M, int64_t N, const double* A, int64_t lda,
                  const double* B, int64_t ldb, double* out);

int qk_gather_rows(qk_ctx* ctx, int64_t R, int64_t width, const int64_t* idx, const double* coef,
                   const double* src, double* dst);

typedef struct qk_knit_plan {
    int32_t n_frag;
    int32_t nbits;
    int64_t terms;
    const int64_t* rows;
    const uint64_t* clbit_masks;
    const double* const* transforms;
} qk_knit_plan;

int qk_knit_workspace_bytes(const qk_knit_plan* plan, int64_t* bytes);
int qk_knit(qk_ctx* ctx, const qk_knit_plan* plan, const double* const* q, void* workspace, int64_t workspace_bytes,
            double* out);

typedef struct qk_lowrank_plan {
    int32_t nbits;
    int32_t terms;
    int64_t rows_a, rows_b;
    uint64_t mask_a, mask_b;
    const double* wt_a;
    const double* wt_b;
    const double* probes;
    double lam_tol, s_tol, s_abs;
    double rank_tol;
    double rank_tol_rel;
} qk_lowrank_plan;

int qk_knit_lowrank_workspace_bytes(qk_ctx* ctx, const qk_lowrank_plan* plan, int64_t* bytes);
int qk_knit_lowrank(qk_ctx* ctx, const qk_lowrank_plan* plan, const double* q_a, const double* q_b, void* workspace,
                    int64_t workspace_bytes, double* out, int32_t* rank_out);

#define QK_COMM_ID_BYTES 128
typedef struct qk_comm qk_comm;
int qk_comm_unique_id(uint8_t* id);
int qk_comm_init(qk_ctx* ctx, const uint8_t* id, int nranks, int rank, qk_comm** out);
int qk_comm_destroy(qk_comm* comm);
int qk_comm_size(qk_comm* comm, int* nranks, int* rank);
int qk_allreduce(qk_ctx* ctx, qk_comm* comm, const double* send, double* recv, int64_t count);
int qk_reduce(qk_ctx* ctx, qk_comm* comm, const double* send, double* recv, int64_t count, int root);
int qk_allgather(qk_ctx* ctx, qk_comm* comm, const double* send, double* recv, int64_t count);
int qk_alltoall(qk_ctx* ctx, qk_comm* comm, const double* send, double* recv, int64_t count);

int qk_rank_factors(qk_ctx* ctx, int64_t K, const double* GA, const double* GB, double lam_tol, double s_tol,
                    double s_abs, int rmax, double* TA, double* TB, int32_t* r_out);

int qk_prep_workspace_bytes(qk_ctx* ctx, int64_t NA, int64_t NB, int64_t* bytes);
int qk_prep_operands(qk_ctx* ctx, int K, int RA, const double* WtA, const double* qA, int64_t ldqA, int64_t NA,
                     double* XA, int RB, const double* WtB, const double* qB, int64_t ldqB, int64_t NB, double* XB,
                     const double* probes, double* GA, double* GB, double* U, double* work, int64_t work_bytes);

int qk_qprep_workspace_bytes(qk_ctx* ctx, int64_t NA, int64_t NB, int64_t* bytes);
int qk_qprep_grams(qk_ctx* ctx, int K, int RA, const double* WtA, const double* qA, int64_t ldqA, int64_t NA, int RB,
                   const double* WtB, const double* qB, int64_t ldqB, int64_t NB, const double* probes, double* GA,
                   double* GB, double* U, double* work, int64_t work_bytes);
int qk_qprep_compress_check(qk_ctx* ctx, int K, int rmax, int RA, const double* WtA, const double* qA, int64_t ldqA,
                            int64_t NA, int RB, const double* WtB, const double* qB, int64_t ldqB, int64_t NB,
                            const double* TA, const double* TB, const double* U, const double* probes, double* A2,
                            double* B2, double* e2, const int32_t* r_dev, double tol, double rel_tol, int32_t* k_out,
                            double* err_out, double* work, int64_t work_bytes);

int qk_compress_operands(qk_ctx* ctx, int K, int rmax, const double* TA, const double* XA, int64_t NA, double* A2,
                         const double* TB, const double* XB, int64_t NB, double* B2);
int qk_compress_operands_ld(qk_ctx* ctx, int K, int rmax, const double* TA, const double* XA, int64_t NA, int64_t ldxa,
                            double* A2, int64_t lda2, const double* TB, const double* XB, int64_t NB, int64_t ldxb,
                            double* B2, int64_t ldb2);

int qk_compress_probe_v(qk_ctx* ctx, int K, int rmax, const double* TA, const double* XA, int64_t NA, int64_t ldxa,
                        double* A2, int64_t lda2, const double* TB, const double* XB, int64_t NB, int64_t ldxb,
                        double* B2, int64_t ldb2, const double* probes, int64_t ldp, double* vpart,
                        int64_t vpart_doubles);

int qk_probe_errors_vpart(qk_ctx* ctx, int K, int rmax, const double* XA, int64_t ldx, int64_t NA, const double* A2,
                          int64_t lda2, const double* U, const double* vpart, int64_t gv, double* e2,
                          const int32_t* r_dev, double tol, double rel_tol, int32_t* k_out, double* err_out,
                          double* work, int64_t work_bytes, int64_t* tally);
// ... 61 lines not shown
```

Before: 515,200.

## Fuse low-rank probe check into outer-stream knit and accept into predicated GEMM

Adds a CHECK variant of the blocked outer-stream knit kernel. Its first n_check blocks compute the low-rank probe residual partials (MFMA f64) before doing their knit work. The predicated keyed GEMM can now fold those partials, make the accept/reject decision in-kernel and write k/err/tally, which replaces the separate check launch and its stream wait. This removes kernel launches and synchronisation from the single-mode step. In exchange the knit kernel must speculatively write at full rank r, and every GEMM block redundantly reduces the partials before deciding to skip.

```diff
diff --git a/hardwareawareoptimalquantumcircuitcuttingandknitting_amd/_lib.py b/hardwareawareoptimalquantumcircuitcuttingandknitting_amd/_lib.py
--- a/hardwareawareoptimalquantumcircuitcuttingandknitting_amd/_lib.py
+++ b/hardwareawareoptimalquantumcircuitcuttingandknitting_amd/_lib.py
@@ -77,6 +77,13 @@
                                           ctypes.POINTER(ctypes.c_int), ctypes.POINTER(ctypes.c_int)]),
     "qk_knit_outer_stream_range": (c_i32, [c_vp, ctypes.c_int, c_i64, c_vp, c_i64, c_vp, c_i64, ctypes.c_uint64,
                                            ctypes.c_uint64, c_i64, c_i64, c_vp, c_vp]),
+    "qk_knit_outer_stream_range_check": (c_i32, [c_vp, ctypes.c_int, c_i64, c_vp, c_i64, c_vp, c_i64, ctypes.c_uint64,
+                                                 ctypes.c_uint64, c_i64, c_i64, c_vp, c_vp, ctypes.c_int, ctypes.c_int,
+                                                 c_vp, c_i64, c_i64, c_vp, c_i64, c_vp, c_vp, c_i64, c_vp,
+                                                 ctypes.c_int]),
+    "qk_gemm_keyed_pred_accept": (c_i32, [c_vp, c_i64, c_i64, c_i64, c_vp, c_i64, c_vp, c_i64, c_vp, c_i64,
+                                          c_vp, c_i64, c_vp, ctypes.c_int, c_vp, ctypes.c_int, c_vp, ctypes.c_double,
+                                          ctypes.c_double, c_vp, c_vp, c_vp, c_vp]),
     "qk_rank_factors": (c_i32, [c_vp, c_i64, c_vp, c_vp, ctypes.c_double, ctypes.c_double, ctypes.c_double,
                                 ctypes.c_int, c_vp, c_vp, c_vp]),
     "qk_prep_workspace_bytes": (c_i32, [c_vp, c_i64, c_i64, ctypes.POINTER(c_i64)]),
diff --git a/hardwareawareoptimalquantumcircuitcuttingandknitting_amd/build.py b/hardwareawareoptimalquantumcircuitcuttingandknitting_amd/build.py
--- a/hardwareawareoptimalquantumcircuitcuttingandknitting_amd/build.py
+++ b/hardwareawareoptimalquantumcircuitcuttingandknitting_amd/build.py
@@ -11,7 +11,7 @@
                                                               "qknit_select.hip", "qknit_comm.hip",
                                                               "qknit_mem.hip", "qknit_trunc.hip",
                                                               "qknit_prim.hip")]
-DEPS = SRCS + [os.path.join(HERE, "csrc", h) for h in ("internal.h", "sweep_ops.h", "prim.h")]
+DEPS = SRCS + [os.path.join(HERE, "csrc", h) for h in ("internal.h", "sweep_ops.h", "prim.h", "probe_check.h")]
 HEADER = os.path.join(os.path.dirname(HERE), "include", "qknit.h")
 OUT = os.path.join(HERE, "libqknit.so")
 ARCH = os.environ.get("QKNIT_ARCH", "gfx950")
diff --git a/hardwareawareoptimalquantumcircuitcuttingandknitting_amd/csrc/probe_check.h b/hardwareawareoptimalquantumcircuitcuttingandknitting_amd/csrc/probe_check.h
--- /dev/null
+++ b/hardwareawareoptimalquantumcircuitcuttingandknitting_amd/csrc/probe_check.h
@@ -0,0 +1,182 @@
+#ifndef QKNIT_PROBE_CHECK_H
+#define QKNIT_PROBE_CHECK_H
+
+#include <hip/hip_runtime.h>
+
+#include <cstdint>
+
+namespace qk_check {
+
+typedef double d4_t __attribute__((ext_vector_type(4)));
+
+constexpr int CK = 64;
+constexpr int CNP = 16;
+constexpr int CV_PART = 8 * 16;
+constexpr int CE = 2 * CNP;
+constexpr int D_LDS = CK * CNP + 16 * CNP + 4 * CE + CV_PART;
+constexpr int ACCEPT_LDS = 256;
+
+struct CheckArgs {
+    int K = 0, rmax = 0;
+    const double* XA = nullptr;
+    int64_t ldx = 0, NA = 0;
+    const double* A2 = nullptr;
+    int64_t lda2 = 0;
+    const double* U = nullptr;
+    const double* vpart = nullptr;
+    int gv = 0;
+    double* epart = nullptr;
+    int n_check = 0;
+};
+
+struct AcceptArgs {
+    const double* epart = nullptr;
+    int n = 0;
+    const int32_t* r_dev = nullptr;
+    double tol = 0.0, rel_tol = 0.0;
+    int32_t* k_out = nullptr;
+    double* err_out = nullptr;
+    double* e2_out = nullptr;
+    int64_t* tally = nullptr;
+};
+
+template <int VF = 16, int KB = CK / 4>
+__device__ __forceinline__ void probe_d_block(double* __restrict__ lds, int K, int rmax,
+                                              const double* __restrict__ XA, int64_t ldx, int64_t NA,
+                                              const double* __restrict__ A2, int64_t lda2,
+                                              const double* __restrict__ U, const double* __restrict__ vpart, int gv,
+                                              double* __restrict__ epart, int wg, int nwg) {
+    double (*Us)[CNP] = reinterpret_cast<double (*)[CNP]>(lds);
+    double (*Vs)[CNP] = reinterpret_cast<double (*)[CNP]>(lds + CK * CNP);
+    double (*ep)[CE] = reinterpret_cast<double (*)[CE]>(lds + CK * CNP + 16 * CNP);
+    double* vh = lds + CK * CNP + 16 * CNP + 4 * CE;
+    const int tid = threadIdx.x, lane = tid & 63, wave = tid >> 6, l16 = lane & 15, l4 = lane >> 4;
+    if ((int64_t)wg * 64 >= NA) {
+        if (tid < CE) epart[(int64_t)wg * CE + tid] = 0.0;
+        return;
+    }
+    {
+        const int e = tid & (CV_PART - 1), h = tid >> 7;
+        double t[16];
+#pragma unroll
+        for (int u = 0; u < 16; ++u) t[u] = 0.0;
+        int b = h;
+        for (; b + 30 < gv; b += 32) {
+#pragma unroll
+            for (int u0 = 0; u0 < 16; u0 += VF) {
+                double v[VF];
+#pragma unroll
+                for (int u = 0; u < VF; ++u) v[u] = vpart[(int64_t)(b + 2 * (u0 + u)) * CV_PART + e];
+#pragma unroll
+                for (int u = 0; u < VF; ++u) t[u0 + u] += v[u];
+            }
+        }
+        for (; b < gv; b += 2) t[0] += vpart[(int64_t)b * CV_PART + e];
+#pragma unroll
+        for (int w = 8; w >= 1; w >>= 1)
+#pragma unroll
+            for (int u = 0; u < w; ++u) t[u] += t[u + w];
+        if (h == 1) vh[e] = t[0];
+        __syncthreads();
+        if (h == 0) Vs[e / 16][e % 16] = -(t[0] + vh[e]);
+        else Vs[8 + e / 16][e % 16] = 0.0;
+    }
+    for (int e = tid; e < CK * CNP; e += 256) Us[e / CNP][e % CNP] = (e / CNP) < K ? U[e] : 0.0;
+    __syncthreads();
+    double e2 = 0.0, f2 = 0.0;
+    for (int64_t cb = (int64_t)wg * 4 + wave; cb * 16 < NA; cb += (int64_t)nwg * 4) {
+        const int64_t c = cb * 16 + l16;
+        int lr = l4;
+        if (KB < CK / 4) asm volatile("" : "+v"(lr));
+        double a2[2];
+#pragma unroll
+        for (int jj = 0; jj < 2; ++jj) a2[jj] = A2[(int64_t)min(4 * jj + lr, rmax - 1) * lda2 + c];
+        d4_t acc = {0, 0, 0, 0};
+#pragma unroll
+        for (int k0 = 0; k0 < CK / 4; k0 += KB) {
+            double av[KB];
+#pragma unroll
+            for (int kk = 0; kk < KB; ++kk) av[kk] = XA[(int64_t)min(4 * (k0 + kk) + lr, K - 1) * ldx + c];
+#pragma unroll
+            for (int kk = 0; kk < KB; ++kk)
+                acc = __builtin_amdgcn_mfma_f64_16x16x4f64(av[kk], Us[4 * (k0 + kk) + l4][l16], acc, 0, 0, 0);
+            if (KB < CK / 4) __builtin_amdgcn_sched_barrier(0);
+        }
+#pragma unroll
+        for (int rr = 0; rr < 4; ++rr) f2 = fma(acc[rr], acc[rr], f2);
+#pragma unroll
+        for (int jj = 0; jj < 2; ++jj)
+            acc = __builtin_amdgcn_mfma_f64_16x16x4f64(a2[jj], Vs[4 * jj + l4][l16], acc, 0, 0, 0);
+#pragma unroll
+        for (int rr = 0; rr < 4; ++rr) e2 = fma(acc[rr], acc[rr], e2);
+    }
+    e2 += __shfl_xor(e2, 16, 64);
+    e2 += __shfl_xor(e2, 32, 64);
+    f2 += __shfl_xor(f2, 16, 64);
+    f2 += __shfl_xor(f2, 32, 64);
+    if (l4 == 0) {
+        ep[wave][l16] = e2;
+        ep[wave][CNP + l16] = f2;
+    }
+    __syncthreads();
+    if (tid < CE) epart[(int64_t)wg * CE + tid] = ep[0][tid] + ep[1][tid] + ep[2][tid] + ep[3][tid];
+}
+
+__device__ __forceinline__ int probe_accept_fold(double* __restrict__ acc, const double* __restrict__ epart, int n,
+                                                 const int32_t* __restrict__ r_dev, double tol, double rel_tol,
+                                                 double* __restrict__ e2_out, int32_t* __restrict__ k_out,
+                                                 double* __restrict__ err_out, int64_t* __restrict__ tally,
+                                                 bool writer) {
+    const int tid = threadIdx.x, p = tid % CE;
+    constexpr int STEP = 256 / CE;
+    double s8[8] = {0, 0, 0, 0, 0, 0, 0, 0};
+    int b = tid / CE;
+    for (; b + 31 * STEP < n; b += 32 * STEP) {
+        double v[32];
+#pragma unroll
+        for (int u = 0; u < 32; ++u) v[u] = epart[(int64_t)(b + u * STEP) * CE + p];
+#pragma unroll
+        for (int u = 0; u < 32; ++u) s8[u & 7] += v[u];
+    }
+    for (; b < n; b += 8 * STEP) {
+        double v[8];
+#pragma unroll
+        for (int u = 0; u < 8; ++u) v[u] = epart[(int64_t)min(b + u * STEP, n - 1) * CE + p];
+#pragma unroll
+        for (int u = 0; u < 8; ++u)
+            if (b + u * STEP < n) s8[0] += v[u];
+    }
+    const double s = ((s8[0] + s8[1]) + (s8[2] + s8[3])) + ((s8[4] + s8[5]) + (s8[6] + s8[7]));
+    acc[tid] = s;
+    __syncthreads();
+    for (int w = 128; w >= CE; w >>= 1) {
+        if (tid < w) acc[tid] += acc[tid + w];
+        __syncthreads();
+    }
+    if (writer && tid < CE && e2_out) e2_out[tid] = acc[tid];
+    if (!r_dev) return 0;
+    double m = 0.0, f = 0.0;
+    for (int q = 0; q < CNP; ++q) {
+        m = fmax(m, acc[q]);
+        f = fmax(f, acc[CNP + q]);
+    }
+    const double err = sqrt(m);
+    const double bound = fmax(tol, rel_tol * sqrt(f));
+    const int r = *r_dev;
+    const int k = (r > 0 && err <= bound) ? r : 0;
+    if (writer && tid == 0 && k_out) {
+        if (err_out) *err_out = err;
+        *k_out = k;
+        if (tally) {
+            tally[0] += r == 0 ? 1 : 0;
+            tally[1] += (r > 0 && k == 0) ? 1 : 0;
+            tally[2] = k;
+            tally[3] += 1;
+        }
+    }
+    return k;
+}
+
+}
+
+#endif
diff --git a/hardwareawareoptimalquantumcircuitcuttingandknitting_amd/csrc/qknit.hip b/hardwareawareoptimalquantumcircuitcuttingandknitting_amd/csrc/qknit.hip
--- a/hardwareawareoptimalquantumcircuitcuttingandknitting_amd/csrc/qknit.hip
+++ b/hardwareawareoptimalquantumcircuitcuttingandknitting_amd/csrc/qknit.hip
@@ -8,6 +8,7 @@
 #include <string>
 
 #include "internal.h"
+#include "probe_check.h"
 #include "sweep_ops.h"
 
 namespace {
@@ -496,9 +497,19 @@
     int beta;
     int64_t tiles_m, tiles_n;
     const int32_t* skip = nullptr;
+    qk_check::AcceptArgs acc;
 };
 
-__device__ __forceinline__ bool gemm_skipped(const GemmArgs& g) { return g.skip && *g.skip > 0; }
+__device__ __forceinline__ bool gemm_skipped(const GemmArgs& g, double* lds) {
+    if (g.acc.epart) {
+        const int k = qk_check::probe_accept_fold(lds, g.acc.epart, g.acc.n, g.acc.r_dev, g.acc.tol, g.acc.rel_tol,
+                                                  g.acc.e2_out, g.acc.k_out, g.acc.err_out, g.acc.tally,
+                                                  blockIdx.x == 0 && blockIdx.y == 0);
+        __syncthreads();
+        return k > 0;
+    }
+    return g.skip && *g.skip > 0;
+}
 
 __device__ __forceinline__ void gemm_tile_coords(int64_t seq, int64_t tiles_m, int64_t tiles_n,
                                                  int64_t& bm, int64_t& bn) {
@@ -661,7 +672,7 @@
 __global__ __launch_bounds__(256, 2) void qk_gemm_keyed_kernel(GemmArgs g) {
     __shared__ __attribute__((aligned(16))) double As[2][GK][GT + GPAD];
     __shared__ __attribute__((aligned(16))) double Bs[2][GK][GT + GPAD];
-    if (gemm_skipped(g)) return;
+    if (gemm_skipped(g, &As[0][0][0])) return;
     const int64_t nblk = g.tiles_m * g.tiles_n;
     int buf = 0;
     int64_t bm, bn;
@@ -739,7 +750,7 @@
 
 __global__ __launch_bounds__(256, 2) void qk_gemm_glds_kernel(GemmArgs g) {
     __shared__ __attribute__((aligned(16))) GemmRing ring[G2S];
-    if (gemm_skipped(g)) return;
+    if (gemm_skipped(g, &ring[0].a[0][0])) return;
     const int lane = threadIdx.x & 63, wave = threadIdx.x >> 6;
     const int wm = wave & 1, wn = wave >> 1;
     const int64_t nblk = g.tiles_m * g.tiles_n;
@@ -859,7 +870,7 @@
 template <int NKS>
 __global__ __launch_bounds__(256, 2) void qk_gemm_wave_kernel(GemmArgs g) {
     __shared__ __attribute__((aligned(16))) WaveRing rings[4];
-    if (gemm_skipped(g)) return;
+    if (gemm_skipped(g, &rings[0].a[0][0][0])) return;
     const int lane = threadIdx.x & 63, wave = threadIdx.x >> 6;
     const int wm = wave & 1, wn = wave >> 1;
     WaveRing& ring = rings[__builtin_amdgcn_readfirstlane(wave)];
@@ -1020,7 +1031,8 @@
 
 template <bool KEYED>
 __global__ __launch_bounds__(256) void qk_gemm_smallk_kernel(GemmArgs g) {
-    if (gemm_skipped(g)) return;
+    __shared__ double pred_lds[qk_check::ACCEPT_LDS];
+    if (gemm_skipped(g, pred_lds)) return;
     const int K = (int)g.K;
     for (int64_t row = blockIdx.x; row < g.M; row += gridDim.x) {
         double a[SK_MAX];
@@ -1171,10 +1183,18 @@
     const int32_t* kdev;
     double* __restrict__ out;
     int64_t spread;
+    qk_check::CheckArgs chk;
 };
 
-template <bool BG>
-__global__ __launch_bounds__(256) void qk_knit_outer_blocked_kernel(OuterBlockedArgs a) {
+template <bool BG, bool CHECK>
+__device__ __forceinline__ void outer_blocked_body(const OuterBlockedArgs& a) {
+    extern __shared__ double stage[];
+    if (CHECK && (int)blockIdx.x < a.chk.n_check) {
+        const qk_check::CheckArgs& c = a.chk;
+        qk_check::probe_d_block<8, 8>(stage, c.K, c.rmax, c.XA, c.ldx, c.NA, c.A2, c.lda2, c.U, c.vpart, c.gv, c.epart,
+                                (int)blockIdx.x, c.n_check);
+        __syncthreads();
+    }
     int K = a.K;
     if (a.kdev) {
         const int kd = *a.kdev;
@@ -1182,7 +1202,6 @@
         K = kd < K ? kd : K;
     }
     __shared__ uint32_t tab[2][2][256];
-    extern __shared__ double stage[];
     const uint32_t low = (1u << a.TB) - 1u;
     const uint32_t mAl = a.maskA & low, mBl = a.maskB & low;
     const int na = 1 << __builtin_popcount(mAl), nb = 1 << __builtin_popcount(mBl);
@@ -1235,6 +1254,16 @@
 #endif
         }
     }
+}
+
+template <bool BG, bool CHECK = false>
+__global__ __launch_bounds__(256) void qk_knit_outer_blocked_kernel(OuterBlockedArgs a) {
+    outer_blocked_body<BG, false>(a);
+}
+
+template <>
+__global__ __launch_bounds__(256, 5) void qk_knit_outer_blocked_kernel<false, true>(OuterBlockedArgs a) {
+    outer_blocked_body<false, true>(a);
 }
 
 struct OuterRowsArgs {
@@ -1531,6 +1560,11 @@
     return QK_OK;
 }
 
+static int gemm_keyed_launch(qk_ctx* ctx, int64_t M, int64_t N, int64_t K, const double* A, int64_t lda,
+                             const double* B, int64_t ldb, const int64_t* keyA, int64_t strideA,
+                             const int64_t* keyB, int64_t strideB, double* out, int beta, const int32_t* skip,
+                             const qk_check::AcceptArgs& acc);
+
 int qk_gemm_keyed(qk_ctx* ctx, int64_t M, int64_t N, int64_t K, const double* A, int64_t lda,
                   const double* B, int64_t ldb, const int64_t* keyA, int64_t strideA,
                   const int64_t* keyB, int64_t strideB, double* out, int beta) {
@@ -1540,6 +1574,37 @@
 int qk_gemm_keyed_pred(qk_ctx* ctx, int64_t M, int64_t N, int64_t K, const double* A, int64_t lda,
                        const double* B, int64_t ldb, const int64_t* keyA, int64_t strideA,
                        const int64_t* keyB, int64_t strideB, double* out, int beta, const int32_t* skip) {
+    return gemm_keyed_launch(ctx, M, N, K, A, lda, B, ldb, keyA, strideA, keyB, strideB, out, beta, skip,
+                             qk_check::AcceptArgs{});
+}
+
+int qk_gemm_keyed_pred_accept(qk_ctx* ctx, int64_t M, int64_t N, int64_t K, const double* A, int64_t lda,
+                              const double* B, int64_t ldb, const int64_t* keyA, int64_t strideA,
+                              const int64_t* keyB, int64_t strideB, double* out, int beta, const double* epart,
+                              int n, const int32_t* r_dev, double tol, double rel_tol, int32_t* k_out,
+                              double* err_out, double* e2_out, int64_t* tally) {
+    if (!ctx) return QK_EARG;
+    if (!epart || n < 1 || !r_dev || !k_out)
+        return fail(ctx, QK_EARG, "qk_gemm_keyed_pred_accept: need epart, n >= 1, r_dev and k_out%s");
+    if (M < 1 || N < 1)
+        return fail(ctx, QK_EARG, "qk_gemm_keyed_pred_accept: empty contraction%s");
+    qk_check::AcceptArgs acc;
+    acc.epart = epart;
+    acc.n = n;
+    acc.r_dev = r_dev;
+    acc.tol = tol;
+    acc.rel_tol = rel_tol;
+    acc.k_out = k_out;
+    acc.err_out = err_out;
+    acc.e2_out = e2_out;
+    acc.tally = tally;
+    return gemm_keyed_launch(ctx, M, N, K, A, lda, B, ldb, keyA, strideA, keyB, strideB, out, beta, nullptr, acc);
+}
+
+static int gemm_keyed_launch(qk_ctx* ctx, int64_t M, int64_t N, int64_t K, const double* A, int64_t lda,
+                             const double* B, int64_t ldb, const int64_t* keyA, int64_t strideA,
+                             const int64_t* keyB, int64_t strideB, double* out, int beta, const int32_t* skip,
+                             const qk_check::AcceptArgs& acc) {
     if (!ctx) return QK_EARG;
     if (M < 0 || N < 0 || K < 0) return fail(ctx, QK_EARG, "qk_gemm_keyed: negative size%s");
     if (M == 0 || N == 0) return QK_OK;
@@ -1550,6 +1615,7 @@
     QK_HIP(ctx, hipSetDevice(ctx->device));
     if (nblk >= (int64_t(1) << 31)) return fail(ctx, QK_EARG, "qk_gemm_keyed: too many tiles%s");
     GemmArgs g{M, N, K, A, lda, B, ldb, keyA, strideA, keyB, strideB, out, beta, tm, tn, skip};
+    g.acc = acc;
     const bool aligned16 = ((reinterpret_cast<uintptr_t>(A) | reinterpret_cast<uintptr_t>(B)) & 15) == 0 &&
                            (lda % 2) == 0 && (ldb % 2) == 0;
     if (K >= 1 && K <= SK_MAX && !beta && !keyB && strideB == 1 && N % 2 == 0 && aligned16 &&
@@ -1617,6 +1683,10 @@
     return QK_OK;
 }
 
+static int outer_stream_range_launch(qk_ctx* ctx, int nbits, int64_t K, const double* A, int64_t lda, const double* B,
+                                     int64_t ldb, uint64_t maskA, uint64_t maskB, int64_t o_begin, int64_t o_count,
+                                     const int32_t* k_dev, double* out, const qk_check::CheckArgs* chk);
+
 int qk_knit_outer_stream(qk_ctx* ctx, int nbits, int64_t K, const double* A, int64_t lda, const double* B,
                          int64_t ldb, uint64_t maskA, uint64_t maskB, double* out) {
     if (!ctx) return QK_EARG;
@@ -1628,6 +1698,47 @@
 int qk_knit_outer_stream_range(qk_ctx* ctx, int nbits, int64_t K, const double* A, int64_t lda, const double* B,
                                int64_t ldb, uint64_t maskA, uint64_t maskB, int64_t o_begin, int64_t o_count,
                                const int32_t* k_dev, double* out) {
+    return outer_stream_range_launch(ctx, nbits, K, A, lda, B, ldb, maskA, maskB, o_begin, o_count, k_dev, out,
+                                     nullptr);
+}
+
+int qk_knit_outer_stream_range_check(qk_ctx* ctx, int nbits, int64_t K, const double* A, int64_t lda, const double* B,
+                                     int64_t ldb, uint64_t maskA, uint64_t maskB, int64_t o_begin, int64_t o_count,
+                                     const int32_t* k_dev, double* out, int Kx, int rmax, const double* XA,
+                                     int64_t ldx, int64_t NA, const double* A2, int64_t lda2, const double* U,
+                                     const double* vpart, int64_t gv, double* epart, int n_check) {
+    if (!ctx) return QK_EARG;
+    if (n_check == 0 && !epart)
+        return outer_stream_range_launch(ctx, nbits, K, A, lda, B, ldb, maskA, maskB, o_begin, o_count, k_dev, out,
+                                         nullptr);
+    if (Kx < 1 || Kx > qk_check::CK || rmax < 1 || rmax > 8 || NA < 16 || NA % 16 || gv < 1 || gv > INT32_MAX ||
+        n_check < 1 || n_check > 1024)
+        return fail(ctx, QK_EARG,
+                    "qk_knit_outer_stream_range_check: need 1 <= Kx <= 64, 1 <= rmax <= 8, NA a multiple of 16, gv >= 1, "
+                    "1 <= n_check <= 1024%s");
+    if (!XA || !A2 || !U || !vpart || !epart)
+        return fail(ctx, QK_EARG, "qk_knit_outer_stream_range_check: null check buffer%s");
+    if (ldx < NA || lda2 < NA) return fail(ctx, QK_EARG, "qk_knit_outer_stream_range_check: leading dimension%s");
+    if (o_count <= 0) return fail(ctx, QK_EARG, "qk_knit_outer_stream_range_check: empty output range%s");
+    qk_check::CheckArgs c;
+    c.K = Kx;
+    c.rmax = rmax;
+    c.XA = XA;
+    c.ldx = ldx;
+    c.NA = NA;
+    c.A2 = A2;
+    c.lda2 = lda2;
+    c.U = U;
+    c.vpart = vpart;
+    c.gv = (int)gv;
+    c.epart = epart;
+    c.n_check = n_check;
+    return outer_stream_range_launch(ctx, nbits, K, A, lda, B, ldb, maskA, maskB, o_begin, o_count, k_dev, out, &c);
+}
+
+static int outer_stream_range_launch(qk_ctx* ctx, int nbits, int64_t K, const double* A, int64_t lda, const double* B,
+                                     int64_t ldb, uint64_t maskA, uint64_t maskB, int64_t o_begin, int64_t o_count,
+                                     const int32_t* k_dev, double* out, const qk_check::CheckArgs* chk) {
     if (!ctx) return QK_EARG;
     if (nbits < 2 || nbits > 32 || K < 1 || K > SK_MAX)
         return fail(ctx, QK_EARG, "qk_knit_outer_stream: need 2 <= nbits <= 32, 1 <= K <= 8%s");
@@ -1644,6 +1755,13 @@
     QK_HIP(ctx, hipSetDevice(ctx->device));
     const int cus = ctx->cus;
     const int align = __builtin_ctzll((uint64_t)(o_begin | o_count));
+    if (chk) {
+        int kind = 0, tbk = 0;
+        if (qk_knit_outer_stream_kind(nbits, K, maskA, maskB, o_begin, o_count, &kind, &tbk) != QK_OK || kind != 1)
+            return fail(ctx, QK_EARG,
+                        "qk_knit_outer_stream_range_check: the check rides only in the blocked kernel with both "
+                        "operands staged (qk_knit_outer_stream_kind 1)%s");
+    }
     if (const int rc = outer_rows_bits(K, maskB, align)) {
         const int64_t pieces = o_count >> rc;
         const int64_t nb = int64_t(1) << (__builtin_popcountll(maskB) - rc);
@@ -1685,7 +1803,17 @@
         if (spread < 1 || tasks % spread) spread = 1;
         OuterBlockedArgs b{(int)K, tb, A, lda, B, ldb, (uint32_t)maskA, (uint32_t)maskB, o_begin >> tb,
                            (o_begin >> tb) + tasks, o_begin, k_dev, out, spread};
-        const dim3 grid((unsigned)(tasks < G0 ? tasks : G0));
+        const int64_t G = tasks < G0 ? tasks : G0;
+        if (chk) {
+            b.chk = *chk;
+            const size_t lds = qk_check::D_LDS * sizeof(double);
+            const dim3 cgrid((unsigned)(G < chk->n_check ? chk->n_check : G));
+            hipLaunchKernelGGL((qk_knit_outer_blocked_kernel<false, true>), cgrid, dim3(256),
+                               stage < lds ? lds : stage, ctx->stream, b);
+            QK_HIP(ctx, hipGetLastError());
+            return QK_OK;
+        }
+        const dim3 grid((unsigned)G);
         if (bg)
             hipLaunchKernelGGL(qk_knit_outer_blocked_kernel<true>, grid, dim3(256), stage, ctx->stream, b);
         else
diff --git a/hardwareawareoptimalquantumcircuitcuttingandknitting_amd/csrc/qknit_plan.hip b/hardwareawareoptimalquantumcircuitcuttingandknitting_amd/csrc/qknit_plan.hip
--- a/hardwareawareoptimalquantumcircuitcuttingandknitting_amd/csrc/qknit_plan.hip
+++ b/hardwareawareoptimalquantumcircuitcuttingandknitting_amd/csrc/qknit_plan.hip
@@ -194,7 +194,7 @@
 constexpr int LR_PROBES = 16;
 
 struct LowrankLayout {
-    int64_t xa, xb, g, u, prep, ta, tb, r, a2, b2, e2, k, err, probe, ka, kb, total;
+    int64_t xa, xb, g, u, prep, ta, tb, r, a2, b2, e2, k, err, probe, ka, kb, vpart, epart, total;
     int64_t prep_bytes, probe_bytes;
     bool qspace;
 };
@@ -255,6 +255,8 @@
     L.probe = take(probe);
     L.ka = contiguous_bits(p->mask_a) ? -1 : take(NA * 8);
     L.kb = contiguous_bits(p->mask_b) ? -1 : take(NB * 8);
+    L.vpart = take(((NB + 511) / 512) * 128 * 8);
+    L.epart = take((int64_t)QK_N_CHECK * 32 * 8);
     L.total = off;
     L.prep_bytes = prep;
     L.probe_bytes = probe;
@@ -294,6 +296,10 @@
     double *XA = D(L.xa), *XB = D(L.xb), *G = D(L.g), *U = D(L.u);
     int32_t* r = reinterpret_cast<int32_t*>(ws + L.r);
     int32_t* k = reinterpret_cast<int32_t*>(ws + L.k);
+    int kind = 0, task_bits = 0;
+    const bool fused = !L.qspace && (reinterpret_cast<uintptr_t>(workspace) & 15) == 0 &&
+                       qk_knit_outer_stream_kind(p->nbits, LR_RMAX, p->mask_a, p->mask_b, 0, int64_t(1) << p->nbits,
+                                                 &kind, &task_bits) == QK_OK && kind == 1;
     if (L.qspace) {
         const int RA = (int)p->rows_a, RB = (int)p->rows_b;
         rc = qk_qprep_grams(ctx, K, RA, p->wt_a, q_a, NA, NA, RB, p->wt_b, q_b, NB, NB, p->probes, G, G + K * K, U,
@@ -309,12 +315,20 @@
         rc = qk_prep_operands(ctx, K, (int)p->rows_a, p->wt_a, q_a, NA, NA, XA, (int)p->rows_b, p->wt_b, q_b, NB, NB,
                               XB, p->probes, G, G + K * K, U, D(L.prep), L.prep_bytes);
         if (!rc) rc = qk_rank_factors(ctx, K, G, G + K * K, p->lam_tol, p->s_tol, p->s_abs, LR_RMAX, D(L.ta), D(L.tb), r);
-        if (!rc) rc = qk_compress_operands(ctx, K, LR_RMAX, D(L.ta), XA, NA, D(L.a2), D(L.tb), XB, NB, D(L.b2));
-        if (!rc)
+        if (!rc && fused)
+            rc = qk_compress_probe_v(ctx, K, LR_RMAX, D(L.ta), XA, NA, NA, D(L.a2), NA, D(L.tb), XB, NB, NB, D(L.b2), NB,
+                                     p->probes, NB, D(L.vpart), ((NB + 511) / 512) * 128);
+        if (!rc && !fused)
+            rc = qk_compress_operands(ctx, K, LR_RMAX, D(L.ta), XA, NA, D(L.a2), D(L.tb), XB, NB, D(L.b2));
+        if (!rc && !fused)
             rc = qk_probe_errors(ctx, K, LR_RMAX, XA, NA, NA, D(L.a2), NA, U, D(L.b2), NB, NB, p->probes, NB, D(L.e2),
                                  r, p->rank_tol, p->rank_tol_rel, k, D(L.err), D(L.probe), L.probe_bytes);
     }
-    if (!rc)
+    if (!rc && fused)
+        rc = qk_knit_outer_stream_range_check(ctx, p->nbits, LR_RMAX, D(L.a2), NA, D(L.b2), NB, p->mask_a, p->mask_b, 0,
+                                              int64_t(1) << p->nbits, r, out, K, LR_RMAX, XA, NA, NA, D(L.a2), NA, U,
+                                              D(L.vpart), (NB + 511) / 512, D(L.epart), QK_N_CHECK);
+    if (!rc && !fused)
         rc = qk_knit_outer_stream_range(ctx, p->nbits, LR_RMAX, D(L.a2), NA, D(L.b2), NB, p->mask_a, p->mask_b, 0,
                                         int64_t(1) << p->nbits, k, out);
     if (rc) return rc;
@@ -324,7 +338,11 @@
     if (kb) hipLaunchKernelGGL(qk_pdep_keys_kernel, dim3(grid_of(NB)), dim3(256), 0, ctx->stream, NB, p->mask_b, kb);
     const int64_t sa = ka ? 0 : int64_t(1) << __builtin_ctzll(p->mask_a);
     const int64_t sb = kb ? 0 : int64_t(1) << __builtin_ctzll(p->mask_b);
-    rc = qk_gemm_keyed_pred(ctx, NA, NB, K, XA, NA, XB, NB, ka, sa, kb, sb, out, 0, k);
+    if (fused)
+        rc = qk_gemm_keyed_pred_accept(ctx, NA, NB, K, XA, NA, XB, NB, ka, sa, kb, sb, out, 0, D(L.epart), QK_N_CHECK, r,
+                                       p->rank_tol, p->rank_tol_rel, k, D(L.err), D(L.e2), nullptr);
+    else
+        rc = qk_gemm_keyed_pred(ctx, NA, NB, K, XA, NA, XB, NB, ka, sa, kb, sb, out, 0, k);
     if (rc) return rc;
     if (rank_out) hipLaunchKernelGGL(qk_copy_i32_kernel, dim3(1), dim3(1), 0, ctx->stream, k, rank_out);
     if (hipGetLastError() != hipSuccess) return pfail(ctx, QK_EHIP, "qk_knit_lowrank: launch failed");
diff --git a/hardwareawareoptimalquantumcircuitcuttingandknitting_amd/csrc/qknit_prep.hip b/hardwareawareoptimalquantumcircuitcuttingandknitting_amd/csrc/qknit_prep.hip
--- a/hardwareawareoptimalquantumcircuitcuttingandknitting_amd/csrc/qknit_prep.hip
+++ b/hardwareawareoptimalquantumcircuitcuttingandknitting_amd/csrc/qknit_prep.hip
@@ -4,6 +4,7 @@
 #include <string>
 
 #include "internal.h"
+#include "probe_check.h"
 
 namespace {
 
@@ -594,116 +595,23 @@
                                                          const double* __restrict__ U,
                                                          const double* __restrict__ vpart, int gv,
                                                          double* __restrict__ epart) {
-    __shared__ double Us[PK][PNP];
-    __shared__ double Vs[16][PNP];
-    __shared__ double ep[4][2 * PNP];
-    const int tid = threadIdx.x, lane = tid & 63, wave = tid >> 6, l16 = lane & 15, l4 = lane >> 4;
-    {
-        __shared__ double vh[PV_PART];
-        const int e = tid & (PV_PART - 1), h = tid >> 7;
-        double t[16];
-#pragma unroll
-        for (int u = 0; u < 16; ++u) t[u] = 0.0;
-        int b = h;
-        for (; b + 30 < gv; b += 32) {
-            double v[16];
-#pragma unroll
-            for (int u = 0; u < 16; ++u) v[u] = vpart[(int64_t)(b + 2 * u) * PV_PART + e];
-#pragma unroll
-            for (int u = 0; u < 16; ++u) t[u] += v[u];
-        }
-        for (; b < gv; b += 2) t[0] += vpart[(int64_t)b * PV_PART + e];
-#pragma unroll
-        for (int w = 8; w >= 1; w >>= 1)
-#pragma unroll
-            for (int u = 0; u < w; ++u) t[u] += t[u + w];
-        if (h == 1) vh[e] = t[0];
-        __syncthreads();
-        if (h == 0) Vs[e / 16][e % 16] = -(t[0] + vh[e]);
-        else Vs[8 + e / 16][e % 16] = 0.0;
-    }
-    for (int e = tid; e < PK * PNP; e += 256) Us[e / PNP][e % PNP] = (e / PNP) < K ? U[e] : 0.0;
-    __syncthreads();
-    double e2 = 0.0, f2 = 0.0;
-    for (int64_t cb = (int64_t)blockIdx.x * 4 + wave; cb * 16 < NA; cb += (int64_t)gridDim.x * 4) {
-        const int64_t c = cb * 16 + l16;
-        double av[PK / 4], a2[2];
-#pragma unroll
-        for (int kk = 0; kk < PK / 4; ++kk) av[kk] = XA[(int64_t)min(4 * kk + l4, K - 1) * ldx + c];
-#pragma unroll
-        for (int jj = 0; jj < 2; ++jj) a2[jj] = A2[(int64_t)min(4 * jj + l4, rmax - 1) * lda2 + c];
-        d4_t acc = {0, 0, 0, 0};
-#pragma unroll
-        for (int kk = 0; kk < PK / 4; ++kk)
-            acc = __builtin_amdgcn_mfma_f64_16x16x4f64(av[kk], Us[4 * kk + l4][l16], acc, 0, 0, 0);
-#pragma unroll
-        for (int rr = 0; rr < 4; ++rr) f2 = fma(acc[rr], acc[rr], f2);
-#pragma unroll
-        for (int jj = 0; jj < 2; ++jj)
-            acc = __builtin_amdgcn_mfma_f64_16x16x4f64(a2[jj], Vs[4 * jj + l4][l16], acc, 0, 0, 0);
-#pragma unroll
-        for (int rr = 0; rr < 4; ++rr) e2 = fma(acc[rr], acc[rr], e2);
-    }
-    e2 += __shfl_xor(e2, 16, 64);
-    e2 += __shfl_xor(e2, 32, 64);
-    f2 += __shfl_xor(f2, 16, 64);
-    f2 += __shfl_xor(f2, 32, 64);
-    if (l4 == 0) {
-        ep[wave][l16] = e2;
-        ep[wave][PNP + l16] = f2;
-    }
-    __syncthreads();
-    if (tid < 2 * PNP)
-        epart[(int64_t)blockIdx.x * 2 * PNP + tid] = ep[0][tid] + ep[1][tid] + ep[2][tid] + ep[3][tid];
+    __shared__ double lds[qk_check::D_LDS];
+    qk_check::probe_d_block(lds, K, rmax, XA, ldx, NA, A2, lda2, U, vpart, gv, epart, (int)blockIdx.x,
+                            (int)gridDim.x);
 }
 
 constexpr int PE = 2 * PNP;
+static_assert(PK == qk_check::CK && PNP == qk_check::CNP && PV_PART == qk_check::CV_PART && PE == qk_check::CE,
+              "probe_check.h constants");
 
 __global__ __launch_bounds__(256) void qk_probe_accept_kernel(const double* __restrict__ epart, int n,
                                                               const int32_t* __restrict__ r_dev, double tol,
                                                               double rel_tol, double* __restrict__ e2_out,
                                                               int32_t* __restrict__ k_out, double* __restrict__ err_out,
                                                               int64_t* __restrict__ tally = nullptr) {
-    __shared__ double acc[256];
-    const int tid = threadIdx.x, p = tid % PE;
-    constexpr int STEP = 256 / PE;
-    double s8[8] = {0, 0, 0, 0, 0, 0, 0, 0};
-    int b = tid / PE;
-    for (; b + 31 * STEP < n; b += 32 * STEP) {
-        double v[32];
-#pragma unroll
-        for (int u = 0; u < 32; ++u) v[u] = epart[(int64_t)(b + u * STEP) * PE + p];
-#pragma unroll
-        for (int u = 0; u < 32; ++u) s8[u & 7] += v[u];
-    }
-    for (; b < n; b += STEP) s8[0] += epart[(int64_t)b * PE + p];
-    const double s = ((s8[0] + s8[1]) + (s8[2] + s8[3])) + ((s8[4] + s8[5]) + (s8[6] + s8[7]));
-    acc[tid] = s;
-    __syncthreads();
-    for (int w = 128; w >= PE; w >>= 1) {
-        if (tid < w) acc[tid] += acc[tid + w];
-        __syncthreads();
-    }
-    if (tid < PE && e2_out) e2_out[tid] = acc[tid];
-    if (tid == 0 && k_out) {
-        double m = 0.0, f = 0.0;
-        for (int q = 0; q < PNP; ++q) {
-            m = fmax(m, acc[q]);
-            f = fmax(f, acc[PNP + q]);
-        }
-        const double err = sqrt(m);
-        const double bound = fmax(tol, rel_tol * sqrt(f));
-        const int r = *r_dev;
-        if (err_out) *err_out = err;
-        const int k = (r > 0 && err <= bound) ? r : 0;
-        *k_out = k;
-        if (tally) {
-            tally[0] += r == 0 ? 1 : 0;
-            tally[1] += (r > 0 && k == 0) ? 1 : 0;
-            tally[2] = k;
-            tally[3] += 1;
-        }
-    }
+    __shared__ double acc[qk_check::ACCEPT_LDS];
+    qk_check::probe_accept_fold(acc, epart, n, k_out ? r_dev : nullptr, tol, rel_tol, e2_out, k_out, err_out, tally,
+                                true);
 }
 
 constexpr int QG_T = 512;
diff --git a/hardwareawareoptimalquantumcircuitcuttingandknitting_amd/engine.py b/hardwareawareoptimalquantumcircuitcuttingandknitting_amd/engine.py
--- a/hardwareawareoptimalquantumcircuitcuttingandknitting_amd/engine.py
+++ b/hardwareawareoptimalquantumcircuitcuttingandknitting_amd/engine.py
@@ -574,7 +574,7 @@
 
 
 def gemm_keyed(ctx: Context, A, B, keyA=None, keyB=None, out=None, strideA: int = 0,
-               strideB: int = 1, beta: int = 0, skip=None):
+               strideB: int = 1, beta: int = 0, skip=None, accept=None):
     K, M = A.shape
     K2, N = B.shape
     assert K == K2 and A.dtype == B.dtype and (A.stride(1) == 1 or M == 1) and (B.stride(1) == 1 or N == 1)
@@ -583,6 +583,20 @@
         assert keyA.shape[0] == M and keyA.dtype == torch().int64
     if keyB is not None:
         assert keyB.shape[0] == N and keyB.dtype == torch().int64
+    if accept is not None:
+        T = torch()
+        ep, r, k = accept["epart"], accept["r"], accept["k"]
+        assert skip is None and ep.is_contiguous() and ep.dtype == T.float64 and ep.shape[1] == 2 * N_PROBES
+        assert r.dtype == T.int32 and k.dtype == T.int32
+        tally = accept.get("tally")
+        assert tally is None or (tally.dtype == T.int64 and tally.numel() == 4)
+        ctx.check(ctx.lib.qk_gemm_keyed_pred_accept(ctx.handle, M, N, K, A.data_ptr(), lda, B.data_ptr(), ldb,
+                                                    _ptr(keyA), strideA, _ptr(keyB), strideB, out.data_ptr(), beta,
+                                                    ep.data_ptr(), ep.shape[0], r.data_ptr(), float(accept["tol"]),
+                                                    float(accept["rel_tol"]), k.data_ptr(), _ptr(accept.get("err")),
+                                                    _ptr(accept.get("e2")), _ptr(tally)),
+                  "qk_gemm_keyed_pred_accept")
+        return out
     ctx.check(ctx.lib.qk_gemm_keyed_pred(ctx.handle, M, N, K, A.data_ptr(), lda, B.data_ptr(), ldb,
                                          _ptr(keyA), strideA, _ptr(keyB), strideB, out.data_ptr(), beta, _ptr(skip)),
               "qk_gemm_keyed_pred")
@@ -617,6 +631,39 @@
                                                  o_begin, o_count, _ptr(k_dev), out.data_ptr()),
               "qk_knit_outer_stream_range")
     return out
+
+
+N_CHECK = 256
+
+
+def knit_outer_stream_check(ctx: Context, A, B, clbits_a: list, clbits_b: list, nbits: int, out, XA, A2, U, vpart,
+                            o_begin: int = 0, o_count: int | None = None, k_dev=None, n_check: int = N_CHECK,
+                            epart=None):
+    T = torch()
+    K, M = A.shape
+    K2, N = B.shape
+    assert K == K2 and 1 <= K <= 8 and A.is_contiguous() and B.is_contiguous()
+    mA, mB = sum(1 << c for c in clbits_a), sum(1 << c for c in clbits_b)
+    if o_count is None:
+        o_count = (1 << nbits) - o_begin
+    assert M == 1 << len(clbits_a) and N == 1 << len(clbits_b) and out.numel() >= o_count
+    if k_dev is not None:
+        assert k_dev.dtype == T.int32 and k_dev.device == out.device
+    Kx, NA = XA.shape
+    rmax = A2.shape[0]
+    assert U.shape == (Kx, N_PROBES) and U.is_contiguous() and A2.shape[1] == NA and A2.is_contiguous()
+    assert XA.stride(1) == 1 and XA.stride(0) >= NA
+    assert vpart.is_contiguous() and vpart.shape[1:] == (8, N_PROBES)
+    if epart is None:
+        epart = T.empty((n_check, 2 * N_PROBES), dtype=T.float64, device=out.device)
+    assert epart.is_contiguous() and epart.shape == (n_check, 2 * N_PROBES)
+    ctx.check(ctx.lib.qk_knit_outer_stream_range_check(ctx.handle, nbits, K, A.data_ptr(), M, B.data_ptr(), N, mA, mB,
+                                                       o_begin, o_count, _ptr(k_dev), out.data_ptr(), Kx, rmax,
+                                                       XA.data_ptr(), XA.stride(0), NA, A2.data_ptr(), NA,
+                                                       U.data_ptr(), vpart.data_ptr(), vpart.shape[0],
+                                                       epart.data_ptr(), n_check),
+              "qk_knit_outer_stream_range_check")
+    return epart
 
 
 OUTER_STREAM_KERNELS = ("qk_knit_outer_stream_kernel", "qk_knit_outer_blocked_kernel",
diff --git a/hardwareawareoptimalquantumcircuitcuttingandknitting_amd/pipeline.py b/hardwareawareoptimalquantumcircuitcuttingandknitting_amd/pipeline.py
--- a/hardwareawareoptimalquantumcircuitcuttingandknitting_amd/pipeline.py
+++ b/hardwareawareoptimalquantumcircuitcuttingandknitting_amd/pipeline.py
@@ -261,6 +261,11 @@
     def outer_stream_kernel(self, K, clbits_a, clbits_b, nbits, o_begin=0, o_count=None):
         return engine.knit_outer_stream_kernel(K, clbits_a, clbits_b, nbits, o_begin, o_count)
 
+    def knit_outer_stream_check(self, A, B, clbits_a, clbits_b, nbits, out, XA, A2, U, vpart, k_dev=None):
+        n_check = int(os.environ.get("QKNIT_N_CHECK", engine.N_CHECK))
+        return engine.knit_outer_stream_check(self.ctx, A, B, clbits_a, clbits_b, nbits, out, XA, A2, U, vpart,
+                                              k_dev=k_dev, n_check=n_check)
+
     def rank_factors(self, GA, GB):
         return engine.rank_factors_device(self.ctx, GA, GB)
 
@@ -316,7 +321,8 @@
 class KnitPipeline:
     def __init__(self, virt, device: int = 0, factored: bool = False, rank: int = 0, world: int = 1,
                  mode: str | None = None, group=None, backend=None, chunk_jobs: int | None = None,
-                 jit: bool | None = None, light_cone: bool = True, data_rank: bool | None = None):
+                 jit: bool | None = None, light_cone: bool = True, data_rank: bool | None = None,
+                 fused_check: bool | None = None):
         self.be = backend if backend is not None else HipBackend(device)
         self.chunk_jobs = int(os.environ.get("QKNIT_SWEEP_CHUNK_JOBS", "0")) if chunk_jobs is None else chunk_jobs
         self.fork = False
@@ -383,6 +389,8 @@
         self.overlap = os.environ.get("QKNIT_OVERLAP", "0") == "1"
         self.spec_write = os.environ.get("QKNIT_SPEC_WRITE", "0") == "1"
         self._spec_stream = None
+        self.fused_check = (os.environ.get("QKNIT_FUSED_CHECK", "1") != "0" if fused_check is None
+                            else bool(fused_check))
         ob = os.environ.get("QKNIT_OUT_BUFFERS", "")
         self.out_buffers = int(ob) if ob else (3 if world >= 8 else 2 if world >= 2 else 1)
         self._outs = None
@@ -777,15 +785,17 @@
             self._probe = hit
         return self._probe
 
-    def _prep_step(self, qs) -> dict:
-        return self._prep_slice(qs) if self.mode == "slice" and self.sharded else self._prep_dev_rank(qs)
+    def _prep_step(self, qs, fused_ok: bool = False) -> dict:
+        if self.mode == "slice" and self.sharded:
+            return self._prep_slice(qs)
+        return self._prep_dev_rank(qs, fused_ok=fused_ok)
 
     def _launch_step(self, p: dict):
         return self._launch_slice(p) if self.mode == "slice" else self._launch_dev_rank(p)
 
     def knit(self, qs: list):
         if self.dev_rank and self.mode in ("single", "slice"):
-            p = self._prep_step(qs)
+            p = self._prep_step(qs, fused_ok=True)
             if self.out is None:
                 self.out = self._alloc_out(None)
             return self._launch_step(p)
@@ -867,7 +877,7 @@
             self._note_rank(r, k_eff)
         return k_eff, err
 
-    def _prep_dev_rank(self, qs) -> dict:
+    def _prep_dev_rank(self, qs, fused_ok: bool = False) -> dict:
         ia, ib = self.order[0], self.order[-1]
         if self._qspace_prep(qs):
             T = self.T
@@ -890,7 +900,7 @@
             mats, G, U = self._prep_fused(qs, x)
             TA, TB, r = self.be.rank_factors(G[0], G[1])
             if not self.spec_write:
-                return self._compress_and_check(TA, TB, r, mats, U, x)
+                return self._compress_and_check(TA, TB, r, mats, U, x, fused_ok=fused_ok)
             A2, B2 = self.be.compress(TA, mats[ia], TB, mats[ib])
             if self.spec_write and getattr(self.be, "dev", None) is not None and self.be.dev.type == "cuda":
                 T = self.T
@@ -926,7 +936,14 @@
         k_eff, _ = self._accept(A, B, A2, B2, self._probes(B.shape[1], B.device), r)
         return {"A2": A2, "B2": B2, "k_eff": k_eff, "mats": mats}
 
-    def _compress_and_check(self, TA, TB, r, mats, U, x) -> dict:
+    def _fused_check_ok(self, rmax: int) -> bool:
+        if not (self.fused_check and self.mode == "single" and len(self.order) == 2
+                and hasattr(self.be, "knit_outer_stream_check") and getattr(self.be, "fuses_tally", False)):
+            return False
+        ia, ib = self.order[0], self.order[-1]
+        return self._kernel_name(rmax, self.ops.clbits[ia], self.ops.clbits[ib]) == "qk_knit_outer_blocked_kernel"
+
+    def _compress_and_check(self, TA, TB, r, mats, U, x, fused_ok: bool = False) -> dict:
         ia, ib = self.order[0], self.order[-1]
         a_cols = self._replicated_a_cols()
         kw = {"a_cols": a_cols} if a_cols is not None else {}
@@ -937,6 +954,12 @@
         else:
             A2, B2 = self.be.compress(TA, mats[ia], TB, mats[ib], **kw)
         XA = mats[ia]
+        if fused_ok and cv is not None and a_cols is None and self._fused_check_ok(A2.shape[0]):
+            k_eff = self.T.empty(1, dtype=self.T.int32, device=r.device)
+            self._pending += 1
+            return {"A2": A2, "B2": B2, "k_eff": k_eff, "mats": mats,
+                    "fused": {"XA": XA, "U": U, "vpart": check["vpart"], "r": r,
+                              "tally": self._tally_for(r.device)}}
         if a_cols is not None:
             XA = XA[:, a_cols[0]:a_cols[0] + a_cols[1]]
             check["a2_cols"] = a_cols
@@ -962,10 +985,20 @@
             start, end = self.be.event(), self.be.event()
             start.record()
         self.last_kernel = self._kernel_name(p["A2"].shape[0], cA, cB)
-        self.be.knit_outer_stream(p["A2"], p["B2"], cA, cB, self.N, self.out, k_dev=p.get("k_write", p["k_eff"]))
+        f = p.get("fused")
+        if f is not None:
+            epart = self.be.knit_outer_stream_check(p["A2"], p["B2"], cA, cB, self.N, self.out, f["XA"], p["A2"],
+                                                    f["U"], f["vpart"], k_dev=f["r"])
+        else:
+            self.be.knit_outer_stream(p["A2"], p["B2"], cA, cB, self.N, self.out,
+                                      k_dev=p.get("k_write", p["k_eff"]))
         if self.record_events:
             end.record()
             self.events.append((start, end))
+        if f is not None:
+            return self._contract(p["mats"], accept={"epart": epart, "r": f["r"], "tol": self.rank_tol,
+                                                     "rel_tol": self.rank_tol_rel, "k": p["k_eff"],
+                                                     "tally": f["tally"]})
         if "check" in p:
             self.T.cuda.current_stream().wait_stream(p["check"])
         return self._contract(p["mats"], skip=p["k_eff"])
@@ -1450,9 +1483,11 @@
             engine.out_selections.append([f"drop-in first call: un-timed mapping wrote at {own.write_gbs:.1f} GB/s, "
                                           "replaced on the next call"])
 
-    def _contract(self, mats, skip=None):
+    def _contract(self, mats, skip=None, accept=None):
         if self.mode != "gather":
-            gemm = self.be.gemm_keyed if skip is None else (lambda A, B, **kw: self.be.gemm_keyed(A, B, skip=skip, **kw))
+            pred = {"accept": accept} if accept is not None else {"skip": skip}
+            gemm = self.be.gemm_keyed if skip is None and accept is None else (
+                lambda A, B, **kw: self.be.gemm_keyed(A, B, **pred, **kw))
             return engine.contract(None, mats, self.ops.clbits, self.out, gemm=gemm, kr=self.be.khatri_rao)
         order = self.order
         A = mats[order[0]]
diff --git a/include/qknit.h b/include/qknit.h
--- a/include/qknit.h
+++ b/include/qknit.h
@@ -128,6 +128,19 @@
 int qk_knit_outer_stream_range(qk_ctx* ctx, int nbits, int64_t K, const double* A, int64_t lda, const double* B,
                                int64_t ldb, uint64_t maskA, uint64_t maskB, int64_t o_begin, int64_t o_count,
                                const int32_t* k_dev, double* out);
+
+#define QK_N_CHECK 256
+int qk_knit_outer_stream_range_check(qk_ctx* ctx, int nbits, int64_t K, const double* A, int64_t lda, const double* B,
+                                     int64_t ldb, uint64_t maskA, uint64_t maskB, int64_t o_begin, int64_t o_count,
+                                     const int32_t* k_dev, double* out, int Kx, int rmax, const double* XA,
+                                     int64_t ldx, int64_t NA, const double* A2, int64_t lda2, const double* U,
+                                     const double* vpart, int64_t gv, double* epart, int n_check);
+
+int qk_gemm_keyed_pred_accept(qk_ctx* ctx, int64_t M, int64_t N, int64_t K, const double* A, int64_t lda,
+                              const double* B, int64_t ldb, const int64_t* keyA, int64_t strideA,
+                              const int64_t* keyB, int64_t strideB, double* out, int beta, const double* epart,
+                              int n, const int32_t* r_dev, double tol, double rel_tol, int32_t* k_out,
+                              double* err_out, double* e2_out, int64_t* tally);
 
 int qk_knit_outer_stream_kind(int nbits, int64_t K, uint64_t maskA, uint64_t maskB, int64_t o_begin,
                               int64_t o_count, int* kind, int* task_bits);
```

After: 516,300, median of 3. No clear change (+0.2%).
